# tomershay100/mp3-steganography-lib

Hardware: AMD Instinct MI355X
Metric: MP3 frames/sec (decode+re-encode) @44.1kHz stereo 128kbps, 1→8 GPU (higher is better)
Workload: dtype f64 (decode) / int32 (encode); 1 GPU; 10000-frame full decode->stego-embed->re-encode pipeline per MI355X (BASELINE configs[2]); MP3 main data + side info resident in HBM, MP3 frames out; the message cursor chain is decided and the serial chains of the rate loop are checked on the device inside every step; frames_per_gpu=10000, channels=2, message_bits=536, chain_verdict_units_to_redo=0, message_variant_entries=1874, parallelism=frames sharded over 1 GPU(s), no collective

## Files before the change

mp3-steganography-lib_amd/csrc/k_encode.hpp:

```cpp
#pragma once
#include <type_traits>
#include "analysis_plan.h"
#include "analysis_sign_plan.h"
#ifndef MP3S_AN_CLOCKS
#define MP3S_AN_CLOCKS 0
#endif
#if MP3S_AN_CLOCKS
__device__ uint32_t g_an_clocks[4096 * 8];
extern "C" __attribute__((visibility("default"))) int mp3s_debug_an_clocks(uint32_t *out)
{
    (void)hipDeviceSynchronize();
    return (int)hipMemcpyFromSymbol(out, HIP_SYMBOL(g_an_clocks), sizeof(uint32_t) * 4096 * 8);
}
#endif

namespace mp3s {

__device__ __forceinline__ int32_t mulhi_vs(int32_t v, int32_t s)
{
    int32_t r;
    asm("v_mul_hi_i32 %0, %1, %2" : "=v"(r) : "v"(v), "s"(s));
    return r;
}
typedef int32_t i32x4 __attribute__((ext_vector_type(4)));
typedef int32_t i32x16 __attribute__((ext_vector_type(16)));
typedef int32_t i32x8 __attribute__((ext_vector_type(8)));
template <int B, int E, class F>
__device__ __forceinline__ void static_for(F &&f)
{
    if constexpr (B < E) { f(std::integral_constant<int, B>{}); static_for<B + 1, E>(f); }
}

constexpr int ENC_ROW = 34;
constexpr int ENC_LDS_DW = 79 * 17 + 1;

constexpr int sign_plan_pass(int n)
{
    int p = 0;
    while (p < 7 && n >= ANALYSIS_SIGN_FIRST[p + 1]) p++;
    return p;
}
constexpr int sign_plan_pos(int n)
{
    int pos = 0;
    if (n >= ANALYSIS_SIGN_PRODUCTS) return 0;
    while (n - pos > ANALYSIS_SIGN_FIRST[sign_plan_pass(n)] && ANALYSIS_SIGN_SET[n - pos - 1] == ANALYSIS_SIGN_SET[n]) pos++;
    return pos;
}

constexpr int ENC_TROW = 33;
template <bool TILE, class Between>
__device__ __forceinline__ void enc_analysis_wave(const int16_t *__restrict__ pcm, const mp3s_frame_hdr *__restrict__ hdr, long Ts, int ch, long t0, int lane,
                                                  uint32_t *lds, int32_t *__restrict__ SB, uint32_t *rows, long tile_t0, long lo, long hi, bool shared, Between between)
{
    int16_t *tw = reinterpret_cast<int16_t *>(lds);
#if MP3S_AN_CLOCKS
    const unsigned long long ck_start = __builtin_readcyclecounter();
    unsigned long long ck_out = 0;
#endif
    if ((reinterpret_cast<uintptr_t>(pcm) & 15u) == 0) {
        const int c0 = (int)(t0 - 15) * 8, c1 = (int)Ts * 8;
        const uint4 *gp = reinterpret_cast<const uint4 *>(pcm);
        const uint32_t sel = ch ? 0x07060302u : 0x05040100u;
        constexpr int TRIPS = (79 * 8 + 63) / 64, LAST = 79 * 8 - 64 * (TRIPS - 1);
        uint4 q[TRIPS];
#pragma unroll
        for (int i = 0; i < TRIPS; i++) {
            const int gc = c0 + lane + 64 * i;
            q[i] = gp[gc < 0 ? 0 : gc < c1 ? gc : c1 - 1];
        }
#pragma unroll
        for (int i = 0; i < TRIPS; i++) {
            const int c = lane + 64 * i, gc = c0 + c;
            const bool in = gc >= 0 && gc < c1;
            asm volatile("" : "+v"(q[i].x), "+v"(q[i].y), "+v"(q[i].z), "+v"(q[i].w));
            uint2 o;
            o.x = in ? __builtin_amdgcn_perm(q[i].y, q[i].x, sel) : 0u;
            o.y = in ? __builtin_amdgcn_perm(q[i].w, q[i].z, sel) : 0u;
            uint32_t *dst = reinterpret_cast<uint32_t *>(tw + (c >> 3) * ENC_ROW + (c & 7) * 4);
            if (i < TRIPS - 1 || lane < LAST) { dst[0] = o.x; dst[1] = o.y; }
        }
    } else {
        for (int e = lane; e < 79 * 32; e += 64) {
            const int r = e >> 5, s = e & 31;
            const long row = t0 - 15 + r;
            int16_t v = 0;
            if (row >= 0 && row < Ts) v = pcm[(row * 32 + s) * 2 + ch];
            tw[r * ENC_ROW + s] = v;
        }
    }
    __builtin_amdgcn_s_waitcnt(0xc07f);
    __builtin_amdgcn_wave_barrier();
#if MP3S_AN_CLOCKS
    const unsigned long long ck_staged = __builtin_readcyclecounter();
#endif
    const long t = t0 + lane;
    const bool valid = t >= 0 && t < Ts;
    long s0 = 0;
    if (valid) s0 = (long)hdr[t / 36].stream_first * 36;

    int32_t y[64];
    const bool starts_inside = __ballot(valid && (t - 15) < s0) != 0;
    const uint32_t tw_lds = (uint32_t)(uintptr_t)(__attribute__((address_space(3))) const int16_t *)tw;
    uint32_t xs[16];
#pragma unroll
    for (int i = 0; i < 16; i++) xs[i] = 0;
#define MP3S_LDS_HI16(reg, addr, off) asm volatile("ds_read_u16_d16_hi %0, %1 offset:%2" : "+v"(reg) : "v"(addr), "n"(off))
    auto window_sums = [&](auto masked) {
    auto trip = [&](int k, auto first) {
        const i32x16 *ewa = reinterpret_cast<const i32x16 *>(c_tab.enwindow + 64 * k), *ewb = ewa + 4;
#pragma unroll
        for (int h = 0; h < 2; h++) {
            const i32x16 a0 = ewa[2 * h], a1 = ewa[2 * h + 1];
            const i32x16 b0 = ewb[2 * h], b1 = ewb[2 * h + 1];
            const int back_a = 2 * k + h, back_b = back_a + 2;
            const bool in_a = (t - back_a) >= s0, in_b = (t - back_b) >= s0;
            const uint32_t ra = tw_lds + (uint32_t)((lane + 15 - back_a) * ENC_ROW * 2), rb = ra - 2 * ENC_ROW * 2;
#pragma unroll
            for (int cb = 0; cb < 4; cb++) {
#pragma unroll
                for (int e = 0; e < 8; e++) {
                    MP3S_LDS_HI16(xs[e], ra, (cb * 8 + e) * 2);
                    MP3S_LDS_HI16(xs[8 + e], rb, (cb * 8 + e) * 2);
                }
                asm volatile("s_waitcnt lgkmcnt(0)" : "+v"(xs[0]), "+v"(xs[1]), "+v"(xs[2]), "+v"(xs[3]), "+v"(xs[4]), "+v"(xs[5]), "+v"(xs[6]), "+v"(xs[7]),
                             "+v"(xs[8]), "+v"(xs[9]), "+v"(xs[10]), "+v"(xs[11]), "+v"(xs[12]), "+v"(xs[13]), "+v"(xs[14]), "+v"(xs[15]));
#pragma unroll
                for (int e = 0; e < 8; e++) {
                    const int col = cb * 8 + e, c = 31 - col;
                    int32_t xa = (int32_t)xs[e], xb = (int32_t)xs[8 + e];
                    if (decltype(masked)::value && !in_a) xa = 0;
                    if (decltype(masked)::value && !in_b) xb = 0;
                    const int32_t two = mulhi_vs(xa, c < 16 ? a0[c & 15] : a1[c & 15]) + mulhi_vs(xb, c < 16 ? b0[c & 15] : b1[c & 15]);
                    if (decltype(first)::value) y[h * 32 + c] = two; else y[h * 32 + c] += two;
                }
                __builtin_amdgcn_sched_barrier(0);
            }
        }
    };
    trip(0, std::true_type{});
#pragma unroll 1
    for (int k = 2; k < 8; k += 2) trip(k, std::false_type{});
    };
    if (starts_inside) window_sums(std::true_type{}); else window_sums(std::false_type{});
#undef MP3S_LDS_HI16
#if MP3S_AN_CLOCKS
    asm volatile("" : "+v"(y[0]), "+v"(y[31]), "+v"(y[32]), "+v"(y[63]));
    const unsigned long long ck_summed = __builtin_readcyclecounter();
#endif
    const bool odd_slot = (t & 1) != 0;
    __builtin_amdgcn_wave_barrier();
    between();
    uint32_t *ot = lds;
    uint32_t *out = TILE ? nullptr : reinterpret_cast<uint32_t *>(SB) + ((long)ch * Ts + t0) * 32;
    const int n_rows = (Ts - t0) < 64 ? (int)(Ts - t0) : 64;
    uint32_t *trow = TILE ? rows + (valid && t >= lo && t < hi ? (t - tile_t0) : -1) * ENC_TROW : nullptr;
    int32_t a[4] = {0, 0, 0, 0};
    i32x8 cur[4], nxt[4];
    typedef const int32_t __attribute__((address_space(4))) *fl_ptr;
    fl_ptr flp = (fl_ptr)&c_tab.fl[0][0];
    asm volatile("" : "+s"(flp));
    auto load_block = [&](auto nc, i32x8 (&c)[4]) {
        constexpr int N = decltype(nc)::value, P = N >> 3, B = N & 7;
        constexpr int O[4] = {P, 15 - P, 16 + P, 31 - P};
#pragma unroll
        for (int o = 0; o < 4; o++) c[o] = *(const i32x8 __attribute__((address_space(4))) *)(flp + O[o] * 64 + 8 * B);
    };
    auto matrix_equal = [&](auto &&finish_pass) {
    load_block(std::integral_constant<int, 0>{}, cur);
    static_for<0, 64>([&](auto nc) {
        constexpr int N = decltype(nc)::value, P = N >> 3, B = N & 7;
        __builtin_amdgcn_sched_barrier(0);
        __builtin_amdgcn_s_waitcnt(0xc07f);
        __builtin_amdgcn_sched_barrier(0);
        if constexpr (N < 63) load_block(std::integral_constant<int, N + 1>{}, nxt);
        __builtin_amdgcn_sched_barrier(0);
#pragma unroll
        for (int j = 0; j < 8; j += 2) {
            int32_t m[2][4];
#pragma unroll
            for (int e = 0; e < 2; e++) {
                const int k = B * 8 + j + e;
                const unsigned plan = ANALYSIS_PLAN[P][k];
                const int32_t cj[4] = {cur[0][j + e], cur[1][j + e], cur[2][j + e], cur[3][j + e]};
#pragma unroll
                for (int o = 0; o < 4; o++) {
                    const unsigned rep = (plan >> (2 * o)) & 3u;
                    if ((plan >> (8 + o)) & 1u) m[e][o] = 0;
                    else if (rep == (unsigned)o) m[e][o] = mulhi_vs(y[k], cj[o]);
                    else m[e][o] = m[e][rep];
                }
            }
#pragma unroll
            for (int o = 0; o < 4; o++) {
                a[o] += m[0][o] + m[1][o];
                asm("" : "+v"(a[o]));
            }
            if (j == 2) __builtin_amdgcn_sched_barrier(0);
        }
        if constexpr (B == 7) {
            finish_pass(std::integral_constant<int, P>{});
            a[0] = a[1] = a[2] = a[3] = 0;
        }
        if constexpr (N < 63) {
#pragma unroll
            for (int o = 0; o < 4; o++) cur[o] = nxt[o];
        }
    });
    };
    auto finish_pass = [&](auto pc) {
            constexpr int P = decltype(pc)::value;
            if (odd_slot) {
                if (P & 1) { a[0] = (int32_t)(0u - (uint32_t)a[0]); a[2] = (int32_t)(0u - (uint32_t)a[2]); }
                else       { a[1] = (int32_t)(0u - (uint32_t)a[1]); a[3] = (int32_t)(0u - (uint32_t)a[3]); }
            }
            constexpr int q = P & 3;
            if constexpr (TILE) {
                trow[P] = (uint32_t)a[0]; trow[15 - P] = (uint32_t)a[1]; trow[16 + P] = (uint32_t)a[2]; trow[31 - P] = (uint32_t)a[3];
            } else {
            ot[lane * 17 + q] = (uint32_t)a[0];
            ot[lane * 17 + 4 + 3 - q] = (uint32_t)a[1];
            ot[lane * 17 + 8 + q] = (uint32_t)a[2];
            ot[lane * 17 + 12 + 3 - q] = (uint32_t)a[3];
            }
            if constexpr (q == 3 && !TILE) {
                constexpr int g = P >> 2;
#if MP3S_AN_CLOCKS
                const unsigned long long ck_o = __builtin_readcyclecounter();
#endif
                __builtin_amdgcn_s_waitcnt(0xc07f);
                __builtin_amdgcn_wave_barrier();
                const int piece = lane & 3;
#pragma unroll
                for (int r = lane >> 2; r < 64; r += 16) {
                    const uint32_t *src = ot + r * 17 + piece * 4;
                    const uint4 v = make_uint4(src[0], src[1], src[2], src[3]);
                    if (r < n_rows) *reinterpret_cast<uint4 *>(out + r * 32 + g * 16 + piece * 4) = v;
                }
                __builtin_amdgcn_s_waitcnt(0xc07f);
                __builtin_amdgcn_wave_barrier();
#if MP3S_AN_CLOCKS
                ck_out += __builtin_readcyclecounter() - ck_o;
#endif
            }
    };
    fl_ptr fsp = (fl_ptr)&c_fl_sign[0];
    auto load_sign_block = [&](auto bc, i32x8 (&c)[4]) {
        constexpr int Bk = decltype(bc)::value;
#pragma unroll
        for (int o = 0; o < 4; o++) c[o] = *(const i32x8 __attribute__((address_space(4))) *)(fsp + Bk * ANALYSIS_SIGN_BLOCK + 8 * o);
    };
    auto matrix_signed = [&]() {
    static_assert(ANALYSIS_SIGN_BLOCK == 32 && ANALYSIS_SIGN_STREAM % ANALYSIS_SIGN_BLOCK == 0, "four s_load_dwordx8 per block");
    constexpr int NBLK = ANALYSIS_SIGN_STREAM / ANALYSIS_SIGN_BLOCK;
    uint32_t S = 0, pend = 0;
    asm volatile("" : "+s"(fsp));
#pragma unroll
    for (int o = 0; o < 4; o++) a[o] = -ANALYSIS_SIGN_NEG[0][o];
    load_sign_block(std::integral_constant<int, 0>{}, cur);
    static_for<0, NBLK>([&](auto bc) {
        constexpr int Bk = decltype(bc)::value;
        __builtin_amdgcn_sched_barrier(0);
        __builtin_amdgcn_s_waitcnt(0xc07f);
        __builtin_amdgcn_sched_barrier(0);
        if constexpr (Bk + 1 < NBLK) load_sign_block(std::integral_constant<int, Bk + 1>{}, nxt);
        __builtin_amdgcn_sched_barrier(0);
        static_for<0, ANALYSIS_SIGN_BLOCK / 8>([&](auto qc) {
            constexpr int Q = decltype(qc)::value;
            uint32_t m[8];
            static_for<0, 8>([&](auto ic) {
                constexpr int I = Q * 8 + decltype(ic)::value, n = Bk * ANALYSIS_SIGN_BLOCK + I;
                if constexpr (n < ANALYSIS_SIGN_PRODUCTS) m[I & 7] = (uint32_t)mulhi_vs(y[ANALYSIS_SIGN_COL[n]], cur[I >> 3][I & 7]);
            });
            static_for<0, 8>([&](auto ic) {
                constexpr int I = Q * 8 + decltype(ic)::value, n = Bk * ANALYSIS_SIGN_BLOCK + I;
                if constexpr (n < ANALYSIS_SIGN_PRODUCTS) {
                    constexpr int P = sign_plan_pass(n), pos = sign_plan_pos(n);
                    constexpr unsigned set = ANALYSIS_SIGN_SET[n];
                    constexpr bool last = sign_plan_pos(n + 1) == 0;
                    constexpr bool multi = ((set & 0x55u) & ((set & 0x55u) - 1u)) != 0;
                    if constexpr ((pos & 1) == 0 && !last) pend = m[I & 7];
                    else {
                        const uint32_t two = (pos & 1) ? pend + m[I & 7] : m[I & 7];
                        if constexpr (!multi) {
#pragma unroll
                            for (int o = 0; o < 4; o++)
                                if ((set >> (2 * o)) & 1u) a[o] = (int32_t)((uint32_t)a[o] + two);
                        } else {
                            if constexpr (pos < 2) S = two; else S += two;
                            if constexpr (last) {
#pragma unroll
                                for (int o = 0; o < 4; o++) {
                                    const unsigned f = (set >> (2 * o)) & 3u;
                                    if (f == 1u) a[o] = (int32_t)((uint32_t)a[o] + S);
                                    if (f == 3u) a[o] = (int32_t)((uint32_t)a[o] - S);
                                }
                            }
                        }
                    }
                    if constexpr (n + 1 == ANALYSIS_SIGN_FIRST[P + 1]) {
                        finish_pass(std::integral_constant<int, P>{});
                        if constexpr (P < 7) {
#pragma unroll
                            for (int o = 0; o < 4; o++) a[o] = -ANALYSIS_SIGN_NEG[P + 1][o];
                        }
                    }
                }
            });
            asm("" : "+v"(a[0]), "+v"(a[1]), "+v"(a[2]), "+v"(a[3]), "+v"(S), "+v"(pend));
            __builtin_amdgcn_sched_barrier(0);
        });
        if constexpr (Bk + 1 < NBLK) {
#pragma unroll
            for (int o = 0; o < 4; o++) cur[o] = nxt[o];
        }
    });
    };
    bool use_signed = shared;
    if (shared) {
        uint32_t ymin = 0xffffffffu;
        static_for<0, 64>([&](auto kc) {
            constexpr int k = decltype(kc)::value;
            if constexpr ((ANALYSIS_SIGN_ZERO_COLS >> k) & 1u) ymin = ymin < (uint32_t)y[k] ? ymin : (uint32_t)y[k];
        });
        const bool counts = valid && (!TILE || (t >= lo && t < hi));
        use_signed = __ballot(counts && ymin == 0u) == 0;
    }
    if (use_signed) matrix_signed(); else matrix_equal(finish_pass);
#if MP3S_AN_CLOCKS
    if (!TILE && lane == 0) {
        const unsigned long long ck_end = __builtin_readcyclecounter();
        uint32_t *d = g_an_clocks + ((size_t)((t0 >> 6) * 2 + ch) & 4095) * 8;
        d[0] = (uint32_t)(ck_staged - ck_start); d[1] = (uint32_t)(ck_summed - ck_staged); d[2] = (uint32_t)(ck_end - ck_summed - ck_out);
        d[3] = (uint32_t)ck_out; d[4] = (uint32_t)(ck_end - ck_start); d[5] = (starts_inside ? 1u : 0u) | (use_signed ? 2u : 0u);
    }
#endif
}

__device__ __forceinline__ int sb_pos(int band) { return (int)((0x37621540u >> (4 * (band >> 2))) & 7u) * 4 + (band & 3); }
__global__ __launch_bounds__(256, 5) void k_enc_analysis(
    const int16_t *__restrict__ pcm, const mp3s_frame_hdr *__restrict__ hdr, int n_frames,
    int32_t *__restrict__ SB, long Ts, int shared)
{
    __shared__ __attribute__((aligned(16))) uint32_t lds_all[4][ENC_LDS_DW];
    static_assert(79 * ENC_ROW * 2 <= ENC_LDS_DW * 4, "PCM tile must fit");
    const int wave = __builtin_amdgcn_readfirstlane(threadIdx.x >> 6), lane = threadIdx.x & 63;
    const long wid = (long)xcd_tile() * 4 + wave;
    const int ch = (int)(wid & 1);
    const long t0 = (wid >> 1) * 64;
    if (t0 >= Ts) return;
    enc_analysis_wave<false>(pcm, hdr, Ts, ch, t0, lane, lds_all[wave], SB, nullptr, 0, 0, 0, shared != 0, [] {});
}

constexpr int MD_ROW = 33, MD_BLK = 18 * MD_ROW;

__device__ __forceinline__ void enc_mdct_pair(const int32_t (&in)[54], int32_t *xs, int lane, int32_t *__restrict__ mdct, long ga, long g_lo, long g_hi)
{
    const int ch = lane >> 5, band = lane & 31;
    int32_t *x0 = xs + ch * MD_BLK + band, *x1 = x0 + 2 * MD_BLK;
    struct Coef { i32x4 q[9]; };
    auto load_coef = [&](int k) {
        Coef c;
        const i32x4 *crow = reinterpret_cast<const i32x4 *>(c_tab.cos_l[k]);
#pragma unroll
        for (int q = 0; q < 9; q++) c.q[q] = crow[q];
        return c;
    };
    Coef cur = load_coef(0);
#pragma unroll 2
    for (int k = 0; k < 18; k++) {
        asm volatile("" ::"s"(cur.q[0].x));
        __builtin_amdgcn_sched_barrier(0);
        const Coef nxt = load_coef(k < 17 ? k + 1 : 17);
        __builtin_amdgcn_sched_barrier(0);
        int32_t a0 = 0, a1 = 0;
#pragma unroll
        for (int q = 0; q < 9; q++) {
            const i32x4 c = cur.q[q];
            a0 += mulhi_vs(in[4 * q], c.x);     a1 += mulhi_vs(in[18 + 4 * q], c.x);
            a0 += mulhi_vs(in[4 * q + 1], c.y); a1 += mulhi_vs(in[19 + 4 * q], c.y);
            a0 += mulhi_vs(in[4 * q + 2], c.z); a1 += mulhi_vs(in[20 + 4 * q], c.z);
            a0 += mulhi_vs(in[4 * q + 3], c.w); a1 += mulhi_vs(in[21 + 4 * q], c.w);
        }
        x0[k * MD_ROW] = a0;
        x1[k * MD_ROW] = a1;
        __builtin_amdgcn_sched_barrier(0);
        cur = nxt;
    }
    __builtin_amdgcn_s_waitcnt(0xc07f);
    __builtin_amdgcn_wave_barrier();
    if (band >= 1) {
#pragma unroll
        for (int g = 0; g < 2; g++)
#pragma unroll
            for (int i = 0; i < 8; i++) {
                int32_t *pa = x0 + g * 2 * MD_BLK + i * MD_ROW, *pb = x0 + g * 2 * MD_BLK + (17 - i) * MD_ROW - 1;
                const int64_t cs = c_tab.mdct_cs[i], ca = c_tab.mdct_ca[i];
                const int64_t a = *pa, b = *pb;
                *pa = (int32_t)((a * cs - b * ca) >> 31);
                *pb = (int32_t)((a * ca + b * cs) >> 31);
            }
    }
    __builtin_amdgcn_s_waitcnt(0xc07f);
    __builtin_amdgcn_wave_barrier();
#pragma unroll
    for (int q = 0; q < 4; q++) {
        const long g = ga + (q >> 1);
        if (g < g_lo || g >= g_hi) continue;
        const int32_t *src = xs + q * MD_BLK;
        int32_t *o = mdct + (((g >> 1) * 2 + (q & 1)) * 2 + (g & 1)) * 576;
#pragma unroll
        for (int t = 0; t < 9; t++) {
            const int e = lane + 64 * t, b = (e * 3641) >> 16, k = e - 18 * b;
            o[e] = src[k * MD_ROW + b];
        }
    }
}

__global__ __launch_bounds__(256, 4) void k_enc_mdct(
    const int32_t *__restrict__ SB, long Ts, const mp3s_frame_hdr *__restrict__ hdr, int n_frames,
    int32_t *__restrict__ mdct)
{
    __shared__ int32_t xs_all[4][4 * MD_BLK];
    const int wave = __builtin_amdgcn_readfirstlane(threadIdx.x >> 6), lane = threadIdx.x & 63;
    const int f = xcd_tile() * 4 + wave;
    if (f >= n_frames) return;
    const int ch = lane >> 5, band = lane & 31;
    const bool has_prev = f > (int)hdr[f].stream_first;
    const int32_t *row = SB + ((long)ch * Ts + (long)f * 36) * 32 + sb_pos(band);
    const int32_t *prow = has_prev ? row - 18 * 32 : row;
    int32_t in[54];
#pragma unroll
    for (int j = 0; j < 18; j++) {
        const int32_t pv = prow[j * 32];
        in[j] = has_prev ? pv : 0;
        in[18 + j] = row[j * 32];
        in[36 + j] = row[(18 + j) * 32];
    }
    enc_mdct_pair(in, xs_all[wave], lane, mdct, 2l * f, 2l * f, 2l * f + 2);
}

constexpr int EF_GR = 13, EF_SLOTS = 18 * (EF_GR + 1), EF_WAVES = 8;
constexpr int EF_TILE_DW = 2 * (EF_SLOTS + 1) * ENC_TROW;
static_assert(EF_SLOTS <= 4 * 64, "four analysis waves per channel");
static_assert(EF_WAVES * ENC_LDS_DW <= EF_TILE_DW, "the waves' PCM staging fits the tile");
static_assert(((EF_GR + 1) / 2) * 4 * MD_BLK <= EF_TILE_DW, "the MDCT waves' butterfly tiles fit the tile");

__global__ __launch_bounds__(EF_WAVES * 64, 4) void k_enc_fused(
    const int16_t *__restrict__ pcm, const mp3s_frame_hdr *__restrict__ hdr, int n_frames, int32_t *__restrict__ mdct, int shared)
{
    __shared__ __attribute__((aligned(16))) uint32_t tile[EF_TILE_DW];
    const int wave = __builtin_amdgcn_readfirstlane(threadIdx.x >> 6), lane = threadIdx.x & 63;
    const long Ts = (long)n_frames * 36, n_gran = (long)n_frames * 2;
    const long g0 = (long)xcd_tile() * EF_GR;
    const long s0 = g0 * 18, t_first = s0 - 18;
    {
        const int ch = wave >> 2;
        const long t0 = t_first + 64 * (wave & 3);
        uint32_t *rows = tile + ((long)ch * (EF_SLOTS + 1) + 1) * ENC_TROW;
        enc_analysis_wave<true>(pcm, hdr, Ts, ch, t0, lane, tile + wave * ENC_LDS_DW, nullptr, rows, t_first, t_first, t_first + EF_SLOTS, shared != 0,
                                [] { __syncthreads(); });
    }
    __syncthreads();
    const long ga = g0 - (g0 & 1) + 2 * wave;
    const long g_hi = g0 + EF_GR < n_gran ? g0 + EF_GR : n_gran;
    const bool unit = ga < g_hi;
    int32_t in[54];
    if (unit) {
        const int ch = lane >> 5, band = lane & 31;
        const bool has_prev = ga >= g0 && ga > (long)hdr[ga >> 1].stream_first * 2;
        const long r_prev = (ga - g0) * 18;
        const uint32_t *row = tile + ((long)ch * (EF_SLOTS + 1) + 1 + (r_prev >= 0 ? r_prev : 0)) * ENC_TROW + band;
        const long r_own = r_prev >= 0 ? 18 : 0;
#pragma unroll
        for (int j = 0; j < 18; j++) {
            const int32_t pv = (int32_t)row[j * ENC_TROW];
            in[j] = has_prev ? pv : 0;
            in[18 + j] = (int32_t)row[(r_own + j) * ENC_TROW];
            in[36 + j] = ga + 1 < g_hi ? (int32_t)row[(r_own + 18 + j) * ENC_TROW] : 0;
        }
    }
    __syncthreads();
    if (unit) enc_mdct_pair(in, reinterpret_cast<int32_t *>(tile) + wave * 4 * MD_BLK, lane, mdct, ga, g0, g_hi);
}

}
```

mp3-steganography-lib_amd/csrc/mp3s_api.cpp:

```cpp
#include "chain_resolve.h"

namespace {
thread_local std::string g_err;
}

int mp3s::fail(int code, const char *fmt, ...)
{
    char buf[512];
    va_list ap;
    va_start(ap, fmt);
    vsnprintf(buf, sizeof buf, fmt, ap);
    va_end(ap);
    g_err = buf;
    return code;
}

int max_part2_3(const mp3s_frame_side *side, long n)
{
    int m = 0;
    for (long f = 0; f < n; f++)
        for (int k = 0; k < 4; k++) m = std::max<int>(m, side[f].unit[k >> 1][k & 1].part2_3_length);
    return m;
}

void select_entries(int first_unit, int reach, int first_entry, int hide_end, int64_t bits_left, int32_t *ent_unit, int32_t *ent_cursor)
{
    const int tail = (int)MP3S_SELECT_TAIL_FIRST(bits_left, (int64_t)reach);
    int at = first_entry;
    for (int v = 0; v < MP3S_SELECT_VARIANTS; v++) {
        const int32_t cur = v < 8 ? 4 * v : hide_end - (10 - v);
        for (int j = v < 8 ? 0 : tail; j < reach; j++) {
            ent_unit[at] = first_unit + j;
            ent_cursor[at++] = cur;
        }
    }
}

enum OptKind { kOptFlag, kOptNumber, kOptClamped, kOptMask, kOptOneOf };
struct OptRow { int id; const char *env; bool env_off; OptKind kind; int64_t dflt, lo, hi; };
constexpr int64_t kOptNoLimit = INT64_MAX, kResampleValues[] = {0, 1, 32000, 44100, 48000};
constexpr OptRow kOptions[] = {
    {MP3S_OPT_ANALYSIS_SHARED, "MP3S_ANALYSIS_SHARED", false, kOptFlag, 1, 0, 1},
    {MP3S_OPT_SELECT, "MP3S_NO_SELECT", true, kOptFlag, 1, 0, 1},
    {MP3S_OPT_REDO, "MP3S_NO_REDO", true, kOptFlag, 1, 0, 1},
    {MP3S_OPT_FAST_IMDCT, "MP3S_FAST_IMDCT", false, kOptFlag, 1, 0, 1},
    {MP3S_OPT_PIPE_TAIL, "MP3S_PIPE_TAIL", false, kOptClamped, 1, 0, 2},
    {MP3S_OPT_CHUNK_FRAMES, "MP3S_CHUNK_FRAMES", false, kOptNumber, 0, 4, kOptNoLimit},
    {MP3S_OPT_DEVICE_PARSE, "MP3S_DEVICE_PARSE", false, kOptFlag, 1, 0, 1},
    {MP3S_OPT_FILE_PIPELINE, "MP3S_FILE_PIPELINE", false, kOptFlag, 1, 0, 1},
    {MP3S_OPT_SCAN_THREADS, "MP3S_SCAN_THREADS", false, kOptNumber, 0, 0, 64},
    {MP3S_OPT_FIRST_CHUNK_FRAMES, "MP3S_FIRST_CHUNK_FRAMES", false, kOptNumber, 0, 4, kOptNoLimit},
    {MP3S_OPT_FILE_UP, "MP3S_NO_FILE_UP", true, kOptFlag, 1, 0, 1},
    {MP3S_OPT_HUF_LANES, "MP3S_HUF_LANES", false, kOptNumber, 0, 0, kOptNoLimit},
    {MP3S_OPT_NUMA, "MP3S_NO_NUMA", true, kOptFlag, 1, 0, 1},
    {MP3S_OPT_FLOAT_FAST, "MP3S_FLOAT_FAST", false, kOptFlag, 0, 0, 1},
    {MP3S_OPT_FAIL_CHUNK, nullptr, false, kOptNumber, 0, 0, kOptNoLimit},
    {MP3S_OPT_FUSED_DECODE, "MP3S_FUSED_DECODE", false, kOptFlag, 1, 0, 1},
    {MP3S_OPT_FUSED_ENCODE, "MP3S_FUSED_ENCODE", false, kOptFlag, 0, 0, 1},
    {MP3S_OPT_PIPE_DEC, "MP3S_PIPE_DEC", false, kOptFlag, 0, 0, 1},
    {MP3S_OPT_RATE_SIGNALS, "MP3S_RATE_SIGNALS", false, kOptFlag, 0, 0, 1},
    {MP3S_OPT_PIPE_SIGNALS, "MP3S_PIPE_SIGNALS", false, kOptMask, 0, 0, 3},
    {MP3S_OPT_WAV_IMPORT, "MP3S_WAV_IMPORT", false, kOptFlag, 0, 0, 1},
    {MP3S_OPT_WAV_RESAMPLE, "MP3S_WAV_RESAMPLE", false, kOptOneOf, 0, 0, 48000},
};
constexpr bool options_in_order(int i = 0) { return i == MP3S_OPT_COUNT || (kOptions[i].id == i && options_in_order(i + 1)); }
static_assert(sizeof kOptions / sizeof *kOptions == MP3S_OPT_COUNT && options_in_order(), "one row per MP3S_OPT_*, row i for option i");

static bool resample_value(int64_t v) { return std::find(std::begin(kResampleValues), std::end(kResampleValues), v) != std::end(kResampleValues); }
static int64_t option_from_env(const OptRow &o)
{
    const char *v = o.env ? getenv(o.env) : nullptr;
    if (o.env_off) return v ? 0 : o.dflt;
    const int64_t x = v && *v ? (int64_t)atoll(v) : o.dflt;
    switch (o.kind) {
    case kOptFlag: return x != 0;
    case kOptNumber: return std::max<int64_t>(0, x);
    case kOptClamped: return std::min(o.hi, std::max(o.lo, x));
    case kOptMask: return x & o.hi;
    default: return resample_value(x) ? x : 0;
    }
}

extern "C" {

const char *mp3s_last_error(void) { return g_err.c_str(); }
const char *mp3s_version(void) { return "mp3s-hip 0.1 (gfx950)"; }
void mp3s_buf_free(mp3s_buf *b) { delete b; }
const void *mp3s_debug_tables(size_t *bytes)
{
    if (bytes) *bytes = sizeof(DevTables);
    return &host_tables().dev;
}

int mp3s_debug_scfsi_energies(const int32_t *xr576, int sr_idx, int32_t *en22)
{
    if (!xr576 || !en22 || sr_idx < 0 || sr_idx > 2) return fail(MP3S_E_ARG, "bad argument");
    host_scfsi_energies(xr576, sr_idx, en22);
    return MP3S_OK;
}

int mp3s_debug_parse_scanned_frame(const void *frame_side, const uint8_t *blob, int16_t *is2304, mp3s_granule_si *si4)
{
    if (!frame_side || !blob || !is2304 || !si4) return fail(MP3S_E_ARG, "null pointer");
    const int rc = parse_scanned_frame(*static_cast<const mp3s_frame_side *>(frame_side), blob, is2304, si4);
    return rc ? fail(rc, "malformed main data") : MP3S_OK;
}

int mp3s_debug_walk_rate(const uint8_t *file, size_t len, double seconds, double *frames_per_s, int64_t *frames_per_pass)
{
    if (!file || !frames_per_s || seconds <= 0) return fail(MP3S_E_ARG, "bad argument");
    std::vector<FrameRef> refs;
    std::vector<uint8_t> tables;
    const double t0 = now_ms();
    int64_t frames = 0, per_pass = 0;
    double t = t0;
    do {
        FrameWalker w;
        const long n = std::max(0L, walk_whole(file, len, refs, w, &tables, 1000));
        if (w.irregular) return fail(MP3S_E_UNSUPPORTED, "not a stream the walk takes");
        if (!w.ended) return fail(MP3S_E_MALFORMED, "malformed or unsupported MP3 stream");
        frames += n; per_pass = n;
        t = now_ms();
    } while (t - t0 < seconds * 1e3);
    *frames_per_s = (double)frames / ((t - t0) * 1e-3);
    if (frames_per_pass) *frames_per_pass = per_pass;
    return MP3S_OK;
}

int mp3s_device_count(int *n)
{
    if (!n) return fail(MP3S_E_ARG, "n is null");
    int k = 0;
    *n = hipGetDeviceCount(&k) == hipSuccess && k > 0 ? k : 0;
    return MP3S_OK;
}

int mp3s_ctx_create(int device, mp3s_ctx **out)
{
    if (!out) return fail(MP3S_E_ARG, "out is null");
    *out = nullptr;
    int n = 0;
    hipError_t e = hipGetDeviceCount(&n);
    if (e != hipSuccess || n <= 0)
        return fail(MP3S_E_NO_DEVICE, "no HIP device available (%s); the transforms have no CPU fallback",
                    e == hipSuccess ? "device count 0" : hipGetErrorString(e));
    if (device < 0 || device >= n) return fail(MP3S_E_ARG, "device %d out of range (0..%d)", device, n - 1);
    e = hipSetDevice(device);
    if (e != hipSuccess) return fail(MP3S_E_NO_DEVICE, "hipSetDevice(%d): %s", device, hipGetErrorString(e));
    mp3s_ctx *c = new mp3s_ctx();
    c->chain = new ChainResolver();
    c->device = device;
    for (const OptRow &o : kOptions) c->opt[o.id] = option_from_env(o);
    if (hipStreamCreateWithFlags(&c->stream, hipStreamNonBlocking) != hipSuccess ||
        hipEventCreate(&c->ev0) != hipSuccess || hipEventCreate(&c->ev1) != hipSuccess ||
        hipEventCreateWithFlags(&c->ev_order, hipEventDisableTiming) != hipSuccess) {
        mp3s_ctx_destroy(c);
        return fail(MP3S_E_NO_DEVICE, "stream/event creation failed");
    }
    if (hipMalloc((void **)&c->d_sync, 32) != hipSuccess || hipMemsetAsync(c->d_sync, 0, 32, c->stream) != hipSuccess) {
        mp3s_ctx_destroy(c);
        return fail(MP3S_E_NO_DEVICE, "device scratch allocation failed");
    }
    const int rc = dev_upload_tables(c->stream);
    if (rc) {
        mp3s_ctx_destroy(c);
        return fail(MP3S_E_NO_DEVICE, "constant table upload failed: %s (is this a gfx950 device?)",
                    hipGetErrorString((hipError_t)rc));
    }
    *out = c;
    return MP3S_OK;
}

void mp3s_ctx_destroy(mp3s_ctx *c)
{
    if (!c) return;
    hipSetDevice(c->device);
    destroy_own_pipe(c);
    if (c->stream) hipStreamSynchronize(c->stream);
    if (c->scratch) hipFree(c->scratch);
    if (c->scratch_enc) hipFree(c->scratch_enc);
    if (c->d_sync) hipFree(c->d_sync);
    for (void *q : c->pool) if (q) hipFree(q);
    for (const mp3s_ctx::ResampleTaps &t : c->res_taps) hipFree(t.d);
    if (c->ev0) hipEventDestroy(c->ev0);
    if (c->ev1) hipEventDestroy(c->ev1);
    if (c->ev_order) hipEventDestroy(c->ev_order);
    if (c->ev_sel) hipEventDestroy(c->ev_sel);
    if (c->ev_pcm_tiles) hipEventDestroy(c->ev_pcm_tiles);
    if (c->stream) hipStreamDestroy(c->stream);
    delete c->chain;
    delete c;
}

int mp3s_ctx_host_share(mp3s_ctx *c, mp3s_host_share *out)
{
    if (!out) return fail(MP3S_E_ARG, "null pointer");
    size_t held = 0, cap = 0;
    PinnedBlock::pool_state(&held, &cap);
    out->pinned_pooled_bytes = held; out->pinned_pool_cap_bytes = cap;
    out->local_world_size = local_world_size();
    out->cpus_allowed = host_cpus_allowed();
    out->gpu_node_cpus = c ? (int32_t)gpu_node_cpus(c->device).size() : 0;
    out->reserved = 0;
    return MP3S_OK;
}

int mp3s_ctx_set_option(mp3s_ctx *c, int option, int64_t value)
{
    if (!c || option < 0 || option >= MP3S_OPT_COUNT) return fail(MP3S_E_ARG, "unknown option %d", option);
    const OptRow &o = kOptions[option];
    if (value < 0 || (o.kind == kOptNumber && ((value != 0 && value < o.lo) || value > o.hi)))
        return fail(MP3S_E_ARG, "option %d: value %lld out of range", option, (long long)value);
    if (o.kind == kOptOneOf && !resample_value(value))
        return fail(MP3S_E_ARG, "option %d: %lld is not 0, 1, 32000, 44100 or 48000", option, (long long)value);
    c->opt[option] = o.kind == kOptFlag ? value != 0 : (o.kind == kOptClamped ? std::min(value, o.hi) : value);
    return MP3S_OK;
}

int mp3s_ctx_run_stats(mp3s_ctx *c, mp3s_run_stats *out)
{
    if (!c || !out) return fail(MP3S_E_ARG, "null pointer");
    *out = c->run_stats;
    own_pipe_lanes(c, out);
    return MP3S_OK;
}

int mp3s_ctx_get_option(mp3s_ctx *c, int option, int64_t *value)
{
    if (!c || !value || option < 0 || option >= MP3S_OPT_COUNT) return fail(MP3S_E_ARG, "unknown option %d", option);
    *value = c->opt[option];
    return MP3S_OK;
}

int mp3s_device_name(mp3s_ctx *c, char *buf, size_t n)
{
    if (!c || !buf || !n) return fail(MP3S_E_ARG, "bad argument");
    hipDeviceProp_t p;
    HIPCHK(hipGetDeviceProperties(&p, c->device));
    snprintf(buf, n, "%s (%s, %d CUs)", p.name, p.gcnArchName, p.multiProcessorCount);
    return MP3S_OK;
}

int mp3s_device_pci(mp3s_ctx *c, char *buf, size_t n)
{
    if (!c || !buf || n < 16) return fail(MP3S_E_ARG, "bad argument");
    HIPCHK(hipDeviceGetPCIBusId(buf, (int)n, c->device));
    for (char *p = buf; *p; p++) *p = (char)tolower(*p);
    return MP3S_OK;
}

int mp3s_sync(mp3s_ctx *c)
{
    if (!c) return fail(MP3S_E_ARG, "ctx is null");
    HIPCHK(hipStreamSynchronize(c->stream));
    return MP3S_OK;
}

int mp3s_ctx_wait(mp3s_ctx *c, mp3s_ctx *other)
{
    if (!c || !other) return fail(MP3S_E_ARG, "ctx is null");
    if (c == other) return MP3S_OK;
    if (c->device != other->device) return fail(MP3S_E_ARG, "contexts on different devices");
    HIPCHK(hipEventRecord(other->ev_order, other->stream));
    HIPCHK(hipStreamWaitEvent(c->stream, other->ev_order, 0));
    return MP3S_OK;
}

int mp3s_ctx_wait_last(mp3s_ctx *c, mp3s_ctx *other)
{
    if (!c || !other) return fail(MP3S_E_ARG, "ctx is null");
    if (c == other) return MP3S_OK;
    if (c->device != other->device) return fail(MP3S_E_ARG, "contexts on different devices");
    HIPCHK(hipStreamWaitEvent(c->stream, other->ev_order, 0));
    return MP3S_OK;
}

int mp3s_dev_alloc(mp3s_ctx *c, size_t bytes, void **dptr)
{
    if (!c || !dptr) return fail(MP3S_E_ARG, "bad argument");
    HIPCHK(hipSetDevice(c->device));
    hipError_t e = hipMalloc(dptr, bytes ? bytes : 16);
    if (e != hipSuccess) return fail(MP3S_E_NOMEM, "hipMalloc(%zu): %s", bytes, hipGetErrorString(e));
    return MP3S_OK;
}
int mp3s_dev_free(mp3s_ctx *c, void *dptr)
{
    if (!c) return fail(MP3S_E_ARG, "ctx is null");
    if (dptr) { HIPCHK(hipStreamSynchronize(c->stream)); HIPCHK(hipFree(dptr)); }
    return MP3S_OK;
}
int mp3s_dev_upload(mp3s_ctx *c, void *dptr, const void *host, size_t bytes)
{
    if (!c || (!dptr && bytes) || (!host && bytes)) return fail(MP3S_E_ARG, "bad argument");
    if (!bytes) return MP3S_OK;
    HIPCHK(hipMemcpyAsync(dptr, host, bytes, hipMemcpyHostToDevice, c->stream));
    HIPCHK(hipStreamSynchronize(c->stream));
    return MP3S_OK;
}
int mp3s_dev_download(mp3s_ctx *c, void *host, const void *dptr, size_t bytes)
{
    if (!c || (!dptr && bytes) || (!host && bytes)) return fail(MP3S_E_ARG, "bad argument");
    if (!bytes) return MP3S_OK;
    HIPCHK(hipMemcpyAsync(host, dptr, bytes, hipMemcpyDeviceToHost, c->stream));
    HIPCHK(hipStreamSynchronize(c->stream));
    return MP3S_OK;
}
int mp3s_dev_memset(mp3s_ctx *c, void *dptr, int value, size_t bytes)
{
    if (!c || !dptr) return fail(MP3S_E_ARG, "bad argument");
    HIPCHK(hipMemsetAsync(dptr, value, bytes, c->stream));
    return MP3S_OK;
}
int mp3s_dev_copy(mp3s_ctx *c, void *d_dst, const void *d_src, size_t bytes)
{
    if (!c || !d_dst || !d_src) return fail(MP3S_E_ARG, "bad argument");
    if (bytes) HIPCHK(hipMemcpyAsync(d_dst, d_src, bytes, hipMemcpyDeviceToDevice, c->stream));
    return MP3S_OK;
}
int mp3s_timer_start(mp3s_ctx *c)
{
    if (!c) return fail(MP3S_E_ARG, "ctx is null");
    HIPCHK(hipEventRecord(c->ev0, c->stream));
    return MP3S_OK;
}
int mp3s_timer_stop(mp3s_ctx *c, float *ms)
{
    if (!c || !ms) return fail(MP3S_E_ARG, "bad argument");
    HIPCHK(hipEventRecord(c->ev1, c->stream));
    HIPCHK(hipEventSynchronize(c->ev1));
    HIPCHK(hipEventElapsedTime(ms, c->ev0, c->ev1));
    return MP3S_OK;
}

int mp3s_synth_mode(mp3s_ctx *c, double eps_scale, int64_t *exact_samples)
{
    if (!c || eps_scale < 0) return fail(MP3S_E_ARG, "bad argument");
    HIPCHK(hipStreamSynchronize(c->stream));
    int32_t n = 0;
    HIPCHK(hipMemcpy(&n, c->d_sync + 2, 4, hipMemcpyDeviceToHost));
    HIPCHK(hipMemset(c->d_sync + 2, 0, 4));
    if (exact_samples) *exact_samples = n;
    c->synth_eps_scale = eps_scale;
    return MP3S_OK;
}

int mp3s_bench_copy(mp3s_ctx *c, size_t bytes, int iters, double *gb_per_s)
{
    if (!c || !gb_per_s || bytes < 4096 || iters < 1) return fail(MP3S_E_ARG, "bad argument");
    HIPCHK(hipSetDevice(c->device));
    bytes &= ~(size_t)15;
    void *a = nullptr, *b = nullptr;
    if (hipMalloc(&a, bytes) != hipSuccess || hipMalloc(&b, bytes) != hipSuccess) { if (a) hipFree(a); return fail(MP3S_E_NOMEM, "hipMalloc(%zu) x 2", bytes); }
    int rc = MP3S_OK;
    float ms = 0;
    if (hipMemsetAsync(a, 1, bytes, c->stream) != hipSuccess || launch_copy(c->stream, a, b, bytes) != 0) rc = fail(MP3S_E_HIP, "copy launch failed");
    if (!rc && hipEventRecord(c->ev0, c->stream) != hipSuccess) rc = fail(MP3S_E_HIP, "event");
    for (int i = 0; i < iters && !rc; i++) if (launch_copy(c->stream, i & 1 ? b : a, i & 1 ? a : b, bytes) != 0) rc = fail(MP3S_E_HIP, "copy launch failed");
    if (!rc && (hipEventRecord(c->ev1, c->stream) != hipSuccess || hipEventSynchronize(c->ev1) != hipSuccess ||
                hipEventElapsedTime(&ms, c->ev0, c->ev1) != hipSuccess)) rc = fail(MP3S_E_HIP, "event");
    hipStreamSynchronize(c->stream);
    hipFree(a); hipFree(b);
    if (!rc) *gb_per_s = 2.0 * (double)bytes * iters / (ms * 1e-3) / 1e9;
    return rc;
}

int mp3s_profile_enable(mp3s_ctx *c, int on)
{
    if (!c) return fail(MP3S_E_ARG, "ctx is null");
    HIPCHK(hipStreamSynchronize(c->stream));
    c->prof.enabled = on != 0;
    c->prof.n_pairs = 0;
    for (int k = 0; k < K_COUNT; k++) { c->prof.total_ms[k] = 0; c->prof.count[k] = 0; }
    return MP3S_OK;
}

int mp3s_profile_select(mp3s_ctx *c, unsigned mask)
{
    if (!c) return fail(MP3S_E_ARG, "ctx is null");
    c->prof.mask = mask;
    return MP3S_OK;
}

int mp3s_profile_collect(mp3s_ctx *c, double *total_ms, int64_t *launches, int n)
{
    if (!c || !total_ms || !launches || n < MP3S_N_KERNELS_MIN) return fail(MP3S_E_ARG, "bad argument (need %d slots)", (int)MP3S_N_KERNELS_MIN);
    HIPCHK(hipStreamSynchronize(c->stream));
    Profiler &p = c->prof;
    for (int i = 0; i < p.n_pairs; i++) {
        float ms = 0;
        HIPCHK(hipEventElapsedTime(&ms, p.ev[2 * i], p.ev[2 * i + 1]));
        p.total_ms[p.kid[i]] += ms;
        p.count[p.kid[i]] += 1;
    }
    p.n_pairs = 0;
    if (p.dropped) {
        const long lost = p.dropped;
        p.dropped = 0;
        return fail(MP3S_E_ARG, "%ld timed launches had no event pair left (collect at least every %d launches)", lost, Profiler::MAX_PAIRS);
    }
    for (int k = 0; k < K_COUNT && k < n; k++) { total_ms[k] = p.total_ms[k]; launches[k] = p.count[k]; }
    static_assert(K_COUNT == MP3S_N_KERNELS, "kernel list out of sync with mp3s.h");
    return MP3S_OK;
}

int mp3s_decode_transform_dev(mp3s_ctx *c, const int16_t *d_is, const mp3s_granule_si *d_si, const mp3s_frame_hdr *d_hdr,
                              int n_frames, int nch, int n_halo, int out_format, void *d_pcm)
{
    if (!c || !d_is || !d_si || !d_hdr || !d_pcm) return fail(MP3S_E_ARG, "null pointer");
    if (n_frames <= 0 || nch < 1 || nch > 2 || n_halo < 0 || n_halo >= n_frames || out_format < 0 || out_format > 2)
        return fail(MP3S_E_ARG, "bad sizes: n_frames=%d nch=%d n_halo=%d fmt=%d", n_frames, nch, n_halo, out_format);
    if (const int rc = c->ensure_scratch(dec_scratch_bytes(n_frames, nch))) return rc;
    if (int pe = guard_probe_usable(c, out_format)) return pe;
    const int e = launch_decode(c->stream, d_is, d_si, d_hdr, n_frames, nch, n_halo, out_format, d_pcm, c->scratch, &c->prof, decode_how(c, 0, nullptr, 0));
    return e ? fail(MP3S_E_HIP, "decode launch: %s", hipGetErrorString((hipError_t)e)) : (int)MP3S_OK;
}

int mp3s_debug_guard_margin(mp3s_ctx *c, double *d_x, double *d_eps, int64_t capacity)
{
    if (!c) return fail(MP3S_E_ARG, "null context");
    if ((d_x == nullptr) != (d_eps == nullptr) || (d_x && capacity <= 0)) return fail(MP3S_E_ARG, "both arrays and their capacity, or neither");
    HIPCHK(hipStreamSynchronize(c->stream));
    c->guard_probe = GuardProbe{d_x, d_eps, 0, d_x ? capacity : 0};
    return MP3S_OK;
}

static int check_hdr(const mp3s_frame_hdr *hdr, int n)
{
    for (int f = 0; f < n; f++) {
        if (hdr[f].stream_first > (uint32_t)f) return fail(MP3S_E_ARG, "hdr[%d].stream_first=%u points forward", f, hdr[f].stream_first);
        if (f && hdr[f].stream_first != (uint32_t)f && hdr[f].stream_first != hdr[f - 1].stream_first)
            return fail(MP3S_E_ARG, "hdr[%d].stream_first is not monotone", f);
        if (hdr[f].sr_idx > 2) return fail(MP3S_E_ARG, "hdr[%d].sr_idx=%d", f, hdr[f].sr_idx);
    }
    if (n && hdr[0].stream_first != 0) return fail(MP3S_E_ARG, "hdr[0].stream_first must be 0");
    return 0;
}

int mp3s_decode_transform(mp3s_ctx *c, const int16_t *is, const mp3s_granule_si *si, const mp3s_frame_hdr *hdr,
                          int n_frames, int nch, int n_halo, int out_format, void *pcm)
{
    if (!c || !is || !si || !hdr || !pcm) return fail(MP3S_E_ARG, "null pointer");
    if (n_frames <= 0 || n_halo < 0 || n_halo >= n_frames) return fail(MP3S_E_ARG, "bad sizes");
    int rc = check_hdr(hdr, n_frames);
    if (rc) return rc;
    for (size_t i = 0; i < (size_t)n_frames * 2304; i++)
        if (is[i] > 8206 || is[i] < -8206) return fail(MP3S_E_ARG, "is[%zu]=%d outside +-8206", i, is[i]);
    HIPCHK(hipSetDevice(c->device));
    void *d_is = nullptr, *d_si = nullptr, *d_hdr = nullptr, *d_pcm = nullptr;
    const size_t b_is = (size_t)n_frames * 2304 * 2, b_si = (size_t)n_frames * 4 * sizeof(mp3s_granule_si),
                 b_hdr = (size_t)n_frames * sizeof(mp3s_frame_hdr),
                 b_pcm = (size_t)(n_frames - n_halo) * 1152 * nch * pcm_elem(out_format);
    rc = MP3S_OK;
    if (hipMalloc(&d_is, b_is) != hipSuccess || hipMalloc(&d_si, b_si) != hipSuccess ||
        hipMalloc(&d_hdr, b_hdr) != hipSuccess || hipMalloc(&d_pcm, b_pcm) != hipSuccess)
        rc = fail(MP3S_E_NOMEM, "hipMalloc failed for a %d-frame batch", n_frames);
    if (!rc) rc = mp3s_dev_upload(c, d_is, is, b_is);
    if (!rc) rc = mp3s_dev_upload(c, d_si, si, b_si);
    if (!rc) rc = mp3s_dev_upload(c, d_hdr, hdr, b_hdr);
    if (!rc) rc = mp3s_decode_transform_dev(c, (const int16_t *)d_is, (const mp3s_granule_si *)d_si,
                                            (const mp3s_frame_hdr *)d_hdr, n_frames, nch, n_halo, out_format, d_pcm);
    if (!rc) rc = mp3s_dev_download(c, pcm, d_pcm, b_pcm);
    hipStreamSynchronize(c->stream);
    hipFree(d_is); hipFree(d_si); hipFree(d_hdr); hipFree(d_pcm);
    return rc;
}

int mp3s_encode_transform_dev(mp3s_ctx *c, const int16_t *d_pcm, const mp3s_frame_hdr *d_hdr, int n_frames, int32_t *d_mdct)
{
    if (!c || !d_pcm || !d_hdr || !d_mdct) return fail(MP3S_E_ARG, "null pointer");
    if (n_frames <= 0) return fail(MP3S_E_ARG, "n_frames=%d", n_frames);
    return encode_transform_step(c, c->stream, d_pcm, d_hdr, n_frames, d_mdct);
}

int mp3s_encode_transform(mp3s_ctx *c, const int16_t *pcm, const mp3s_frame_hdr *hdr, int n_frames, int32_t *mdct)
{
    if (!c || !pcm || !hdr || !mdct) return fail(MP3S_E_ARG, "null pointer");
    if (n_frames <= 0) return fail(MP3S_E_ARG, "n_frames=%d", n_frames);
    int rc = check_hdr(hdr, n_frames);
    if (rc) return rc;
    HIPCHK(hipSetDevice(c->device));
    void *d_pcm = nullptr, *d_hdr = nullptr, *d_mdct = nullptr;
    const size_t b_pcm = (size_t)n_frames * 1152 * 2 * 2, b_hdr = (size_t)n_frames * sizeof(mp3s_frame_hdr),
                 b_mdct = (size_t)n_frames * 2304 * 4;
    if (hipMalloc(&d_pcm, b_pcm) != hipSuccess || hipMalloc(&d_hdr, b_hdr) != hipSuccess ||
        hipMalloc(&d_mdct, b_mdct) != hipSuccess)
        rc = fail(MP3S_E_NOMEM, "hipMalloc failed for a %d-frame batch", n_frames);
    if (!rc) rc = mp3s_dev_upload(c, d_pcm, pcm, b_pcm);
    if (!rc) rc = mp3s_dev_upload(c, d_hdr, hdr, b_hdr);
    if (!rc) rc = mp3s_encode_transform_dev(c, (const int16_t *)d_pcm, (const mp3s_frame_hdr *)d_hdr, n_frames, (int32_t *)d_mdct);
    if (!rc) rc = mp3s_dev_download(c, mdct, d_mdct, b_mdct);
    hipStreamSynchronize(c->stream);
    hipFree(d_pcm); hipFree(d_hdr); hipFree(d_mdct);
    return rc;
}

int mp3s_rate_loop_dev(mp3s_ctx *c, const int32_t *d_mdct, const mp3s_rate_frame *d_frames, int n_frames,
                       const uint8_t *d_hide_bits, int n_hide, const int32_t *d_cursor_in, const int32_t *d_state_in,
                       const int32_t *d_unit_list, int n_list, int16_t *d_ix, mp3s_gr_out *d_out, int32_t *d_en)
{
    if (!c || !d_mdct || !d_frames || !d_ix || !d_out || !d_en) return fail(MP3S_E_ARG, "null pointer");
    if (n_frames <= 0 || n_hide < 0 || (n_hide > 0 && (!d_hide_bits || !d_cursor_in)))
        return fail(MP3S_E_ARG, "bad sizes / missing hide inputs");
    return rate_step(c, c->stream, rate_signal_default(c), d_mdct, d_frames, n_frames, d_hide_bits, n_hide, d_cursor_in, d_state_in, d_unit_list, n_list, d_ix, d_out, d_en);
}

void mp3s_select_patterns(uint8_t out[32])
{
    for (int v = 0; v < 8; v++) { out[4 * v] = (v >> 2) & 1; out[4 * v + 1] = (v >> 1) & 1; out[4 * v + 2] = v & 1; out[4 * v + 3] = 0; }
}

int mp3s_select_plan(const mp3s_chain_seg *segs, int n_segs, mp3s_select_span *spans, int32_t *ent_unit, int32_t *ent_cursor, int cap)
{
    return select_plan(segs, n_segs, spans, ent_unit, ent_cursor, cap, nullptr);
}

}

int select_plan(const mp3s_chain_seg *segs, int n_segs, mp3s_select_span *spans, int32_t *ent_unit, int32_t *ent_cursor, int cap,
                const int32_t *min_reach)
{
    if (!segs || !spans || n_segs <= 0 || cap < 0 || ((ent_unit == nullptr) != (ent_cursor == nullptr))) return fail(MP3S_E_ARG, "bad argument");
    int used = 0;
    for (int i = 0; i < n_segs; i++) {
        const mp3s_chain_seg &g = segs[i];
        spans[i].first_entry = used; spans[i].reach = 0;
        const int64_t left = (int64_t)g.hide_end - g.hide_begin;
        if (left <= 0 || g.n_frames <= 0 || g.hide_base < 32) continue;
        const int64_t reach = std::min<int64_t>((int64_t)g.n_frames * 4, std::max<int64_t>(left * 5 / 14 + 32, min_reach ? min_reach[i] : 0));
        if (reach > MP3S_SELECT_MAX_REACH || (int64_t)used + MP3S_SELECT_ENTRIES(left, reach) > cap) continue;
        spans[i].reach = (int32_t)reach;
        if (ent_unit) select_entries(g.first_frame * 4, (int)reach, used, g.hide_end, left, ent_unit, ent_cursor);
        used += (int)MP3S_SELECT_ENTRIES(left, reach);
    }
    return used;
}

int encode_transform_step(mp3s_ctx *c, hipStream_t stream, const int16_t *d_pcm, const mp3s_frame_hdr *d_hdr, int n_frames, int32_t *d_mdct)
{
    if (!host_tables().analysis_plan_ok)
        return fail(MP3S_E_TABLES, "the analysis filter table built on this host does not repeat itself where the kernel shares products "
                                   "(csrc/analysis_plan.h, csrc/analysis_sign_plan.h: run tools/gen_analysis_plan.py and tools/gen_analysis_sign_plan.py here and rebuild)");
    const bool fused = c->opt[MP3S_OPT_FUSED_ENCODE] != 0;
    if (const int rc = fused ? (int)MP3S_OK : c->ensure_scratch_enc(enc_scratch_bytes(n_frames))) return rc;
    const int e = launch_encode(stream, d_pcm, d_hdr, n_frames, d_mdct, c->scratch_enc, &c->prof, fused, c->opt[MP3S_OPT_ANALYSIS_SHARED] != 0);
    return e ? fail(MP3S_E_HIP, "encode launch: %s", hipGetErrorString((hipError_t)e)) : (int)MP3S_OK;
}

int rate_step(mp3s_ctx *c, hipStream_t stream, hipEvent_t done, const int32_t *d_mdct, const mp3s_rate_frame *d_frames, int n_frames, const uint8_t *d_hide,
              int n_hide, const int32_t *d_cursor, const int32_t *d_state, const int32_t *d_list, int n_list, int16_t *d_ix, mp3s_gr_out *d_out, int32_t *d_en,
              const RateVariantArgs *variants)
{
    if (variants && c->sel_pending && hipStreamWaitEvent(stream, c->ev_sel, 0) != hipSuccess) return fail(MP3S_E_HIP, "ordering behind the previous selection failed");
    if (variants) c->sel_pending = false;
    const int e = launch_rate(stream, d_mdct, d_frames, n_frames, d_hide, n_hide, d_cursor, d_state, d_list, n_list, d_ix, d_out, d_en, &c->prof, 0, 0, variants, done);
    return e ? fail(MP3S_E_HIP, "rate launch: %s", hipGetErrorString((hipError_t)e)) : (int)MP3S_OK;
}

int select_step(mp3s_ctx *c, hipStream_t stream, const uint8_t *d_hide, int32_t *d_cursor, const mp3s_chain_seg *d_segs, const mp3s_select_span *d_spans,
                int n_segs, int max_reach, const RateVariantArgs &va, int16_t *d_ix, mp3s_gr_out *d_out, int32_t *d_en)
{
    void *d_pairs = c->grab(kPoolSelectDev, (size_t)n_segs * max_reach * 8, stream);
    if (!d_pairs) return fail(MP3S_E_NOMEM, "hipMalloc failed for the selection scratch");
    const int e = launch_select(stream, d_segs, d_spans, n_segs, max_reach, d_hide, va, d_ix, d_en, d_out, d_cursor, d_pairs, &c->prof);
    if (e) return fail(MP3S_E_HIP, "select launch: %s", hipGetErrorString((hipError_t)e));
    if (stream == c->stream) return MP3S_OK;
    if (!c->ev_sel && hipEventCreateWithFlags(&c->ev_sel, hipEventDisableTiming) != hipSuccess) return fail(MP3S_E_HIP, "event creation failed");
    if (hipEventRecord(c->ev_sel, stream) != hipSuccess) return fail(MP3S_E_HIP, "event record failed");
    c->sel_pending = true;
    return MP3S_OK;
}

int pack_step(mp3s_ctx *c, hipStream_t stream, const int16_t *d_ix, const mp3s_gr_out *d_gr, const int32_t *d_en, int n_frames, int sri, int bri, int whole,
              const uint32_t *d_frame_off, const uint8_t *d_padding, uint8_t *d_mp3, int32_t *d_scfsi, int32_t *d_status)
{
    const int e = launch_pack(stream, d_ix, d_gr, d_en, n_frames, sri, bri, whole, d_frame_off, d_padding, d_mp3, d_scfsi, d_status, c->d_sync, &c->prof);
    return e ? fail(MP3S_E_HIP, "pack launch: %s", hipGetErrorString((hipError_t)e)) : (int)MP3S_OK;
}

extern "C" {

int mp3s_rate_variants_dev(mp3s_ctx *c, const int32_t *d_mdct, const mp3s_rate_frame *d_frames, int n_frames, const uint8_t *d_hide_bits,
                           int n_hide, const int32_t *d_cursor, const int32_t *d_ent_unit, const int32_t *d_ent_cursor, int n_entries,
                           int16_t *d_ix, mp3s_gr_out *d_out, int32_t *d_en, int16_t *d_ixv, mp3s_gr_out *d_outv, int32_t *d_env)
{
    if (!c || !d_mdct || !d_frames || !d_ix || !d_out || !d_en || !d_hide_bits || !d_cursor || !d_ent_unit || !d_ent_cursor || !d_ixv ||
        !d_outv || !d_env)
        return fail(MP3S_E_ARG, "null pointer");
    if (n_frames <= 0 || n_hide < 32 || n_entries <= 0) return fail(MP3S_E_ARG, "bad sizes");
    const RateVariantArgs va = variant_args(d_ent_unit, d_ent_cursor, n_entries, d_ixv, d_outv, d_env);
    return rate_step(c, c->stream, rate_signal_default(c), d_mdct, d_frames, n_frames, d_hide_bits, n_hide, d_cursor, nullptr, nullptr, 0, d_ix, d_out, d_en, &va);
}

int mp3s_select_dev(mp3s_ctx *c, const uint8_t *d_hide_bits, int32_t *d_cursor, const mp3s_chain_seg *d_segs, const mp3s_select_span *d_spans,
                    int n_segs, int max_reach, const int32_t *d_ent_unit, const int32_t *d_ent_cursor, int n_entries, int16_t *d_ix,
                    mp3s_gr_out *d_out, int32_t *d_en, int16_t *d_ixv, mp3s_gr_out *d_outv, int32_t *d_env)
{
    if (!c || !d_ix || !d_out || !d_en || !d_hide_bits || !d_cursor || !d_segs || !d_spans || !d_ent_unit || !d_ent_cursor || !d_ixv ||
        !d_outv || !d_env)
        return fail(MP3S_E_ARG, "null pointer");
    if (n_segs <= 0 || n_entries <= 0 || max_reach <= 0 || max_reach > MP3S_SELECT_MAX_REACH) return fail(MP3S_E_ARG, "bad sizes");
    return select_step(c, c->stream, d_hide_bits, d_cursor, d_segs, d_spans, n_segs, max_reach, variant_args(d_ent_unit, d_ent_cursor, n_entries, d_ixv, d_outv, d_env),
                       d_ix, d_out, d_en);
}

int mp3s_rate_select_dev(mp3s_ctx *c, const int32_t *d_mdct, const mp3s_rate_frame *d_frames, int n_frames, const uint8_t *d_hide_bits,
                         int n_hide, int32_t *d_cursor, const mp3s_chain_seg *d_segs, const mp3s_select_span *d_spans, int n_segs,
                         int max_reach, const int32_t *d_ent_unit, const int32_t *d_ent_cursor, int n_entries, int16_t *d_ix,
                         mp3s_gr_out *d_out, int32_t *d_en, int16_t *d_ixv, mp3s_gr_out *d_outv, int32_t *d_env)
{
    if (!d_segs || !d_spans) return fail(MP3S_E_ARG, "null pointer");
    if (n_segs <= 0 || max_reach <= 0 || max_reach > MP3S_SELECT_MAX_REACH) return fail(MP3S_E_ARG, "bad sizes");
    if (const int rc = mp3s_rate_variants_dev(c, d_mdct, d_frames, n_frames, d_hide_bits, n_hide, d_cursor, d_ent_unit, d_ent_cursor, n_entries, d_ix, d_out, d_en, d_ixv,
                                              d_outv, d_env)) return rc;
    return mp3s_select_dev(c, d_hide_bits, d_cursor, d_segs, d_spans, n_segs, max_reach, d_ent_unit, d_ent_cursor, n_entries, d_ix, d_out, d_en,
                           d_ixv, d_outv, d_env);
}

int mp3s_chain_resolve_dev(mp3s_ctx *c, mp3s_gr_out *d_gr, const mp3s_rate_frame *d_frames, int n_frames, const mp3s_chain_seg *d_segs,
                           int n_segs, const int32_t *d_cursor_in, const int32_t *d_state_in, int32_t *d_verdict,
                           mp3s_chain_seg_out *d_seg_out)
{
    if (!c || !d_gr || !d_frames || !d_segs || !d_verdict || !d_seg_out) return fail(MP3S_E_ARG, "null pointer");
    if (n_frames <= 0 || n_segs <= 0) return fail(MP3S_E_ARG, "bad sizes");
    void *d_agg = c->grab(kPoolChainDev, chain_agg_bytes(n_frames));
    if (!d_agg) return fail(MP3S_E_NOMEM, "hipMalloc failed for the chain scratch");
    const int e = launch_chain(c->stream, d_gr, d_frames, n_frames, d_segs, d_cursor_in, d_state_in, d_agg, d_verdict, d_seg_out, &c->prof);
    if (e) return fail(MP3S_E_HIP, "chain launch: %s", hipGetErrorString((hipError_t)e));
    return MP3S_OK;
}

int mp3s_chain_redo_dev(mp3s_ctx *c, const int32_t *d_mdct, const mp3s_rate_frame *d_frames, int n_frames, const uint8_t *d_hide_bits, int n_hide,
                        int32_t *d_cursor, const mp3s_chain_seg *d_segs, int n_segs, int16_t *d_ix, mp3s_gr_out *d_gr, int32_t *d_en,
                        int32_t *d_verdict, mp3s_chain_seg_out *d_seg_out)
{
    if (!c || !d_mdct || !d_gr || !d_frames || !d_segs || !d_verdict || !d_seg_out || !d_ix || !d_en) return fail(MP3S_E_ARG, "null pointer");
    if (n_frames <= 0 || n_segs <= 0 || n_hide < 0 || (n_hide > 0 && (!d_hide_bits || !d_cursor))) return fail(MP3S_E_ARG, "bad sizes");
    void *d_agg = c->grab(kPoolChainDev, chain_agg_bytes(n_frames));
    if (!d_agg) return fail(MP3S_E_NOMEM, "hipMalloc failed for the chain scratch");
    const ChainRedoArgs redo = {d_mdct, d_hide_bits, n_hide, d_ix, d_en};
    const int e = launch_chain(c->stream, d_gr, d_frames, n_frames, d_segs, d_cursor, nullptr, d_agg, d_verdict, d_seg_out, &c->prof, &redo);
    if (e) return fail(MP3S_E_HIP, "chain launch: %s", hipGetErrorString((hipError_t)e));
    return MP3S_OK;
}

int mp3s_huffman_decode_dev(mp3s_ctx *c, const uint8_t *d_blob, const mp3s_frame_side *d_side, int n_frames, int nch,
                            int max_part2_3_length, int16_t *d_is, mp3s_granule_si *d_si, int32_t *d_status)
{
    if (!c || !d_blob || !d_side || !d_is || !d_si || !d_status) return fail(MP3S_E_ARG, "null pointer");
    if (n_frames <= 0 || nch < 1 || nch > 2 || max_part2_3_length < 0) return fail(MP3S_E_ARG, "bad sizes");
    if (max_part2_3_length == 0 || max_part2_3_length > 4095) max_part2_3_length = 4095;
    const int e = launch_huffman(c->stream, d_blob, d_side, n_frames, nch, max_part2_3_length, d_is, d_si, d_status, c->d_sync + 4, &c->prof, false, (int)c->opt[MP3S_OPT_HUF_LANES]);
    if (e) return fail(MP3S_E_HIP, "huffman launch: %s", hipGetErrorString((hipError_t)e));
    return MP3S_OK;
}

int mp3s_pack_frames_dev(mp3s_ctx *c, const int16_t *d_ix, const mp3s_gr_out *d_gr, const int32_t *d_en, int n_frames,
                         int samplerate, int bitrate_kbps, const uint32_t *d_frame_off, const uint8_t *d_padding,
                         uint8_t *d_mp3, int32_t *d_scfsi, int32_t *d_status)
{
    if (!c || !d_ix || !d_gr || !d_en || !d_frame_off || !d_padding || !d_mp3 || !d_scfsi || !d_status)
        return fail(MP3S_E_ARG, "null pointer");
    int sri, bri, whole;
    if (n_frames <= 0 || stream_params(samplerate, bitrate_kbps, &sri, &bri, &whole))
        return fail(MP3S_E_UNSUPPORTED, "unsupported samplerate/bitrate %d/%d", samplerate, bitrate_kbps);
    return pack_step(c, c->stream, d_ix, d_gr, d_en, n_frames, sri, bri, whole, d_frame_off, d_padding, d_mp3, d_scfsi, d_status);
}

int mp3s_scan_stream(const uint8_t *file, size_t len, mp3s_buf **owner, mp3s_scanned *out)
{
    if (!file || !owner || !out) return fail(MP3S_E_ARG, "null pointer");
    mp3s_buf *b = new mp3s_buf();
    const int rc = parse_stream(file, len, b->parsed, &b->scanned);
    if (rc) { delete b; return fail(rc, "malformed or unsupported MP3 stream"); }
    const ParsedStream &p = b->parsed;
    out->n_frames = p.n_frames; out->nch = p.nch; out->sampling_rate = p.sampling_rate; out->bit_rate = p.bit_rate;
    out->n_bits = (int32_t)p.bits.size(); out->dup_last_frame = p.dup_last_frame;
    out->gpu_ok = b->scanned.gpu_ok ? 1 : 0;
    out->max_part2_3_length = max_part2_3(b->scanned.side.data(), p.n_frames);
    out->side = b->scanned.side.data(); out->hdr = p.hdr.data();
    out->blob = b->scanned.blob.data(); out->blob_len = b->scanned.blob.size();
    out->bits = p.bits.data(); out->frame_size = p.frame_size.data();
    *owner = b;
    return MP3S_OK;
}

int mp3s_walk_stream(const uint8_t *file, size_t len, mp3s_buf **owner, mp3s_walked *out)
{
    if (!file || !owner || !out) return fail(MP3S_E_ARG, "null pointer");
    std::memset(out, 0, sizeof *out);
    std::unique_ptr<mp3s_buf> b(new mp3s_buf());
    FrameWalker w;
    const long n = std::max(0L, walk_whole(file, len, b->refs, w, &b->bits, 0x7fffffffffffffffL));
    if (!w.irregular && !w.ended) return fail(w.error, "malformed or unsupported MP3 stream");
    const FrameRef *refs = b->refs.data();
    const uint8_t *tables = b->bits.data();
    *owner = b.release();
    if (w.irregular) return MP3S_OK;
    out->regular = 1;
    out->n_frames = (int32_t)n; out->nch = w.nch; out->sampling_rate = w.sampling_rate; out->bit_rate = w.bit_rate;
    out->dup_last_frame = w.dup_last ? 1 : 0; out->max_part2_3_length = w.max_p23; out->any_silent = w.any_silent ? 1 : 0;
    out->blob_len = n > 0 ? (size_t)refs[n - 1].md_off + refs[n - 1].md_len + 8 : 0; out->refs = refs; out->tables = tables;
    out->stream.base = 0; out->stream.end = (uint32_t)len; out->stream.first_frame = 0; out->stream.n_frames = (uint32_t)n;
    if (n > 0) FrameWalker::history(refs, 0, out->stream.prev_size);
    return MP3S_OK;
}

int mp3s_parse_frames_dev(mp3s_ctx *c, const uint8_t *d_image, uint32_t image_base, const mp3s_frame_ref *d_refs, const mp3s_stream_ref *d_streams,
                          int n_frames, uint32_t md_base, mp3s_frame_side *d_side, mp3s_frame_hdr *d_hdr, uint8_t *d_blob, uint64_t *d_tsel,
                          int32_t *d_status)
{
    if (!c || !d_image || !d_refs || !d_streams || !d_side || !d_hdr || !d_blob || !d_status) return fail(MP3S_E_ARG, "null pointer");
    if (n_frames <= 0) return fail(MP3S_E_ARG, "n_frames=%d", n_frames);
    const int e = launch_parse(c->stream, d_image, image_base, d_refs, d_streams, n_frames, md_base, d_side, d_hdr, d_blob, d_tsel, d_status);
    if (e) return fail(MP3S_E_HIP, "parse launch: %s", hipGetErrorString((hipError_t)e));
    return MP3S_OK;
}

int mp3s_stego_bits(const uint64_t *tsel, int64_t n_frames, int nch, uint8_t carry[4], mp3s_buf **owner, const uint8_t **bits, size_t *n_bits)
{
    if ((!tsel && n_frames) || n_frames < 0 || nch < 1 || nch > 2 || !carry || !owner || !bits || !n_bits) return fail(MP3S_E_ARG, "bad argument");
    mp3s_buf *b = new mp3s_buf();
    stego_bits_from_tsel(tsel, (long)n_frames, nch, carry, b->bits);
    *bits = b->bits.data(); *n_bits = b->bits.size(); *owner = b;
    return MP3S_OK;
}

int mp3s_parse_stream(const uint8_t *file, size_t len, mp3s_buf **owner, mp3s_parsed *out)
{
    if (!file || !owner || !out) return fail(MP3S_E_ARG, "null pointer");
    mp3s_buf *b = new mp3s_buf();
    const int rc = parse_stream(file, len, b->parsed);
    if (rc) { delete b; return fail(rc, "malformed or unsupported MP3 stream"); }
    const ParsedStream &p = b->parsed;
    out->n_frames = p.n_frames; out->nch = p.nch; out->sampling_rate = p.sampling_rate; out->bit_rate = p.bit_rate;
    out->n_bits = (int32_t)p.bits.size(); out->dup_last_frame = p.dup_last_frame;
    out->is = p.is.data(); out->si = p.si.data(); out->hdr = p.hdr.data(); out->bits = p.bits.data();
    out->table_select = p.table_select.data(); out->frame_size = p.frame_size.data();
    *owner = b;
    return MP3S_OK;
}

int mp3s_rate_frames(int samplerate, int bitrate_kbps, int nch, int n_frames, mp3s_rate_frame *out, int32_t *padding)
{
    if (!out || n_frames < 0) return fail(MP3S_E_ARG, "bad argument");
    const int rc = rate_frames(samplerate, bitrate_kbps, nch, n_frames, out, padding);
    if (rc) return fail(rc, "unsupported samplerate/bitrate %d/%d", samplerate, bitrate_kbps);
    return MP3S_OK;
}

int mp3s_format_stream(int samplerate, int bitrate_kbps, int n_frames, const int16_t *ix, const mp3s_gr_out *gr,
                       const int32_t *scfsi, mp3s_buf **owner, const uint8_t **mp3, size_t *mp3_len)
{
    if (!ix || !gr || !scfsi || !owner || !mp3 || !mp3_len) return fail(MP3S_E_ARG, "null pointer");
    mp3s_buf *b = new mp3s_buf();
    const int rc = format_stream(samplerate, bitrate_kbps, n_frames, ix, gr, scfsi, b->bytes);
    if (rc) { delete b; return fail(rc, "format_stream failed"); }
    *owner = b; *mp3 = b->bytes.data(); *mp3_len = b->bytes.size();
    return MP3S_OK;
}

int mp3s_wav_parse(const uint8_t *file, size_t len, int bitrate_kbps, mp3s_wav_info *out)
{
    if ((!file && len) || !out) return fail(MP3S_E_ARG, "null pointer");
    const char *msg = "";
    const int rc = wav_parse(file, len, bitrate_kbps, out, &msg);
    return rc ? fail(rc, "%s", msg) : MP3S_OK;
}

int mp3s_wav_import_info(const uint8_t *file, size_t len, int bitrate_kbps, mp3s_wav_import *out)
{
    if (!file || !len || !out) return fail(MP3S_E_ARG, "null pointer");
    const char *msg = "";
    const int rc = wav_import_parse(file, len, bitrate_kbps, out, &msg);
    return rc ? fail(rc, "%s", msg) : MP3S_OK;
}

int mp3s_wav_resample_info(const uint8_t *file, size_t len, int bitrate_kbps, int mode, mp3s_wav_resample *out)
{
    if (!file || !len || !out) return fail(MP3S_E_ARG, "null pointer");
    if (mode != 1 && mode != 32000 && mode != 44100 && mode != 48000) return fail(MP3S_E_ARG, "mode %d is not 1, 32000, 44100 or 48000", mode);
    const char *msg = "";
    mp3s_wav_import w;
    const int rc = wav_import_parse(file, len, bitrate_kbps, &w, &msg, mode, out);
    return rc ? fail(rc, "%s", msg) : MP3S_OK;
}

int mp3s_wav_resample_taps(int L, int M, int32_t *taps, int cap, int32_t *T)
{
    if (!taps || !T || cap < 0) return fail(MP3S_E_ARG, "bad argument");
    std::vector<int32_t> c;
    int t = 0;
    *T = 0;
    if (wav_resample_taps(L, M, c, &t)) return fail(MP3S_E_ARG, "no tap table for the ratio %d / %d", L, M);
    *T = t;
    if (c.size() > (size_t)cap) return fail(MP3S_E_ARG, "%zu taps, room for %d", c.size(), cap);
    std::memcpy(taps, c.data(), c.size() * sizeof(int32_t));
    return MP3S_OK;
}

int mp3s_wav_header(int64_t n_rows, int nch, int rate, uint8_t *out44)
{
    if (!out44 || n_rows < 0 || nch < 1 || nch > 2 || rate < 0) return fail(MP3S_E_ARG, "bad argument");
    wav_header(n_rows, nch, rate, out44);
    return MP3S_OK;
}

int mp3s_message_frame(const uint8_t *utf8, size_t n, mp3s_buf **owner, const uint8_t **bits, size_t *n_bits)
{
    if ((!utf8 && n) || !owner || !bits || !n_bits) return fail(MP3S_E_ARG, "null pointer");
    mp3s_buf *b = new mp3s_buf();
    message_frame(utf8, n, b->bits);
    *bits = b->bits.data(); *n_bits = b->bits.size(); *owner = b;
    return MP3S_OK;
}

int mp3s_message_reveal(const uint8_t *bits, size_t n_bits, mp3s_buf **owner, const uint8_t **text, size_t *n_text)
{
    if ((!bits && n_bits) || !owner || !text || !n_text) return fail(MP3S_E_ARG, "null pointer");
    mp3s_buf *b = new mp3s_buf();
    message_reveal(bits, n_bits, b->bytes);
    *text = b->bytes.data(); *n_text = b->bytes.size(); *owner = b;
    return MP3S_OK;
}

int mp3s_reveal_message(const uint8_t *mp3, size_t len, mp3s_buf **owner, mp3s_file *out)
{
    if (!mp3 || !owner || !out) return fail(MP3S_E_ARG, "null pointer");
    mp3s_buf *b = new mp3s_buf();
    const int rc = parse_stream(mp3, len, b->parsed, &b->scanned);
    if (rc) { delete b; return fail(rc, "malformed or unsupported MP3 stream"); }
    message_reveal(b->parsed.bits.data(), b->parsed.bits.size(), b->bytes);
    std::memset(out, 0, sizeof *out);
    out->data = b->bytes.data(); out->len = b->bytes.size();
    out->kbps = b->parsed.bit_rate / 1000; out->sampling_rate = b->parsed.sampling_rate; out->channels = b->parsed.nch;
    out->n_frames = b->parsed.n_frames; out->n_bits = (int32_t)b->parsed.bits.size(); out->bits = b->parsed.bits.data();
    *owner = b;
    return MP3S_OK;
}

}
```

mp3-steganography-lib_amd/csrc/mp3s_device.h:

```cpp
#pragma once
#include <hip/hip_runtime_api.h>
#include <stddef.h>
#include <stdint.h>

#include "../../include/mp3s.h"

namespace mp3s {

#ifndef MP3S_DEC_SYNTH_TW
#define MP3S_DEC_SYNTH_TW 2
#endif
constexpr int DEC_SYNTH_TW = MP3S_DEC_SYNTH_TW;
constexpr int DEC_SYNTH_FAST_TW = 2;

enum KernelId { K_DEC_IMDCT = 0, K_DEC_SYNTH, K_ENC_ANALYSIS, K_ENC_MDCT, K_RATE_LOOP, K_DEC_HUFFMAN, K_ENC_PACK, K_CHAIN, K_WAV_RESAMPLE, K_COUNT };
struct Profiler {
    static constexpr int MAX_PAIRS = 8192;
    hipEvent_t ev[2 * MAX_PAIRS];
    int kid[MAX_PAIRS];
    int n_pairs = 0, n_created = 0;
    long dropped = 0;
    bool enabled = false;
    unsigned mask = ~0u;
    double total_ms[K_COUNT] = {0};
    long count[K_COUNT] = {0};
    int take(int k);
    int begin(hipStream_t s, int k);
    void end(hipStream_t s, int pair);
    bool attach(int k, hipEvent_t *start, hipEvent_t *stop);
};

int dev_upload_tables(hipStream_t stream);

struct GuardProbe { double *x, *eps; int64_t base, cap; };
size_t dec_scratch_bytes(int n_frames, int nch);
struct DecodeHow {
    int sf_base;
    double eps_scale;
    int32_t *d_sync;
    bool fast_imdct, float_fast, fused;
    hipEvent_t done;
    const GuardProbe *probe;
};
int launch_decode(hipStream_t stream, const int16_t *d_is, const mp3s_granule_si *d_si, const mp3s_frame_hdr *d_hdr,
                  int n_frames, int nch, int n_halo, int out_format, void *d_pcm, void *d_scratch, Profiler *prof, const DecodeHow &how);

size_t enc_scratch_bytes(int n_frames);
int launch_encode(hipStream_t stream, const int16_t *d_pcm, const mp3s_frame_hdr *d_hdr, int n_frames, int32_t *d_mdct,
                  void *d_scratch, Profiler *prof, bool fused = false ,
                  bool analysis_shared = true );

struct RateVariantArgs {
    const int32_t *d_unit, *d_cursor;
    int n;
    int16_t *d_ix; mp3s_gr_out *d_out; int32_t *d_en;
    uint8_t *d_tables;
};
inline size_t variant_out_bytes(int n) { return (size_t)n * sizeof(mp3s_gr_out) + (((size_t)n + 15) & ~(size_t)15); }
int launch_rate(hipStream_t stream, const int32_t *d_mdct, const mp3s_rate_frame *d_frames, int n_frames,
                const uint8_t *d_hide, int n_hide, const int32_t *d_cursor, const int32_t *d_state,
                const int32_t *d_list, int n_list, int16_t *d_ix, mp3s_gr_out *d_out, int32_t *d_en, Profiler *prof,
                int out_base = 0 ,
                int compact = 0 ,
                const RateVariantArgs *variants = nullptr,
                hipEvent_t done = nullptr );

struct ChainRedoArgs { const int32_t *d_mdct; const uint8_t *d_hide; int n_hide; int16_t *d_ix; int32_t *d_en; };
size_t chain_agg_bytes(int n_frames);
int launch_chain(hipStream_t stream, mp3s_gr_out *d_gr, const mp3s_rate_frame *d_frames, int n_frames, const mp3s_chain_seg *d_segs,
                 const int32_t *d_cursor, const int32_t *d_state, void *d_agg, int32_t *d_verdict, mp3s_chain_seg_out *d_seg_out,
                 Profiler *prof, const ChainRedoArgs *redo = nullptr);

int launch_select(hipStream_t stream, const mp3s_chain_seg *d_segs, const mp3s_select_span *d_spans, int n_segs, int max_reach,
                  const uint8_t *d_hide, const RateVariantArgs &v, int16_t *d_ix, int32_t *d_en, mp3s_gr_out *d_out, int32_t *d_cursor,
                  void *d_pairs , Profiler *prof);

using FrameRef = mp3s_frame_ref;
using StreamRef = mp3s_stream_ref;
constexpr int kParseInherits = 1, kParseMismatch = 2;
int launch_parse(hipStream_t stream, const uint8_t *d_image, uint32_t image_base, const FrameRef *d_refs, const StreamRef *d_streams, int n_frames,
                 uint32_t md_base, mp3s_frame_side *d_side, mp3s_frame_hdr *d_hdr, uint8_t *d_blob, uint64_t *d_tsel, int32_t *d_status);

constexpr int kRevealTile = MP3S_REVEAL_TILE;
constexpr int kRevealBadRef = MP3S_RV_BAD_REF;
constexpr int kRevealMaxStreams = 65535;
inline size_t reveal_packed_bytes(uint64_t n_frames) { return (size_t)((n_frames * 12 + 31) / 32 * 4); }
int launch_reveal(hipStream_t stream, const uint8_t *d_image, uint32_t image_base, const FrameRef *d_refs, const StreamRef *d_streams, int n_streams,
                  const uint32_t *d_out_off, uint8_t *d_packed, int32_t *d_n_bits, int32_t *d_status);

int launch_capacity(hipStream_t stream, const mp3s_gr_out *d_gr, const mp3s_chain_seg *d_segs, int n_segs, mp3s_capacity_seg *d_out, uint32_t *d_profile);

int launch_table_audit(hipStream_t stream, const int16_t *d_is, const mp3s_frame_side *d_side, int n_frames, int nch, const mp3s_table_audit_seg *d_segs,
                       int n_segs, mp3s_table_audit_unit *d_units, mp3s_table_audit *d_out, uint32_t *d_profile);

constexpr int kPcmDiffWaves = 4;
struct PcmTile { uint32_t pair, first; };
template <class Tiles>
bool pcm_diff_tiles(const mp3s_pcm_pair *pairs, int n_pairs, Tiles &tiles)
{
    uint64_t n = tiles.size();
    for (int p = 0; p < n_pairs; p++) n += ((uint64_t)pairs[p].n_frames + kPcmDiffWaves - 1) / kPcmDiffWaves;
    if (n > 0x7fffffffu) return false;
    for (int p = 0; p < n_pairs; p++)
        for (uint64_t f = 0; f < pairs[p].n_frames; f += kPcmDiffWaves) tiles.push_back(PcmTile{(uint32_t)p, (uint32_t)f});
    return true;
}
int launch_pcm_diff(hipStream_t stream, const int16_t *d_pcm, int nch, const mp3s_pcm_pair *d_pairs, int n_pairs, const PcmTile *d_tiles, int n_tiles,
                    mp3s_pcm_frame_diff *d_frames, mp3s_pcm_pair_diff *d_out);

constexpr int kPcmMaxLag = MP3S_PCM_MAX_LAG;
int launch_pcm_align(hipStream_t stream, const int16_t *d_pcm, int nch, const mp3s_pcm_run_pair *d_runs, int n_pairs, int max_lag, int search_rows,
                     const int32_t *d_given, const PcmTile *d_tiles, int n_tiles, uint64_t *d_scores, mp3s_pcm_lag *d_lags, mp3s_pcm_pair *d_geo,
                     mp3s_pcm_frame_diff *d_frames, mp3s_pcm_pair_diff *d_out);
template <class Pairs>
void pcm_align_bound_pairs(const mp3s_pcm_run_pair *runs, int n_pairs, Pairs &pairs)
{
    for (int p = 0; p < n_pairs; p++) {
        const uint32_t rows = runs[p].a_rows < runs[p].b_rows ? runs[p].a_rows : runs[p].b_rows;
        pairs.push_back(mp3s_pcm_pair{0, 0, (uint32_t)(((uint64_t)rows + 1151) / 1152), 0});
    }
}

constexpr int kPcmBatchThreads = 256;
struct PcmBatchTile { uint32_t item, first; };
template <class Tiles>
bool pcm_batch_tiles(int n_items, int64_t T, Tiles &tiles)
{
    if (n_items <= 0 || T <= 0 || T > ((int64_t)1 << 40)) return false;
    const uint64_t groups = ((uint64_t)T + 6) / 8 + 1, per = (groups + kPcmBatchThreads - 1) / kPcmBatchThreads;
    if ((uint64_t)tiles.size() + per * (uint64_t)n_items > 0x7fffffffu) return false;
    for (int i = 0; i < n_items; i++)
        for (uint64_t f = 0; f < per; f++) tiles.push_back(PcmBatchTile{(uint32_t)i, (uint32_t)f});
    return true;
}
template <class Tiles>
bool pcm_unbatch_tiles(const mp3s_pcm_unbatch_item *items, int n_items, Tiles &tiles)
{
    uint64_t n = tiles.size();
    for (int i = 0; i < n_items; i++) {
        if (items[i].n_rows < 1 || items[i].n_rows > ((int64_t)1 << 40)) return false;
        n += (((uint64_t)items[i].n_rows + 1151) / 1152 * 288 + kPcmBatchThreads - 1) / kPcmBatchThreads;
    }
    if (n > 0x7fffffffu) return false;
    for (int i = 0; i < n_items; i++) {
        const uint64_t per = (((uint64_t)items[i].n_rows + 1151) / 1152 * 288 + kPcmBatchThreads - 1) / kPcmBatchThreads;
        for (uint64_t f = 0; f < per; f++) tiles.push_back(PcmBatchTile{(uint32_t)i, (uint32_t)f});
    }
    return true;
}
inline bool pcm_batch_items_ok(const mp3s_pcm_batch_item *items, int n_items)
{
    for (int i = 0; i < n_items; i++)
        if (items[i].src_row < 0 || items[i].n_rows < 0 || items[i].first_row < 0 || items[i].slot < 0 || items[i].src_row > INT64_MAX / 4 - items[i].first_row) return false;
    return true;
}
inline bool pcm_unbatch_items_ok(const mp3s_pcm_unbatch_item *items, int n_items, int64_t T)
{
    for (int i = 0; i < n_items; i++)
        if (items[i].dst_frame < 0 || items[i].dst_frame > 0x7fffffff || items[i].n_rows < 1 || items[i].n_rows > T || items[i].slot < 0) return false;
    return true;
}
int launch_pcm_batch(hipStream_t stream, const int16_t *d_pcm, int nch, const mp3s_pcm_batch_item *d_items, const PcmBatchTile *d_tiles, int n_tiles,
                     int out_channels, int out_format, int64_t T, void *d_out);
int launch_pcm_unbatch(hipStream_t stream, const void *d_in, int in_channels, int in_format, int64_t T, const mp3s_pcm_unbatch_item *d_items,
                       const PcmBatchTile *d_tiles, int n_tiles, int16_t *d_pcm);

struct WavRun { uint64_t src; uint32_t first_frame, n_frames; };
struct WavImportRun { uint64_t src, n_samples; uint32_t first_frame, n_frames, format, channels; };
constexpr size_t kWavSlack = 64;
struct WavResampleRun { const uint32_t *taps; uint64_t src_row, n_in, n_out; uint32_t first_frame, n_frames, L, M, T, span, mono, taps_lds; };
constexpr int kResTile = 1024;
constexpr uint32_t kResTapsLds = 2048;
inline uint32_t resample_span(uint32_t L, uint32_t M, uint32_t T) { return (uint32_t)(((uint64_t)(kResTile - 1) * M + L - 1) / L) + T; }
int launch_wav_resample(hipStream_t stream, const uint32_t *d_rows, const WavResampleRun *d_runs, int n_runs, int max_frames ,
                        size_t lds_bytes , int16_t *d_pcm, Profiler *prof);
struct PcmResampleRun { const uint32_t *taps; int64_t src_row, n_in, n_out, first_row; uint32_t L, M, T, span, taps_lds, mono; int32_t slot; uint32_t pad; };
constexpr int kPcmResGroups = 128, kPcmResRows = 8 * kPcmResGroups + 8;
inline uint32_t pcm_resample_span(uint32_t L, uint32_t M, uint32_t T) { return T ? (uint32_t)(((uint64_t)(kPcmResRows - 1) * M + L - 1) / L) + T : (uint32_t)kPcmResRows; }
inline size_t pcm_resample_lds(const PcmResampleRun &r) { return ((size_t)kPcmResRows + r.span + (r.taps_lds ? (size_t)r.L * (r.T / 2) : 0)) * 4; }
template <class Tiles>
bool pcm_resample_tiles(int n_items, int64_t T, Tiles &tiles)
{
    if (n_items <= 0 || T <= 0 || T > ((int64_t)1 << 40)) return false;
    const uint64_t groups = ((uint64_t)T + 6) / 8 + 1, per = (groups + kPcmResGroups - 1) / kPcmResGroups;
    if ((uint64_t)tiles.size() + per * (uint64_t)n_items > 0x7fffffffu) return false;
    for (int i = 0; i < n_items; i++)
        for (uint64_t f = 0; f < per; f++) tiles.push_back(PcmBatchTile{(uint32_t)i, (uint32_t)f});
    return true;
}
int launch_pcm_batch_resample(hipStream_t stream, const int16_t *d_pcm, int nch, const PcmResampleRun *d_runs, const PcmBatchTile *d_tiles, int n_tiles,
                              size_t lds_bytes, int out_channels, int out_format, int64_t T, void *d_out);
int launch_wav_import(hipStream_t stream, const uint8_t *d_image, const WavImportRun *d_runs, int n_runs, int max_frames , int16_t *d_pcm);
int launch_wav_gather(hipStream_t stream, const uint8_t *d_image, const WavRun *d_runs, int n_runs, int max_frames , int16_t *d_pcm);

struct PlaceEntry { int32_t frame; int32_t pad[3]; int16_t is[2304]; mp3s_granule_si si[4]; };
static_assert(sizeof(PlaceEntry) == 4912 && offsetof(PlaceEntry, is) == 16 && offsetof(PlaceEntry, si) == 16 + 4608, "k_place_frames copies dwords from byte 16 on");
template <class Decode>
static inline bool fill_place_entry(PlaceEntry &e, int32_t frame, Decode &&decode) { e.frame = frame; e.pad[0] = e.pad[1] = e.pad[2] = 0; return decode(e.is, e.si); }
int launch_place_frames(hipStream_t stream, const uint8_t *d_entries, int n_entries, int16_t *d_is, mp3s_granule_si *d_si);
int launch_copy(hipStream_t stream, const void *d_src, void *d_dst, size_t bytes);
int launch_spin(hipStream_t stream, int microseconds);
int launch_noop(hipStream_t stream);

int launch_huffman(hipStream_t stream, const uint8_t *d_blob, const mp3s_frame_side *d_side, int n_frames, int nch, int max_bits,
                   int16_t *d_is, mp3s_granule_si *d_si, int32_t *d_status, int32_t *d_sync ,
                   Profiler *prof,
                   bool per_frame = false ,
                   int lanes_opt = 0 );
int launch_gather_tables(hipStream_t stream, const mp3s_gr_out *d_outv, int n, uint8_t *d_tables);
int launch_scatter(hipStream_t stream, const int32_t *d_pairs, int n_pairs, const int16_t *d_ixv, const int32_t *d_env,
                   const mp3s_gr_out *d_outv, int16_t *d_ix, int32_t *d_en, mp3s_gr_out *d_out);
int launch_pack(hipStream_t stream, const int16_t *d_ix, const mp3s_gr_out *d_gr, const int32_t *d_en, int n_frames, int sri,
                int bri, int whole_slots, const uint32_t *d_frame_off, const uint8_t *d_padding, uint8_t *d_mp3,
                int32_t *d_scfsi, int32_t *d_status, int32_t *d_sync , Profiler *prof,
                int f_begin = 0, int f_end = -1 );

}
```

mp3-steganography-lib_amd/csrc/mp3s_device.hip:

```cpp
#include <hip/hip_runtime.h>
#include <hip/hip_ext.h>
#include <atomic>
#include <stdint.h>
#include <stdlib.h>

#include "../../include/mp3s.h"
#include "mp3s_device.h"
#include "mp3s_host.h"
#include "mp3s_tables.h"
#include "analysis_sign_plan.h"

namespace mp3s {
__constant__ DevTables c_tab;
__constant__ __attribute__((aligned(64))) int32_t c_fl_sign[ANALYSIS_SIGN_STREAM];
}

#include "k_wave.hpp"
#include "k_sync.hpp"
#include "k_decode.hpp"
#include "k_decode_stream.hpp"
#include "k_encode.hpp"
#include "k_rate.hpp"
#include "k_huffman.hpp"
#include "k_parse.hpp"
#include "k_reveal.hpp"
#include "k_capacity.hpp"
#include "k_table_audit.hpp"
#include "k_pcmdiff.hpp"
#include "k_pcmalign.hpp"
#include "k_pcmbatch.hpp"
#include "k_pack.hpp"
#include "k_chain.hpp"
#include "k_wav.hpp"
#include "k_resample.hpp"
#include "k_pcmresample.hpp"

namespace mp3s {

int Profiler::take(int k)
{
    if (!enabled || !((mask >> k) & 1u)) return -1;
    if (n_pairs >= MAX_PAIRS) { dropped++; return -1; }
    while (n_created < 2 * (n_pairs + 1)) {
        if (hipEventCreate(&ev[n_created]) != hipSuccess) { dropped++; return -1; }
        n_created++;
    }
    kid[n_pairs] = k;
    return n_pairs++;
}
int Profiler::begin(hipStream_t s, int k)
{
    const int pair = take(k);
    if (pair >= 0) (void)hipEventRecord(ev[2 * pair], s);
    return pair;
}
void Profiler::end(hipStream_t s, int pair)
{
    if (pair >= 0) (void)hipEventRecord(ev[2 * pair + 1], s);
}
bool Profiler::attach(int k, hipEvent_t *start, hipEvent_t *stop)
{
    const int pair = take(k);
    if (pair < 0) return false;
    *start = ev[2 * pair]; *stop = ev[2 * pair + 1];
    return true;
}

int dev_upload_tables(hipStream_t stream)
{
    const HostTables &h = host_tables();
    hipError_t e = hipMemcpyToSymbolAsync(HIP_SYMBOL(c_tab), &h.dev, sizeof(DevTables), 0, hipMemcpyHostToDevice, stream);
    if (e != hipSuccess) return (int)e;
    static_assert(sizeof h.fl_sign == sizeof(int32_t) * ANALYSIS_SIGN_STREAM, "the coefficient stream and its symbol");
    e = hipMemcpyToSymbolAsync(HIP_SYMBOL(c_fl_sign), h.fl_sign, sizeof h.fl_sign, 0, hipMemcpyHostToDevice, stream);
    if (e != hipSuccess) return (int)e;
    return (int)hipStreamSynchronize(stream);
}

static size_t dec_S_bytes(int n_frames, int nch) { return (size_t)nch * (size_t)n_frames * 36 * 32 * sizeof(double); }
static size_t dec_G_bytes(int n_frames) { return (size_t)n_frames * 2 * 2 * sizeof(double); }
size_t dec_scratch_bytes(int n_frames, int nch)
{
    return dec_S_bytes(n_frames, nch) + dec_G_bytes(n_frames) + (size_t)nch * (size_t)n_frames * 36 * sizeof(uint2);
}

static int dec_run_length(int n_gran, int r_min, int r_max, long slots, double priming)
{
    int run = r_max; double best = 1e30;
    for (int r = r_min; r <= r_max; r++) {
        const long waves = (n_gran + r - 1) / r;
        const long rounds = (waves + slots - 1) / slots;
        const double cost = (double)rounds * (r + priming);
        if (cost < best) { best = cost; run = r; }
    }
    return run;
}

static void launch_dec_fixup(hipStream_t stream, hipEvent_t done, const int16_t *d_is, const mp3s_granule_si *d_si, const mp3s_frame_hdr *d_hdr,
                             int n_gran, int nch, long T, int n_halo, int sf_base, void *d_pcm, const uint2 *fix_list, int32_t *d_sync)
{
    const int fix_groups = (int)((T * nch + DEC_A_WAVES - 1) / DEC_A_WAVES) < 128 ? (int)((T * nch + DEC_A_WAVES - 1) / DEC_A_WAVES) : 128;
    if (done)
        hipExtLaunchKernelGGL(k_dec_fixup, dim3(fix_groups), dim3(DEC_A_WAVES * 64), 0, stream, nullptr, done, 0, d_is, d_si, d_hdr, n_gran, nch, T, n_halo,
                              sf_base, (int16_t *)d_pcm, fix_list, d_sync + 6, d_sync + 2);
    else
        hipLaunchKernelGGL(k_dec_fixup, dim3(fix_groups), dim3(DEC_A_WAVES * 64), 0, stream, d_is, d_si, d_hdr, n_gran, nch, T, n_halo,
                           sf_base, (int16_t *)d_pcm, fix_list, d_sync + 6, d_sync + 2);
}

int launch_decode(hipStream_t stream, const int16_t *d_is, const mp3s_granule_si *d_si, const mp3s_frame_hdr *d_hdr,
                  int n_frames, int nch, int n_halo, int out_format, void *d_pcm, void *d_scratch, Profiler *prof, const DecodeHow &how)
{
    const int sf_base = how.sf_base; int32_t *const d_sync = how.d_sync; hipEvent_t done = how.done;
    const long T = (long)n_frames * 36;
    double *S = (double *)d_scratch;
    double *G = (double *)((char *)d_scratch + dec_S_bytes(n_frames, nch));
    uint2 *fix_list = (uint2 *)((char *)G + dec_G_bytes(n_frames));
    const int n_gran = n_frames * 2;
    const bool fast = out_format == MP3S_PCM_I16 && how.eps_scale > 0 && d_sync;
    const bool fast32 = out_format == MP3S_PCM_F32 && how.float_fast;
    const bool streamed = how.fused && ((fast && how.fast_imdct) || fast32);
    const int run = streamed ? dec_run_length(n_gran, 4, 16, 2048, 1.6) : dec_run_length(n_gran, 2, 8, 3072, 0.55);
    const int runs = (n_gran + run - 1) / run;
    const double eps = fast ? how.eps_scale : 1.0;
    uint2 *const fix = fast ? fix_list : nullptr;
    int32_t *const fix_count = fast ? d_sync + 6 : nullptr;
    int pp;
    if (streamed) {
        const bool probing = !fast32 && how.probe && how.probe->x;
        auto *const kernel = fast32 ? (nch == 2 ? k_dec_stream<2, true> : k_dec_stream<1, true>)
                           : probing ? (nch == 2 ? k_dec_stream<2, false, true> : k_dec_stream<1, false, true>)
                                     : (nch == 2 ? k_dec_stream<2, false> : k_dec_stream<1, false>);
        pp = prof ? prof->begin(stream, K_DEC_SYNTH) : -1;
        hipLaunchKernelGGL(kernel, dim3((runs + ST_WAVES - 1) / ST_WAVES), dim3(ST_WAVES * 64), 0, stream, d_is, d_si, d_hdr, n_gran, run, n_halo, d_pcm, sf_base, eps, fix, fix_count,
                           probing ? how.probe->x : (double *)nullptr, probing ? how.probe->eps : (double *)nullptr, probing ? (long)how.probe->base : 0L,
                           probing ? (long)how.probe->cap : 0L);
        if (!fast32) {
            launch_dec_fixup(stream, done, d_is, d_si, d_hdr, n_gran, nch, T, n_halo, sf_base, d_pcm, fix_list, d_sync);
            done = nullptr;
        }
    } else {
        pp = prof ? prof->begin(stream, K_DEC_IMDCT) : -1;
        const bool mirrored = (fast && how.fast_imdct) || fast32;
        hipLaunchKernelGGL(mirrored ? k_dec_imdct<true> : k_dec_imdct<false>, dim3((runs + DEC_A_WAVES - 1) / DEC_A_WAVES), dim3(DEC_A_WAVES * 64), 0, stream,
                           d_is, d_si, d_hdr, n_gran, nch, run, S, T, sf_base, mirrored && !fast32 ? G : (double *)nullptr);
        if (prof) prof->end(stream, pp);
        constexpr int TW = DEC_SYNTH_TW, W = DEC_SYNTH_FAST_TW;
        pp = prof ? prof->begin(stream, K_DEC_SYNTH) : -1;
        if (fast32 || fast) {
            hipLaunchKernelGGL((fast32 ? k_dec_synth_fast<W, true> : k_dec_synth_fast<W>), dim3((unsigned)((T + (W * 64 - 15) - 1) / (W * 64 - 15))), dim3(W * 64 * nch), 0, stream,
                               (const double *)S, T, d_hdr, nch, n_halo, (int16_t *)d_pcm, sf_base, eps, mirrored && !fast32 ? (const double *)G : nullptr, n_gran, fix, fix_count);
            if (!fast32) launch_dec_fixup(stream, nullptr, d_is, d_si, d_hdr, n_gran, nch, T, n_halo, sf_base, d_pcm, fix_list, d_sync);
        } else {
            const int tiles = (int)((T + (TW * 64 - 15) - 1) / (TW * 64 - 15));
            hipLaunchKernelGGL(k_dec_synth<TW>, dim3(tiles), dim3(TW * 64 * nch), 0, stream, (const double *)S, T, d_hdr, nch, n_halo, out_format, d_pcm, sf_base);
        }
    }
    if (prof) prof->end(stream, pp);
    if (done && hipEventRecord(done, stream) != hipSuccess) return (int)hipErrorUnknown;
    return (int)hipGetLastError();
}

size_t enc_scratch_bytes(int n_frames)
{
    return (size_t)2 * 32 * (size_t)n_frames * 36 * sizeof(int32_t);
}

int launch_encode(hipStream_t stream, const int16_t *d_pcm, const mp3s_frame_hdr *d_hdr, int n_frames, int32_t *d_mdct,
                  void *d_scratch, Profiler *prof, bool fused, bool analysis_shared)
{
    if (fused) {
        const long n_gran = (long)n_frames * 2;
        const int pf = prof ? prof->begin(stream, K_ENC_ANALYSIS) : -1;
        hipLaunchKernelGGL(k_enc_fused, dim3((unsigned)((n_gran + EF_GR - 1) / EF_GR)), dim3(EF_WAVES * 64), 0, stream, d_pcm, d_hdr, n_frames, d_mdct, (int)analysis_shared);
        if (prof) prof->end(stream, pf);
        return (int)hipGetLastError();
    }
    const long Ts = (long)n_frames * 36;
    int32_t *SB = (int32_t *)d_scratch;
    const long waves = 2 * ((Ts + 63) / 64);
    int pp = prof ? prof->begin(stream, K_ENC_ANALYSIS) : -1;
    hipLaunchKernelGGL(k_enc_analysis, dim3((unsigned)((waves + 3) / 4)), dim3(256), 0, stream, d_pcm, d_hdr, n_frames, SB,
                       Ts, (int)analysis_shared);
    if (prof) prof->end(stream, pp);
    pp = prof ? prof->begin(stream, K_ENC_MDCT) : -1;
    hipLaunchKernelGGL(k_enc_mdct, dim3((n_frames + 3) / 4), dim3(256), 0, stream, (const int32_t *)SB, Ts, d_hdr, n_frames,
                       d_mdct);
    if (prof) prof->end(stream, pp);
    return (int)hipGetLastError();
}

int launch_rate(hipStream_t stream, const int32_t *d_mdct, const mp3s_rate_frame *d_frames, int n_frames,
                const uint8_t *d_hide, int n_hide, const int32_t *d_cursor, const int32_t *d_state,
                const int32_t *d_list, int n_list, int16_t *d_ix, mp3s_gr_out *d_out, int32_t *d_en, Profiler *prof, int out_base, int compact,
                const RateVariantArgs *variants, hipEvent_t done)
{
    const int n_units = n_frames * 4;
    if (compact && !d_list) return (int)hipErrorInvalidValue;
    const int n = d_list ? n_list : n_units;
    RateVariants var = {nullptr, nullptr, 0, nullptr, nullptr, nullptr, nullptr};
    if (variants && variants->n > 0) var = RateVariants{variants->d_unit, variants->d_cursor, variants->n, variants->d_ix, variants->d_out, variants->d_en, variants->d_tables};
    if (n + var.n <= 0) return done ? (int)hipEventRecord(done, stream) : 0;
    hipEvent_t t_start = nullptr, t_stop = nullptr;
    const bool timed = prof && prof->attach(K_RATE_LOOP, &t_start, &t_stop);
    if (timed || done)
        hipExtLaunchKernelGGL(k_rate_loop, dim3((n + var.n + RL_WAVES - 1) / RL_WAVES), dim3(RL_WAVES * 64), 0, stream, timed ? t_start : nullptr, timed ? t_stop : done, 0,
                              d_mdct, d_frames, n_units, d_hide, n_hide, d_cursor, d_state, d_list, n, d_ix, d_out, d_en, out_base, compact, var);
    else
        hipLaunchKernelGGL(k_rate_loop, dim3((n + var.n + RL_WAVES - 1) / RL_WAVES), dim3(RL_WAVES * 64), 0, stream, d_mdct, d_frames,
                           n_units, d_hide, n_hide, d_cursor, d_state, d_list, n, d_ix, d_out, d_en, out_base, compact, var);
    if (timed && done && hipEventRecord(done, stream) != hipSuccess) return (int)hipErrorUnknown;
    return (int)hipGetLastError();
}

static size_t chain_scan_bytes(int n_frames) { return ((size_t)((n_frames + CH_THREADS - 1) / CH_THREADS) * sizeof(ChainEl) + 31) & ~(size_t)15; }
constexpr int kRedoRounds = 1;
size_t chain_agg_bytes(int n_frames) { return chain_scan_bytes(n_frames) + (size_t)2 * REDO_WORDS * 4; }

int launch_chain(hipStream_t stream, mp3s_gr_out *d_gr, const mp3s_rate_frame *d_frames, int n_frames, const mp3s_chain_seg *d_segs,
                 const int32_t *d_cursor, const int32_t *d_state, void *d_agg, int32_t *d_verdict, mp3s_chain_seg_out *d_seg_out,
                 Profiler *prof, const ChainRedoArgs *redo)
{
    if (n_frames <= 0) return 0;
    const int blocks = (n_frames + CH_THREADS - 1) / CH_THREADS;
    int32_t *d_redo = redo ? (int32_t *)((uint8_t *)d_agg + chain_scan_bytes(n_frames)) : nullptr;
    int32_t *cursor = const_cast<int32_t *>(d_cursor);
    const int pp = prof ? prof->begin(stream, K_CHAIN) : -1;
    hipLaunchKernelGGL(k_chain_sum, dim3(blocks), dim3(CH_THREADS), 0, stream, (const mp3s_gr_out *)d_gr, d_frames, d_segs, n_frames,
                       (ChainEl *)d_agg, d_verdict, d_seg_out, d_redo, (const int32_t *)nullptr);
    hipLaunchKernelGGL(k_chain_apply, dim3(blocks), dim3(CH_THREADS), 0, stream, d_gr, d_frames, d_segs, n_frames,
                       (const ChainEl *)d_agg, cursor, d_state, d_verdict, d_seg_out, d_redo, (const int32_t *)nullptr);
    if (redo) {
        int32_t *lists[2] = {d_redo, d_redo + REDO_WORDS};
        for (int round = 0; round < kRedoRounds; round++) {
            const int32_t *cur = lists[round & 1];
            int32_t *nxt = round + 1 < kRedoRounds ? lists[(round + 1) & 1] : nullptr;
            hipLaunchKernelGGL(k_rate_redo, dim3(REDO_GROUPS), dim3(RL_WAVES * 64), 0, stream, redo->d_mdct, d_frames, n_frames * 4,
                               redo->d_hide, redo->n_hide, cur, redo->d_ix, d_gr, redo->d_en, (const int32_t *)d_cursor);
            hipLaunchKernelGGL(k_chain_sum, dim3(blocks), dim3(CH_THREADS), 0, stream, (const mp3s_gr_out *)d_gr, d_frames, d_segs, n_frames,
                               (ChainEl *)d_agg, d_verdict, d_seg_out, nxt, cur);
            hipLaunchKernelGGL(k_chain_apply, dim3(blocks), dim3(CH_THREADS), 0, stream, d_gr, d_frames, d_segs, n_frames,
                               (const ChainEl *)d_agg, cursor, d_state, d_verdict, d_seg_out, nxt, cur);
        }
    }
    if (prof) prof->end(stream, pp);
    return (int)hipGetLastError();
}

int launch_select(hipStream_t stream, const mp3s_chain_seg *d_segs, const mp3s_select_span *d_spans, int n_segs, int max_reach,
                  const uint8_t *d_hide, const RateVariantArgs &v, int16_t *d_ix, int32_t *d_en, mp3s_gr_out *d_out, int32_t *d_cursor,
                  void *d_pairs, Profiler *prof)
{
    if (n_segs <= 0 || max_reach <= 0 || v.n <= 0) return 0;
    if (max_reach > MP3S_SELECT_MAX_REACH || (int64_t)n_segs * max_reach > 0x3fffffff) return (int)hipErrorInvalidValue;
    const int pp = prof ? prof->begin(stream, K_CHAIN) : -1;
    hipLaunchKernelGGL(k_chain_select, dim3(n_segs), dim3(SEL_THREADS), select_lds_bytes(max_reach), stream, d_segs, d_spans, max_reach,
                       d_hide, (const uint8_t *)v.d_tables, (const mp3s_gr_out *)d_out, d_cursor, (int2 *)d_pairs);
    const int n_pairs = n_segs * max_reach;
    hipLaunchKernelGGL(k_scatter_entries, dim3((n_pairs + 3) / 4), dim3(256), 0, stream, (const int2 *)d_pairs, n_pairs,
                       (const int16_t *)v.d_ix, (const int32_t *)v.d_en, (const mp3s_gr_out *)v.d_out, d_ix, d_en, d_out);
    if (prof) prof->end(stream, pp);
    return (int)hipGetLastError();
}

int launch_gather_tables(hipStream_t stream, const mp3s_gr_out *d_outv, int n, uint8_t *d_tables)
{
    if (n <= 0) return 0;
    hipLaunchKernelGGL(k_gather_tables, dim3((n + 255) / 256), dim3(256), 0, stream, d_outv, n, d_tables);
    return (int)hipGetLastError();
}

int launch_scatter(hipStream_t stream, const int32_t *d_pairs, int n_pairs, const int16_t *d_ixv, const int32_t *d_env,
                   const mp3s_gr_out *d_outv, int16_t *d_ix, int32_t *d_en, mp3s_gr_out *d_out)
{
    if (n_pairs <= 0) return 0;
    hipLaunchKernelGGL(k_scatter_entries, dim3((n_pairs + 3) / 4), dim3(256), 0, stream, (const int2 *)d_pairs, n_pairs, d_ixv, d_env,
                       d_outv, d_ix, d_en, d_out);
    return (int)hipGetLastError();
}

int launch_huffman(hipStream_t stream, const uint8_t *d_blob, const mp3s_frame_side *d_side, int n_frames, int nch, int max_bits,
                   int16_t *d_is, mp3s_granule_si *d_si, int32_t *d_status, int32_t *d_sync, Profiler *prof, bool per_frame, int lanes_opt)
{
    const long units = (long)n_frames * 4;
    const int W = huf_words_for(max_bits);
    int dev = 0;
    (void)hipGetDevice(&dev);
    const int dslot = dev >= 0 && dev < 64 ? dev : 0;
    static std::atomic<int> lds_of_device[64];
    int lds_max = lds_of_device[dslot].load(std::memory_order_relaxed);
    if (lds_max == 0) {
        if (hipDeviceGetAttribute(&lds_max, hipDeviceAttributeMaxSharedMemoryPerBlock, dev) != hipSuccess || lds_max < 64 * 1024) lds_max = 64 * 1024;
        lds_of_device[dslot].store(lds_max, std::memory_order_relaxed);
    }
    const size_t kLdsMax = (size_t)lds_max;
    auto dyn = [&](int cols, int wv) { return ((size_t)(W + 17) * cols + 17 * wv) * 4; };
    auto fits = [&](int cols) { return dyn(cols, 8) + HUF_TAB_N * 2 + 256 <= kLdsMax; };
    int lanes = 16, waves = 4;
    if (fits(128)) { lanes = 32; waves = 4; }
    if (fits(256) && units > 32 * 1024) { lanes = 64; waves = 4; }
    if (lanes_opt > 0) {
        const int a = lanes_opt;
        if (a == 64 && fits(256)) { lanes = 64; waves = 4; }
        if (a == 62 && fits(128)) { lanes = 64; waves = 2; }
        if (a == 32 && fits(128)) { lanes = 32; waves = 4; }
        if (a == 16) { lanes = 16; waves = 4; }
        if (a == 8) { lanes = 8; waves = 8; }
    }
    static const bool trace = getenv("MP3S_TRACE") != nullptr;
    if (trace) fprintf(stderr, "[mp3s] huffman launch: %ld units, W %d, %d waves x %d lanes, %zu bytes of dynamic LDS\n", units, W, waves, lanes, dyn(waves * lanes, waves));
    const int pp = prof ? prof->begin(stream, K_DEC_HUFFMAN) : -1;
#define MP3S_HUF_LAUNCH(WV, LN)                                                                                         \
    do {                                                                                                                \
        static std::atomic<unsigned long long> asked{0};                                                              \
        if (!(asked.load(std::memory_order_relaxed) & (1ull << dslot))) {                                               \
            (void)hipFuncSetAttribute(reinterpret_cast<const void *>(&k_dec_huffman<WV, LN>), hipFuncAttributeMaxDynamicSharedMemorySize, \
                                      (int)(kLdsMax - HUF_TAB_N * 2 - 256));                                            \
            asked.fetch_or(1ull << dslot, std::memory_order_relaxed);                                                   \
        }                                                                                                               \
        hipLaunchKernelGGL((k_dec_huffman<WV, LN>), dim3((unsigned)((units + WV * LN - 1) / (WV * LN))), dim3(WV * 64), \
                           dyn(WV * LN, WV), stream, d_blob, d_side, n_frames, nch, W, max_bits, d_is, d_si, d_status, per_frame ? 1 : 0, d_sync); \
    } while (0)
    if (lanes == 64 && waves == 4) MP3S_HUF_LAUNCH(4, 64);
    else if (lanes == 64) MP3S_HUF_LAUNCH(2, 64);
    else if (lanes == 32) MP3S_HUF_LAUNCH(4, 32);
    else if (lanes == 8) MP3S_HUF_LAUNCH(8, 8);
    else MP3S_HUF_LAUNCH(4, 16);
#undef MP3S_HUF_LAUNCH
    if (prof) prof->end(stream, pp);
    return (int)hipGetLastError();
}

static_assert(sizeof(ParseFrameRef) == sizeof(FrameRef) && sizeof(ParseStreamRef) == sizeof(StreamRef), "frame / stream references out of sync with mp3s_host.h");

int launch_parse(hipStream_t stream, const uint8_t *d_image, uint32_t image_base, const FrameRef *d_refs, const StreamRef *d_streams, int n_frames,
                 uint32_t md_base, mp3s_frame_side *d_side, mp3s_frame_hdr *d_hdr, uint8_t *d_blob, uint64_t *d_tsel, int32_t *d_status)
{
    if (n_frames <= 0) return 0;
    hipLaunchKernelGGL(k_dec_parse, dim3((n_frames + PARSE_WAVES - 1) / PARSE_WAVES), dim3(PARSE_WAVES * 64), 0, stream, d_image, image_base,
                       reinterpret_cast<const ParseFrameRef *>(d_refs), reinterpret_cast<const ParseStreamRef *>(d_streams), n_frames, md_base, d_side,
                       d_hdr, d_blob, d_tsel, d_status);
    return (int)hipGetLastError();
}

static_assert(REVEAL_TILE == kRevealTile && REVEAL_BAD_REF == kRevealBadRef, "k_reveal's constants out of sync with mp3s_device.h");

int launch_reveal(hipStream_t stream, const uint8_t *d_image, uint32_t image_base, const FrameRef *d_refs, const StreamRef *d_streams, int n_streams,
                  const uint32_t *d_out_off, uint8_t *d_packed, int32_t *d_n_bits, int32_t *d_status)
{
    if (n_streams <= 0) return 0;
    if (n_streams > kRevealMaxStreams) return (int)hipErrorInvalidValue;
    const HostTables &HT = host_tables();
    uint32_t h0_mask = 0;
    for (int t = 0; t < 32; t++) if (HT.in_h0[t]) h0_mask |= 1u << t;
    hipLaunchKernelGGL(k_reveal, dim3((unsigned)n_streams), dim3(REVEAL_TILE), 0, stream, d_image, image_base, reinterpret_cast<const ParseFrameRef *>(d_refs),
                       reinterpret_cast<const ParseStreamRef *>(d_streams), d_out_off, h0_mask, d_packed, d_n_bits, d_status);
    return (int)hipGetLastError();
}

int launch_capacity(hipStream_t stream, const mp3s_gr_out *d_gr, const mp3s_chain_seg *d_segs, int n_segs, mp3s_capacity_seg *d_out, uint32_t *d_profile)
{
    if (n_segs <= 0) return 0;
    hipLaunchKernelGGL(k_capacity, dim3((unsigned)n_segs), dim3(CAP_TILE), 0, stream, d_gr, d_segs, d_out, d_profile);
    return (int)hipGetLastError();
}

int launch_table_audit(hipStream_t stream, const int16_t *d_is, const mp3s_frame_side *d_side, int n_frames, int nch, const mp3s_table_audit_seg *d_segs,
                       int n_segs, mp3s_table_audit_unit *d_units, mp3s_table_audit *d_out, uint32_t *d_profile)
{
    if (n_frames <= 0 || n_segs <= 0) return 0;
    if ((nch != 1 && nch != 2) || ((uintptr_t)d_is & 3) || ((uintptr_t)d_units & 15)) return (int)hipErrorInvalidValue;
    hipLaunchKernelGGL(k_table_audit_units, dim3((unsigned)n_frames), dim3(256), 0, stream, d_is, d_side, nch, d_units);
    if (const hipError_t e = hipGetLastError()) return (int)e;
    hipLaunchKernelGGL(k_table_audit_streams, dim3((unsigned)n_segs), dim3(TA_TILE), 0, stream, d_units, d_segs, nch, d_out, d_profile);
    return (int)hipGetLastError();
}

int launch_pcm_diff(hipStream_t stream, const int16_t *d_pcm, int nch, const mp3s_pcm_pair *d_pairs, int n_pairs, const PcmTile *d_tiles, int n_tiles,
                    mp3s_pcm_frame_diff *d_frames, mp3s_pcm_pair_diff *d_out)
{
    if (n_pairs <= 0) return 0;
    if ((nch != 1 && nch != 2) || ((uintptr_t)d_pcm & 15)) return (int)hipErrorInvalidValue;
    if (n_tiles > 0) {
        if (nch == 2) hipLaunchKernelGGL(k_pcm_diff_frames<2>, dim3((unsigned)n_tiles), dim3(PCMDIFF_WAVES * 64), 0, stream, d_pcm, d_pairs, d_tiles, d_frames);
        else hipLaunchKernelGGL(k_pcm_diff_frames<1>, dim3((unsigned)n_tiles), dim3(PCMDIFF_WAVES * 64), 0, stream, d_pcm, d_pairs, d_tiles, d_frames);
        if (const hipError_t e = hipGetLastError()) return (int)e;
    }
    hipLaunchKernelGGL(k_pcm_diff_pairs, dim3((unsigned)n_pairs), dim3(PCMDIFF_TILE), 0, stream, d_pairs, d_frames, nch, d_out);
    return (int)hipGetLastError();
}

int launch_pcm_align(hipStream_t stream, const int16_t *d_pcm, int nch, const mp3s_pcm_run_pair *d_runs, int n_pairs, int max_lag, int search_rows,
                     const int32_t *d_given, const PcmTile *d_tiles, int n_tiles, uint64_t *d_scores, mp3s_pcm_lag *d_lags, mp3s_pcm_pair *d_geo,
                     mp3s_pcm_frame_diff *d_frames, mp3s_pcm_pair_diff *d_out)
{
    if (n_pairs <= 0) return 0;
    if ((nch != 1 && nch != 2) || ((uintptr_t)d_pcm & 15) || max_lag < 0 || max_lag > kPcmMaxLag || search_rows < 1) return (int)hipErrorInvalidValue;
    if (!d_given) {
        const int tiles_per_pair = (2 * max_lag + 1 + PCMALIGN_LAGS - 1) / PCMALIGN_LAGS;
        if ((uint64_t)n_pairs * (uint64_t)tiles_per_pair > 0x7fffffffu) return (int)hipErrorInvalidValue;
        const dim3 grid((unsigned)n_pairs * (unsigned)tiles_per_pair);
        if (nch == 2) hipLaunchKernelGGL(k_pcm_lag_scores<2>, grid, dim3(64), 0, stream, d_pcm, d_runs, max_lag, search_rows, tiles_per_pair, d_scores);
        else hipLaunchKernelGGL(k_pcm_lag_scores<1>, grid, dim3(64), 0, stream, d_pcm, d_runs, max_lag, search_rows, tiles_per_pair, d_scores);
        if (const hipError_t e = hipGetLastError()) return (int)e;
    }
    hipLaunchKernelGGL(k_pcm_lag_pick, dim3((unsigned)n_pairs), dim3(PCMALIGN_PICK), 0, stream, d_runs, d_scores, d_given, max_lag, search_rows, d_lags, d_geo);
    if (const hipError_t e = hipGetLastError()) return (int)e;
    if (n_tiles > 0) {
        if (nch == 2) hipLaunchKernelGGL(k_pcm_diff_lagged<2>, dim3((unsigned)n_tiles), dim3(PCMDIFF_WAVES * 64), 0, stream, d_pcm, d_geo, d_lags, d_tiles, d_frames);
        else hipLaunchKernelGGL(k_pcm_diff_lagged<1>, dim3((unsigned)n_tiles), dim3(PCMDIFF_WAVES * 64), 0, stream, d_pcm, d_geo, d_lags, d_tiles, d_frames);
        if (const hipError_t e = hipGetLastError()) return (int)e;
    }
    hipLaunchKernelGGL(k_pcm_diff_pairs, dim3((unsigned)n_pairs), dim3(PCMDIFF_TILE), 0, stream, d_geo, d_frames, nch, d_out);
    return (int)hipGetLastError();
}

int launch_pcm_batch(hipStream_t stream, const int16_t *d_pcm, int nch, const mp3s_pcm_batch_item *d_items, const PcmBatchTile *d_tiles, int n_tiles,
                     int out_channels, int out_format, int64_t T, void *d_out)
{
    if (n_tiles <= 0) return 0;
    const bool f32 = out_format == MP3S_BATCH_F32;
    if ((nch != 1 && nch != 2) || (out_channels != 1 && out_channels != 2) || (!f32 && out_format != MP3S_BATCH_I16) || T <= 0 ||
        ((uintptr_t)d_pcm & (uintptr_t)(2 * nch - 1)) || ((uintptr_t)d_out & (uintptr_t)(f32 ? 3 : 1)))
        return (int)hipErrorInvalidValue;
#define PCM_BATCH_LAUNCH(N, C, F) hipLaunchKernelGGL((k_pcm_batch<N, C, F>), dim3((unsigned)n_tiles), dim3(PCMBATCH_THREADS), 0, stream, d_pcm, d_items, d_tiles, T, (uint8_t *)d_out)
    switch ((nch - 1) * 4 + (out_channels - 1) * 2 + (f32 ? 1 : 0)) {
    case 0: PCM_BATCH_LAUNCH(1, 1, false); break;
    case 1: PCM_BATCH_LAUNCH(1, 1, true); break;
    case 2: PCM_BATCH_LAUNCH(1, 2, false); break;
    case 3: PCM_BATCH_LAUNCH(1, 2, true); break;
    case 4: PCM_BATCH_LAUNCH(2, 1, false); break;
    case 5: PCM_BATCH_LAUNCH(2, 1, true); break;
    case 6: PCM_BATCH_LAUNCH(2, 2, false); break;
    default: PCM_BATCH_LAUNCH(2, 2, true); break;
    }
#undef PCM_BATCH_LAUNCH
    return (int)hipGetLastError();
}

int launch_pcm_unbatch(hipStream_t stream, const void *d_in, int in_channels, int in_format, int64_t T, const mp3s_pcm_unbatch_item *d_items,
                       const PcmBatchTile *d_tiles, int n_tiles, int16_t *d_pcm)
{
    if (n_tiles <= 0) return 0;
    const bool f32 = in_format == MP3S_BATCH_F32;
    if ((in_channels != 1 && in_channels != 2) || (!f32 && in_format != MP3S_BATCH_I16) || T <= 0 || ((uintptr_t)d_pcm & 15) ||
        ((uintptr_t)d_in & (uintptr_t)(f32 ? 3 : 1)))
        return (int)hipErrorInvalidValue;
#define PCM_UNBATCH_LAUNCH(C, F) hipLaunchKernelGGL((k_pcm_unbatch<C, F>), dim3((unsigned)n_tiles), dim3(PCMBATCH_THREADS), 0, stream, (const uint8_t *)d_in, d_items, d_tiles, T, d_pcm)
    if (in_channels == 1) { if (f32) PCM_UNBATCH_LAUNCH(1, true); else PCM_UNBATCH_LAUNCH(1, false); }
    else { if (f32) PCM_UNBATCH_LAUNCH(2, true); else PCM_UNBATCH_LAUNCH(2, false); }
#undef PCM_UNBATCH_LAUNCH
    return (int)hipGetLastError();
}

__global__ __launch_bounds__(256) void k_place_frames(const uint8_t *__restrict__ entries, int n_entries, int16_t *__restrict__ is,
                                                      mp3s_granule_si *__restrict__ si)
{
    const uint8_t *e = entries + (size_t)blockIdx.x * sizeof(PlaceEntry);
    const int f = *reinterpret_cast<const int32_t *>(e);
    const uint32_t *src = reinterpret_cast<const uint32_t *>(e + 16);
    uint32_t *d_is = reinterpret_cast<uint32_t *>(is + (size_t)f * 2304), *d_si = reinterpret_cast<uint32_t *>(si + (size_t)f * 4);
    for (int i = threadIdx.x; i < 1152; i += 256) d_is[i] = src[i];
    for (int i = threadIdx.x; i < 72; i += 256) d_si[i] = src[1152 + i];
}
int launch_place_frames(hipStream_t stream, const uint8_t *d_entries, int n_entries, int16_t *d_is, mp3s_granule_si *d_si)
{
    if (n_entries <= 0) return 0;
    hipLaunchKernelGGL(k_place_frames, dim3(n_entries), dim3(256), 0, stream, d_entries, n_entries, d_is, d_si);
    return (int)hipGetLastError();
}

__global__ void k_spin(long long ticks, int *sink)
{
    const long long t0 = wall_clock64();
    int it = 0;
    while (wall_clock64() - t0 < ticks && it < (1 << 22)) it++;
    if (sink && it < 0) *sink = it;
}
__global__ void k_noop() {}
int launch_spin(hipStream_t stream, int microseconds)
{
    hipLaunchKernelGGL(k_spin, dim3(1), dim3(64), 0, stream, (long long)microseconds * 100, (int *)nullptr);
    return (int)hipGetLastError();
}
int launch_noop(hipStream_t stream)
{
    hipLaunchKernelGGL(k_noop, dim3(1), dim3(64), 0, stream);
    return (int)hipGetLastError();
}

// ... 83 lines not shown
```

mp3-steganography-lib_amd/csrc/mp3s_internal.h:

```cpp
#pragma once
#include <hip/hip_runtime_api.h>

#include <algorithm>
#include <array>
#include <atomic>
#include <chrono>
#include <cstdarg>
#include <cstddef>
#include <cstdio>
#include <cstdlib>
#include <cstring>
#include <functional>
#include <memory>
#include <mutex>
#include <string>
#include <thread>
#include <type_traits>
#include <vector>

#include "../../include/mp3s.h"
#include "mp3s_device.h"
#include "mp3s_host.h"

namespace mp3s {
int fail(int code, const char *fmt, ...) __attribute__((format(printf, 2, 3)));
}

using namespace mp3s;

#define HIPCHK(call)                                                                                 \
    do {                                                                                             \
        hipError_t e_ = (call);                                                                      \
        if (e_ != hipSuccess) return fail(MP3S_E_HIP, "%s: %s", #call, hipGetErrorString(e_));       \
    } while (0)

enum PoolSlot : int {
    kPoolIs0, kPoolSi0,
    kPoolFrameHdr, kPoolPcmChunk, kPoolHufStatus, kPoolMainData, kPoolSideInfo,
    kPoolPcm0,
    kPoolPcmUp,
    kPoolInputs,
    kPoolMdct,
    kPoolRedo,
    kPoolIx, kPoolGrOut, kPoolEnergy,
    kPoolChainAgg,
    kPoolMp3, kPoolScfsi,
    kPoolSmall,
    kPoolVarEntries, kPoolVarIx, kPoolVarOut, kPoolVarEnergy, kPoolVarPairs,
    kPoolIs1, kPoolSi1, kPoolPcm1,
    kPoolWavImage, kPoolResampleRows,
    kPoolSelectDev,
    kPoolChainDev,
    kPoolReveal,
    kPoolSlotCount
};
constexpr PoolSlot kPoolIs[2] = {kPoolIs0, kPoolIs1}, kPoolSi[2] = {kPoolSi0, kPoolSi1}, kPoolPcm[2] = {kPoolPcm0, kPoolPcm1};

struct mp3s_pipe;
struct ChainResolver;
struct mp3s_ctx {
    int device = 0;
    int64_t opt[MP3S_OPT_COUNT] = {0};
    mp3s_run_stats run_stats = {0, 0, 0, 0, 0};
    mp3s_pipe *own_pipe = nullptr;
    std::vector<mp3s_pipe *> parked_pipes;
    int sink_fd = -1; size_t sink_done = 0, sink_base = 0; bool sink_early = false;
    hipStream_t stream = nullptr;
    hipEvent_t ev0 = nullptr, ev1 = nullptr, ev_order = nullptr;
    hipEvent_t ev_sel = nullptr; bool sel_pending = false;
    int32_t *d_sync = nullptr;
    double synth_eps_scale = 1.0;
    GuardProbe guard_probe = {nullptr, nullptr, 0, 0};
    void *scratch = nullptr, *scratch_enc = nullptr; size_t scratch_bytes = 0, scratch_enc_bytes = 0;
    Profiler prof;
    static constexpr int kPoolSlots = 32;
    struct ResampleTaps { int L, M, T; uint32_t *d; };
    std::vector<ResampleTaps> res_taps;
    void *pool[kPoolSlots] = {nullptr};
    size_t pool_bytes[kPoolSlots] = {0};
    void *grab(PoolSlot slot, size_t bytes, hipStream_t user = nullptr )
    {
        if (slot < 0 || slot >= kPoolSlots) return nullptr;
        if (bytes < 16) bytes = 16;
        if (pool_bytes[slot] >= bytes) return pool[slot];
        if (pool[slot]) { hipStreamSynchronize(user ? user : stream); hipFree(pool[slot]); pool[slot] = nullptr; pool_bytes[slot] = 0; }
        const size_t want = bytes + bytes / 4;
        if (hipMalloc(&pool[slot], want) != hipSuccess) { pool[slot] = nullptr; return nullptr; }
        pool_bytes[slot] = want;
        return pool[slot];
    }
    ChainResolver *chain = nullptr;
    std::vector<uint8_t> h_in;
    std::vector<mp3s_frame_hdr> h_hdr;
    std::vector<mp3s_frame_side> h_side;
    std::vector<uint8_t> h_blob;
    ScannedStream spare_scan;
    std::vector<FrameRef> h_refs;
    std::vector<uint8_t> h_tables;
    std::vector<PcmTile> h_pcm_tiles;
    hipEvent_t ev_pcm_tiles = nullptr;
    std::vector<uint8_t> h_pcm_align;
    std::vector<uint8_t> h_pcm_batch;
    static int ensure(void *&buf, size_t &have, size_t bytes)
    {
        if (bytes <= have) return 0;
        if (buf) { hipFree(buf); buf = nullptr; have = 0; }
        hipError_t e = hipMalloc(&buf, bytes);
        if (e != hipSuccess) return fail(MP3S_E_NOMEM, "hipMalloc(%zu) for scratch: %s", bytes, hipGetErrorString(e));
        have = bytes;
        return 0;
    }
    int ensure_scratch(size_t bytes) { return ensure(scratch, scratch_bytes, bytes); }
    int ensure_scratch_enc(size_t bytes) { return ensure(scratch_enc, scratch_enc_bytes, bytes); }
};
static_assert(kPoolSlotCount <= mp3s_ctx::kPoolSlots, "every PoolSlot needs a place in mp3s_ctx::pool");

inline int guard_probe_usable(const mp3s_ctx *c, int out_format)
{
    if (!c->guard_probe.x || out_format != MP3S_PCM_I16) return MP3S_OK;
    if (c->opt[MP3S_OPT_FUSED_DECODE] && c->opt[MP3S_OPT_FAST_IMDCT] && c->synth_eps_scale > 0 && c->d_sync) return MP3S_OK;
    return fail(MP3S_E_ARG, "the guard probe is set (mp3s_debug_guard_margin) and this int16 decode would not run the stream kernel that fills it "
                            "(MP3S_OPT_FUSED_DECODE / MP3S_OPT_FAST_IMDCT off, or the guard's scale is 0)");
}

inline DecodeHow decode_how(mp3s_ctx *c, int sf_base, hipEvent_t done, int64_t probe_base)
{
    if (c->guard_probe.x) c->guard_probe.base = probe_base;
    return {sf_base, c->synth_eps_scale, c->d_sync, c->opt[MP3S_OPT_FAST_IMDCT] != 0, c->opt[MP3S_OPT_FLOAT_FAST] != 0, c->opt[MP3S_OPT_FUSED_DECODE] != 0,
            done, c->guard_probe.x ? &c->guard_probe : nullptr};
}

int local_world_size();

class PinnedBlock {
public:
    PinnedBlock() = default;
    PinnedBlock(const PinnedBlock &) = delete;
    PinnedBlock &operator=(const PinnedBlock &) = delete;
    ~PinnedBlock() { release(); }
    bool reserve(size_t bytes)
    {
        if (bytes <= cap_) return true;
        release();
        if (bytes > kMaxPinned) {
            p_ = (uint8_t *)std::malloc(bytes);
            if (!p_) return false;
            cap_ = bytes; pinned_ = false;
            return true;
        }
        pinned_ = true;
        {
            std::lock_guard<std::mutex> g(mu());
            auto &fl = free_list();
            size_t best = fl.size();
            const size_t too_big = std::max(4 * bytes, bytes + ((size_t)1 << 20));
            for (size_t i = 0; i < fl.size(); i++)
                if (fl[i].second >= bytes && fl[i].second <= too_big && (best == fl.size() || fl[i].second < fl[best].second)) best = i;
            if (best < fl.size()) { p_ = fl[best].first; cap_ = fl[best].second; fl.erase(fl.begin() + best); return true; }
        }
        const size_t want = bytes + bytes / 8 + (1 << 16);
        void *q = nullptr;
        if (hipHostMalloc(&q, want, hipHostMallocDefault) != hipSuccess) return false;
        p_ = (uint8_t *)q; cap_ = want;
        return true;
    }
    uint8_t *data() const { return p_; }
    static void pool_state(size_t *held, size_t *cap)
    {
        std::lock_guard<std::mutex> g(mu());
        size_t h = 0;
        for (auto &e : free_list()) h += e.second;
        *held = h; *cap = pool_cap();
    }

private:
    void release()
    {
        if (!p_) return;
        if (!pinned_) { std::free(p_); p_ = nullptr; cap_ = 0; return; }
        std::lock_guard<std::mutex> g(mu());
        auto &fl = free_list();
        size_t held = 0;
        for (auto &e : fl) held += e.second;
        if (fl.size() < 48 && held + cap_ <= pool_cap()) fl.emplace_back(p_, cap_);
        else hipHostFree(p_);
        p_ = nullptr; cap_ = 0;
    }
    static std::mutex &mu() { static std::mutex *m = new std::mutex(); return *m; }
    static std::vector<std::pair<uint8_t *, size_t>> &free_list()
    {
        static auto *v = new std::vector<std::pair<uint8_t *, size_t>>();
        return *v;
    }
    static constexpr size_t kMaxPinned = (size_t)4 << 30;
    static size_t pool_cap()
    {
        static const size_t cap = std::max<size_t>((size_t)1 << 30, kMaxPinned / (size_t)local_world_size());
        return cap;
    }
    uint8_t *p_ = nullptr;
    size_t cap_ = 0;
    bool pinned_ = true;
};

struct mp3s_multi {
    std::vector<std::pair<const uint8_t *, size_t>> files;
    std::vector<ParsedStream> parsed;
    std::vector<ScannedStream> scanned;
    PinnedBlock arena[3];
    size_t head_room = 0;
    std::vector<const uint8_t *> pcm;
    struct Window { long first, count; bool keep_dup; };
    std::vector<Window> window;
    std::vector<std::vector<uint8_t>> all_bits;
    const StreamIndex *index = nullptr;
};

struct mp3s_buf {
    std::shared_ptr<mp3s_multi> multi;
    ParsedStream parsed;
    ScannedStream scanned;
    std::vector<uint8_t> bytes;
    std::vector<uint8_t> bits;
    std::vector<FrameRef> refs;
    std::vector<int32_t> scfsi;
    std::vector<std::unique_ptr<mp3s_buf>> parts;
    std::vector<std::vector<uint8_t>> lists;
    PinnedBlock big[3];
    uint8_t *mp3 = nullptr;
    mp3s_gr_out *gr_out = nullptr;
};

inline bool trace_on() { static const bool on = getenv("MP3S_TRACE") != nullptr; return on; }
inline double now_ms() { return std::chrono::duration<double, std::milli>(std::chrono::steady_clock::now().time_since_epoch()).count(); }


inline size_t up16(size_t x) { return (x + 15) & ~(size_t)15; }

inline int file_workers(int n, size_t total_bytes, int max_threads)
{
    return (int)std::min<size_t>({(size_t)n, (size_t)max_threads, total_bytes / (256u << 10) + 1});
}
inline int host_threads16() { const unsigned hw = std::thread::hardware_concurrency(); return (int)std::min(hw ? hw : 1u, 16u); }
template <class F>
void parallel_files(int workers, int n, F f)
{
    if (workers <= 1) {
        for (int i = 0; i < n; i++) f(0, i);
        return;
    }
    std::atomic<int> next{0};
    auto run = [&](int w) { for (int i; (i = next.fetch_add(1)) < n;) f(w, i); };
    std::vector<std::thread> pool;
    for (int w = 1; w < workers; w++) pool.emplace_back(run, w);
    run(0);
    for (auto &t : pool) t.join();
}

long walk_whole(const uint8_t *file, size_t len, std::vector<FrameRef> &refs, FrameWalker &w, std::vector<uint8_t> *tables = nullptr,
                long tables_wanted = 0);

struct EncSeg;
void file_from_seg(const EncSeg &seg, const uint8_t *mp3_base, int kbps, int rate, int64_t hide_offset, mp3s_file *out);

struct FileGroups {
    struct Group { int a, b; std::vector<int> idx; };
    std::vector<Group> groups;
    void add(int a, int b, int i)
    {
        size_t g = 0;
        while (g < groups.size() && (groups[g].a != a || groups[g].b != b)) g++;
        if (g == groups.size()) groups.push_back({a, b, {}});
        groups[g].idx.push_back(i);
    }
};

struct FileStatus {
    std::vector<int32_t> st;
    std::vector<std::string> why;
    explicit FileStatus(int n) : st((size_t)n, MP3S_OK), why((size_t)n) {}
    void set(int i, int code) { st[(size_t)i] = code; if (code) why[(size_t)i] = mp3s_last_error(); }
};
int front_end_failed(int code, int i);
int finish_files(const FileStatus &fs, int32_t *status);
int finish_list(const FileStatus &fs, int32_t *status, std::unique_ptr<mp3s_buf> &top, mp3s_buf **owner);

struct mp3s_multi;
std::vector<int32_t> mp3_list_front(mp3s_ctx *c, mp3s_multi &m, int n_files, const std::function<std::pair<const uint8_t *, size_t>(int)> &file_of);
void mp3_list_done(mp3s_ctx *c, mp3s_multi &m);
void reencode_list_front(mp3s_ctx *c, mp3s_multi &m, const uint8_t *const *mp3s, const size_t *lens, int n_files, const uint8_t *const *msgs,
                         const size_t *msg_lens, FileStatus &fs, std::vector<std::vector<uint8_t>> &bits, FileGroups &groups, double *t_scanned = nullptr);

template <class Run, class After>
void run_groups(const FileGroups &groups, Run run, FileStatus &fs, After after_failure)
{
    for (const FileGroups::Group &g : groups.groups) {
        const int rc = run(g.a, g.b, g.idx);
        if (!rc) continue;
        if (g.idx.size() == 1) fs.set(g.idx[0], rc);
        after_failure();
        if (g.idx.size() > 1)
            for (int i : g.idx) fs.set(i, run(g.a, g.b, std::vector<int>{i}));
    }
}

constexpr int kDecodeChunk = 16384;
inline size_t pcm_elem(int fmt) { return fmt == MP3S_PCM_I16 ? 2 : (fmt == MP3S_PCM_F32 ? 4 : 8); }
int max_part2_3(const mp3s_frame_side *side, long n);
void cut_window(ParsedStream &p, ScannedStream &sc, long first, long count);
int front_end(mp3s_multi &m, int i);
int decode_transform_chunk(mp3s_ctx *c, const int16_t *d_is, const mp3s_granule_si *d_si, const mp3s_frame_hdr *d_hdr, long first, int cnt,
                           int nch, int halo, int out_format, void *d_pcm, hipStream_t stream = nullptr ,
                           hipEvent_t done = nullptr );
struct DecodeFront {
    long n = 0;
    std::vector<long> first_of;
    void *d_is = nullptr, *d_si = nullptr, *d_hdr = nullptr, *d_pcm = nullptr, *d_st = nullptr, *d_blob = nullptr, *d_side = nullptr;
};
int decode_front(mp3s_ctx *c, mp3s_multi &m, const std::vector<int> &idx, int nch, size_t frame_bytes, DecodeFront &F);
int decode_group(mp3s_ctx *c, mp3s_multi &m, const std::vector<int> &idx, int nch, int out_format, void *d_keep = nullptr);

inline int64_t pcm_frames(const ParsedStream &p) { return (int64_t)p.n_frames + (p.dup_last_frame ? 1 : 0); }
void distortion_from_record(const mp3s_pcm_pair_diff &r, const ParsedStream &a, const ParsedStream &b, int64_t n_frames, int64_t n_samples,
                            const mp3s_pcm_frame_diff *profile, mp3s_pcm_distortion *out);
struct PcmPairBatch {
    std::vector<int> streams;
    std::vector<int64_t> first, frames_a, frames_b;
    std::vector<int64_t> out_first;
    int64_t rows_frames = 0, cmp_frames = 0;
    std::unique_ptr<mp3s_buf> part;
    const uint8_t *res = nullptr;
    int lay(const mp3s_multi &m, int n_pairs, const std::vector<int> &idx, int64_t max_frames);
    int run(mp3s_ctx *c, mp3s_multi &m, int nch, const uint8_t *in, size_t in_bytes, size_t res_bytes, size_t down_bytes,
            const std::function<int(const int16_t *d_pcm, const uint8_t *d_in, uint8_t *d_res)> &launch);
private:
    int n_pairs = 0;
    const std::vector<int> *idx = nullptr;
};
int pcm_pairs_call(mp3s_ctx *c, const uint8_t *const *a, const size_t *a_lens, const uint8_t *const *b, const size_t *b_lens, int n_pairs, void *out,
                   size_t out_size, mp3s_buf **owner, int32_t *status, const std::function<void(const mp3s_multi &m, int i)> &empty,
                   const std::function<bool(const mp3s_multi &m, FileStatus &fs, int i)> &refuse,
                   const std::function<int(mp3s_multi &m, const std::vector<int> &idx, int nch, mp3s_buf *top)> &group);
int pcm_dev_host_block(mp3s_ctx *c, const std::function<int()> &fill_and_copy);

constexpr int kLongMessageBits = 1024;
constexpr int32_t kNoCursor = MP3S_NO_CURSOR;
constexpr int kPatternBytes = 32;
constexpr int kVariantEntries = 65536;
constexpr size_t kFewUnits = 8;

struct EncSeg {
    int n_frames = 0;
    const uint8_t *hide = nullptr;
    int n_hide = 0;
    int lead = 0;
    int64_t first_frame = 0;
    bool last = true;
    const mp3s_carry *carry_in = nullptr;
    const uint8_t *tables_guess = nullptr;
    int n_guess = -1;
    int any_silent = -1;
    int first = 0, hide_base = 0;
    int reach = 0, first_entry = 0;
    int64_t hide_offset = 0;
    size_t mp3_off = 0, mp3_len = 0;
// ... 181 lines not shown
```

mp3-steganography-lib_amd/csrc/mp3s_tables.cpp:

```cpp
#include "mp3s_tables.h"
#include "iso_tables.h"
#include "analysis_plan.h"
#include "analysis_sign_plan.h"

#include <algorithm>
#include <cmath>
#include <cstdio>
#include <cstdlib>
#include <cstring>
#include <functional>
#include <mutex>

namespace mp3s {

namespace {

double round_decimals(double x, int nd)
{
    char buf[64];
    std::snprintf(buf, sizeof buf, "%.*f", nd, x);
    return std::strtod(buf, nullptr);
}

const int kSfbLong[3][23] = {
    {0, 4, 8, 12, 16, 20, 24, 30, 36, 44, 52, 62, 74, 90, 110, 134, 162, 196, 238, 288, 342, 418, 576},
    {0, 4, 8, 12, 16, 20, 24, 30, 36, 42, 50, 60, 72, 88, 106, 128, 156, 190, 230, 276, 330, 384, 576},
    {0, 4, 8, 12, 16, 20, 24, 30, 36, 44, 54, 66, 82, 102, 126, 156, 194, 240, 296, 364, 448, 550, 576}};
const int kSfbShortW[3][12] = {{4, 4, 4, 4, 6, 8, 10, 12, 14, 18, 22, 30},
                               {4, 4, 4, 4, 6, 6, 10, 12, 14, 16, 20, 26},
                               {4, 4, 4, 4, 6, 8, 12, 16, 20, 26, 34, 42}};
const int kPreTab[21] = {0, 0, 0, 0, 0, 0, 0, 0, 0, 0, 0, 1, 1, 1, 1, 2, 2, 3, 3, 3, 2};
const int kSlen[16][2] = {{0, 0}, {0, 1}, {0, 2}, {0, 3}, {3, 0}, {1, 1}, {1, 2}, {1, 3},
                          {2, 1}, {2, 2}, {2, 3}, {3, 1}, {3, 2}, {3, 3}, {4, 2}, {4, 3}};
const int kSubdv[23][2] = {{0, 0}, {0, 0}, {0, 0}, {0, 0}, {0, 0}, {0, 1}, {1, 1}, {1, 1}, {1, 2}, {2, 2}, {2, 3}, {2, 3},
                           {3, 4}, {3, 4}, {3, 4}, {4, 5}, {4, 5}, {4, 6}, {5, 6}, {5, 6}, {5, 7}, {6, 7}, {6, 7}};
const double kAliasC[8] = {-0.6, -0.535, -0.33, -0.185, -0.095, -0.041, -0.0142, -0.0037};
const uint8_t kTransform[32][2] = {
    {0, 0},   {3, 1},   {3, 2},   {3, 2},   {0, 0},   {6, 5},   {6, 5},   {8, 7},   {8, 7},   {8, 9},   {11, 10},
    {11, 10}, {12, 10}, {15, 13}, {0, 0},   {15, 13}, {17, 16}, {17, 18}, {19, 18}, {19, 20}, {21, 20}, {21, 22},
    {23, 22}, {23, 31}, {24, 25}, {26, 25}, {26, 27}, {28, 27}, {28, 29}, {30, 29}, {30, 31}, {23, 31}};
const int kH0[14] = {3, 6, 8, 11, 12, 15, 17, 19, 21, 23, 24, 26, 28, 30};

HostTables g_tables;
std::once_flag g_once;

void set_huff(int n, int xl, int yl, int lb, int lm, const uint16_t *c, const uint8_t *l)
{
    g_tables.huff[n] = HostHuff{xl, yl, lb, lm, c, l};
}

void build_rq_map(int sr, int cse, uint8_t *map)
{
    const int *short_win = kSfbShortW[sr];
    const int *long_win = kSfbLong[sr];
    const bool bt2 = cse == 1, mixed = cse == 2;
    int window = 0, sfb = 0, i = 0;
    for (int sample = 0; sample < 576; sample++, i++) {
        bool sh;
        if (bt2 || (mixed && sfb >= 8)) {
            int swv = sfb < 12 ? short_win[sfb] : 0;
            if (i == swv) {
                i = 0;
                if (window == 2) { window = 0; sfb += 1; } else window += 1;
            }
            sh = true;
        } else {
            if (sample == long_win[sfb + 1]) sfb += 1;
            sh = false;
        }
        const int slot = sh ? 22 + 13 * window + (sfb < 13 ? sfb : 12) : (sfb < 22 ? sfb : 21);
        map[sample] = (uint8_t)(((sh ? 1 + window : 0) << 6) | slot);
    }
}

void build()
{
    HostTables &H = g_tables;
    DevTables &T = H.dev;
    std::memset(&H, 0, sizeof H);
    const double kPi = 3.141592653589793;

    for (int i = 0; i < 512; i++) {
        T.synth_window[i] = round_decimals((double)ISO_WINDOW_NUM[i] / 65536.0, 9);
        T.synth_window_t[i & 31][i >> 5] = T.synth_window[i];
        T.enwindow[i] = (int32_t)(round_decimals((double)ISO_WINDOW_NUM[i] / 2097152.0, 6) * 2147483647.0);
    }
    for (int i = 0; i < 64; i++)
        for (int j = 0; j < 32; j++) T.synth_matrix[i][j] = std::cos((16.0 + i) * (2.0 * j + 1.0) * (kPi / 64.0));
    for (int i = 0; i < 36; i++)
        for (int k = 0; k < 18; k++)
            T.imdct_cos36[i][k] = std::cos(kPi / (double)(2 * 36) * (double)(2 * i + 1 + 18) * (double)(2 * k + 1));
    for (int i = 0; i < 12; i++)
        for (int k = 0; k < 6; k++)
            T.imdct_cos12[i][k] = std::cos(kPi / (double)(2 * 12) * (double)(2 * i + 1 + 6) * (double)(2 * k + 1));
    for (int i = 0; i < 36; i++) T.sine_block[0][i] = std::sin(kPi / 36.0 * (i + 0.5));
    for (int i = 0; i < 18; i++) T.sine_block[1][i] = std::sin(kPi / 36.0 * (i + 0.5));
    for (int i = 18; i < 24; i++) T.sine_block[1][i] = 1.0;
    for (int i = 24; i < 30; i++) T.sine_block[1][i] = std::sin(kPi / 12.0 * (i - 18.0 + 0.5));
    for (int i = 30; i < 36; i++) T.sine_block[1][i] = 1.0;
    for (int i = 0; i < 12; i++) T.sine_block[2][i] = std::sin(kPi / 12.0 * (i + 0.5));
    for (int i = 6; i < 12; i++) T.sine_block[3][i] = std::sin(kPi / 12.0 * (i - 6.0 + 0.5));
    for (int i = 12; i < 18; i++) T.sine_block[3][i] = 1.0;
    for (int i = 18; i < 36; i++) T.sine_block[3][i] = std::sin(kPi / 36.0 * (i + 0.5));
    for (int i = 0; i < 8; i++) {
        const double c = kAliasC[i];
        T.alias_cs[i] = round_decimals(1.0 / std::sqrt(1.0 + c * c), 10);
        T.alias_ca[i] = round_decimals(c / std::sqrt(1.0 + c * c), 10);
        T.mdct_ca[i] = (int32_t)(c / std::sqrt(1.0 + (c * c)) * 2147483647.0);
        T.mdct_cs[i] = (int32_t)(1.0 / std::sqrt(1.0 + (c * c)) * 2147483647.0);
    }
    for (int i = 0; i < POW43_N; i++) T.pow43[i] = std::pow((double)i, 4.0 / 3.0);
    for (int i = 0; i < POW2Q_N; i++) T.pow2q[i] = std::pow(2.0, (double)(i + POW2Q_MIN) / 4.0);
    for (int i = 0; i < POW2H_N; i++) T.pow2h[i] = std::pow(2.0, -((double)i * 0.5));
    T.sqrt2 = std::sqrt(2.0);
    {
        int o = 0;
        for (int n = 32; n >= 2; n >>= 1)
            for (int m = 0; m < n / 2; m++)
                for (int j = 0; j < n / 2; j++)
                    T.synth_fast[o++] = std::cos((double)((2 * j + 1) * (2 * m + 1)) * (kPi / (2.0 * n)));
        const double u = 1.1102230246251565e-16;
        long double dN = 0;
        const long double pil = 3.14159265358979323846264338327950288L;
        for (int i = 0; i < 64; i++)
            for (int j = 0; j < 32; j++) {
                const long double c = cosl((long double)((16 + i) * (2 * j + 1)) * pil / 64.0L);
                const long double d = fabsl((long double)T.synth_matrix[i][j] - c);
                if (d > dN) dN = d;
            }
        double dsum = 0;
        for (int i = 0; i < 32; i++) {
            double a = 0;
            for (int k = 0; k < 16; k++) a += std::fabs(T.synth_window[32 * k + i]);
            if (a > dsum) dsum = a;
        }
        const double g33 = 33 * u / (1 - 33 * u), g24 = 24 * u / (1 - 24 * u), g18s = 18 * u / (1 - 18 * u);
        const double dV = (double)dN + 1e-19 + g33 + g24;
        T.synth_eps_a = 2.0 * 32767.0 * dsum * (dV + 2 * g18s * (1 + dV));
        long double dT = 0;
        for (int i = 0; i < 9; i++)
            for (int k = 0; k < 18; k++) {
                const long double a = fabsl((long double)T.imdct_cos36[i][k] + (long double)T.imdct_cos36[17 - i][k]);
                const long double b = fabsl((long double)T.imdct_cos36[18 + i][k] - (long double)T.imdct_cos36[35 - i][k]);
                if (a > dT) dT = a;
                if (b > dT) dT = b;
            }
        const double g18 = 18 * u / (1 - 18 * u);
        long double dC = 0;
        for (int i = 0; i < 36; i++)
            for (int k = 0; k < 18; k++) {
                const long double c = cosl((long double)((2 * i + 19) * (2 * k + 1)) * pil / 72.0L);
                const long double d = fabsl((long double)T.imdct_cos36[i][k] - c);
                if (d > dC) dC = d;
            }
        const double kappa_mirror = 2 * g18 + (double)dT + 4.2 * u, kappa_dct4 = g18 + (double)dC + 1e-19 + 22 * u + 4.2 * u;
        T.imdct_kappa = kappa_mirror > kappa_dct4 ? kappa_mirror : kappa_dct4;
        for (int k = 0; k < 9; k++) {
            T.imdct_rot[0][2 * k] = (double)cosl((long double)(2 * k + 1) * pil / 72.0L);
            T.imdct_rot[0][2 * k + 1] = (double)sinl((long double)(2 * k + 1) * pil / 72.0L);
        }
        for (int m = 0; m < 10; m++)
            for (int k = 0; k < 9; k++) {
                const int r = (m * (2 * k + 1)) % 36;
                T.imdct_pq[m][k] = m == 9 ? 0.0 : (double)cosl((long double)r * pil / 18.0L);
                T.imdct_pq[m][9 + k] = m == 0 ? 0.0 : (double)sinl((long double)r * pil / 18.0L);
            }
        T.synth_eps_g = 2.0 * 32767.0 * dsum * 2.0002 * T.imdct_kappa;
        T.synth_eps_x = 2.0 * 2 * u;
        for (int i = 0; i < 32; i++)
            for (int k = 0; k < 16; k++) {
                double w = T.synth_window_t[i][k];
                if (i == 0 && (k & 1)) w = -w;
                if (i == 16 && !(k & 1)) w = 0.0;
                if (i > 16 && !(k & 1)) w = -w;
                T.synth_window_f[i][k] = w;
                T.synth_window_fs[i][k] = w * 32767.0;
            }
        T.synth_xbound = 32767.0 * dsum * (1.0 + 1e-6);
        for (int v = 0; v < 2; v++)
            for (int t = 0; t < 8; t++) {
                double *q = T.synth_stream[v][t];
                const double (*W)[16] = v ? T.synth_window_fs : T.synth_window_f;
                const double *C32 = T.synth_fast, *C16 = T.synth_fast + 256, *C8 = T.synth_fast + 320, *C4 = T.synth_fast + 336;
                const int ka1 = 17 + 2 * t, kb1 = 15 - 2 * t, ka0 = 16 + 2 * t, kb0 = 16 - 2 * t;
                for (int j = 0; j < 16; j++) { q[j] = C32[(ka1 >> 1) * 16 + j]; q[16 + j] = C32[(kb1 >> 1) * 16 + j]; }
                if (t & 1) for (int j = 0; j < 8; j++) { q[32 + j] = C16[((ka0 - 2) >> 2) * 8 + j]; q[40 + j] = C16[((kb0 - 2) >> 2) * 8 + j]; }
                else if (t & 2) for (int j = 0; j < 4; j++) { q[32 + j] = C8[((ka0 - 4) >> 3) * 4 + j]; q[40 + j] = C8[((kb0 - 4) >> 3) * 4 + j]; }
                else if (t) for (int j = 0; j < 2; j++) { q[32 + j] = C4[((ka0 - 8) >> 4) * 2 + j]; q[40 + j] = C4[((kb0 - 8) >> 4) * 2 + j]; }
                const int oa = 2 * t, ob = t ? 32 - 2 * t : 16, oc = 2 * t + 1, od = 31 - 2 * t;
                if (t) for (int j = 0; j < 8; j++) { q[48 + j] = W[oa][j]; q[56 + j] = W[ob][j]; q[64 + j] = W[oa][8 + j]; q[72 + j] = W[ob][8 + j]; }
                else for (int j = 0; j < 16; j++) { q[48 + j] = W[oa][j]; q[64 + j] = W[ob][j]; }
                for (int j = 0; j < 8; j++) { q[80 + j] = W[oc][j]; q[88 + j] = W[od][j]; q[96 + j] = W[oc][8 + j]; q[104 + j] = W[od][8 + j]; }
            }
    }
    for (int sb = 0; sb < 32; sb++)
        for (int j = 0; j < 16; j++) {
            const int k = sb < 16 ? 2 * sb + 1 : 2 * (sb - 16);
            const int n = ((sb < 16 ? 2 * j + 1 : 31 - 2 * j) * k) % 128;
            T.stream_cx[sb][j] = (double)cosl((long double)n * 3.14159265358979323846264338327950288L / 64.0L);
            const double d = T.synth_window_t[sb][j];
            const double w = (j & 1) ? -d : (sb <= 15 ? d : (sb == 16 ? 0.0 : -d));
            T.stream_taps[0][sb][j] = w;
            T.stream_taps[1][sb][j] = w * 32767.0;
        }
    for (int sr = 0; sr < 3; sr++) {
        for (int c = 0; c < 3; c++) {
            uint8_t flat[576];
            build_rq_map(sr, c, flat);
            for (int sb = 0; sb < 32; sb++)
                for (int k = 0; k < 18; k++) T.rq_map[sr][c][sb][k] = flat[sb * 18 + k];
        }
        for (int i = 0; i < 576; i++) T.reorder_src[sr][i] = -1;
        int total = 0, start = 0, block = 0;
        for (int sb = 0; sb < 12; sb++) {
            const int w = kSfbShortW[sr][sb];
            for (int ss = 0; ss < w; ss++) {
                T.reorder_src[sr][start + block + 0] = (int16_t)(total + ss + w * 0);
                T.reorder_src[sr][start + block + 6] = (int16_t)(total + ss + w * 1);
                T.reorder_src[sr][start + block + 12] = (int16_t)(total + ss + w * 2);
                if (block != 0 && block % 5 == 0) { start += 18; block = 0; } else block += 1;
            }
            total += w * 3;
        }
        for (int i = 0; i < 23; i++) T.sfb_long[sr][i] = kSfbLong[sr][i];
        for (int i = 0; i < 12; i++) H.sfb_short_width[sr][i] = kSfbShortW[sr][i];
    }
    for (int sr = 0; sr < 3; sr++)
        for (int bv = 1; bv <= 288; bv++) {
            const int *sfb = kSfbLong[sr];
            const int bvr = 2 * bv;
            int anz = 0;
            while (sfb[anz] < bvr) anz++;
            int tc = kSubdv[anz][0];
            while (tc > 0) { if (sfb[tc + 1] <= bvr) break; tc--; }
            const int r0c = tc, a1 = sfb[tc + 1], base = tc + 1;
            tc = kSubdv[anz][1];
            while (tc > 0) { if (sfb[base + tc + 1] <= bvr) break; tc--; }
            const int r1c = tc, a2 = sfb[base + tc + 1];
            T.subdiv_lut[sr][bv] = (uint32_t)r0c | ((uint32_t)r1c << 4) | ((uint32_t)a1 << 8) | ((uint32_t)a2 << 18);
        }
    for (int i = 0; i < 21; i++) T.pre_tab[i] = (uint8_t)kPreTab[i];
    std::memcpy(H.slen, kSlen, sizeof kSlen);
    std::memcpy(T.subdv, kSubdv, sizeof kSubdv);
    std::memcpy(T.transform, kTransform, sizeof kTransform);
    for (int t : kH0) H.in_h0[t] = 1;

    for (int i = 0; i < 32; i++)
        for (int j = 0; j < 64; j++) {
            double f = 1e9 * std::cos((double)((2 * i + 1) * (16 - j)) * 0.049087385212), ip;
            if (f >= 0) std::modf(f + 0.5, &ip); else std::modf(f - 0.5, &ip);
            T.fl[i][j] = (int32_t)(ip * 2147483647.0 * 1e-9);
        }
    H.analysis_plan_ok = true;
    for (int p = 0; p < 8; p++)
        for (int k = 0; k < 64; k++) {
            const int o[4] = {p, 15 - p, 16 + p, 31 - p};
            unsigned word = 0;
            for (int j = 0; j < 4; j++) {
                int rep = j;
                for (int q = j - 1; q >= 0; q--) if (T.fl[o[q]][k] == T.fl[o[j]][k]) rep = q;
                word |= (unsigned)rep << (2 * j);
                if (T.fl[o[j]][k] == 0) word |= 1u << (8 + j);
            }
            if (word != ANALYSIS_PLAN[p][k]) H.analysis_plan_ok = false;
        }
    {
        static_assert(sizeof H.fl_sign == sizeof(int32_t) * ANALYSIS_SIGN_STREAM, "HostTables::fl_sign holds the plan's stream");
        uint8_t fed[32][64] = {};
        for (int p = 0; p < 8; p++) {
            const int o[4] = {p, 15 - p, 16 + p, 31 - p};
            for (int n = ANALYSIS_SIGN_FIRST[p]; n < ANALYSIS_SIGN_FIRST[p + 1]; n++) {
                const int k = ANALYSIS_SIGN_COL[n];
                const unsigned set = ANALYSIS_SIGN_SET[n];
                int32_t rep = 0;
                bool have = false;
                for (int j = 0; j < 4; j++) {
                    const unsigned f = (set >> (2 * j)) & 3u;
                    if (!f) continue;
                    const int32_t c = T.fl[o[j]][k];
                    if (!have) { rep = c; have = true; if (f != 1u) H.analysis_plan_ok = false; }
                    if (c == 0 || c == INT32_MIN || (int64_t)c != (f == 1u ? (int64_t)rep : -(int64_t)rep)) H.analysis_plan_ok = false;
                    fed[o[j]][k]++;
                }
                if (!have || rep != ANALYSIS_SIGN_COEF[n]) H.analysis_plan_ok = false;
                H.fl_sign[n] = rep;
            }
        }
        for (int i = 0; i < 32; i++)
            for (int k = 0; k < 64; k++)
                if (fed[i][k] != (T.fl[i][k] != 0 ? 1 : 0)) H.analysis_plan_ok = false;
    }
    for (int m = 0; m < 18; m++)
        for (int k = 0; k < 36; k++)
            T.cos_l[m][k] = (int32_t)(std::sin(0.087266462599717 * (k + 0.5)) *
                                      std::cos((3.14159265358979 / 72) * (double)(2 * k + 19) * (double)(2 * m + 1)) *
                                      2147483647.0);
    for (int i = 0; i < 128; i++) {
        T.steptab[i] = std::pow(2.0, (double)(127 - i) / 4);
        T.steptabi[i] = (T.steptab[i] * 2 > 2147483647.0) ? 0x7fffffff : (int32_t)(T.steptab[i] * 2 + 0.5);
    }
    for (int i = 0; i < 10000; i++)
        T.int2idx[i] = (uint16_t)(int32_t)(std::sqrt(std::sqrt((double)i) * (double)i) - 0.0946 + 0.5);
    {
        int l1 = 0, l2 = 0;
        while (l1 < 9999 && T.int2idx[l1] < 1) l1++;
        while (l2 < 9999 && T.int2idx[l2] < 2) l2++;
        auto at_least = [](int ln, uint32_t scalei) -> uint32_t {
            if (scalei == 0) return 0xffffffffu;
            const unsigned __int128 need = ((unsigned __int128)(uint32_t)ln << 32) - (1ull << 31);
            const unsigned __int128 a = (need + scalei - 1) / scalei;
            return a > 0x80000000ull ? 0xffffffffu : (uint32_t)a;
        };
        for (int i = 0; i < 128; i++) {
            const uint32_t sc = (uint32_t)T.steptabi[i];
            T.rl_t1[i] = at_least(l1, sc);
            T.rl_t2[i] = at_least(l2, sc);
            auto big = [&](uint64_t a) {
                const double dbl = (double)(uint32_t)a * T.steptab[i] * 4.656612875e-10;
                return (int32_t)std::sqrt(std::sqrt(dbl) * dbl) > 8192;
            };
            const uint64_t lo_ln = at_least(10000, sc);
            uint64_t lo = lo_ln, hi = 0x80000000ull;
            if (lo_ln == 0xffffffffu || !big(hi)) T.rl_t8[i] = 0xffffffffu;
            else {
                while (lo < hi) { const uint64_t mid = (lo + hi) / 2; if (big(mid)) hi = mid; else lo = mid + 1; }
                T.rl_t8[i] = (uint32_t)lo;
            }
        }
    }

    set_huff(0, 0, 0, 0, 0, nullptr, nullptr);
    set_huff(1, 2, 2, 0, 0, ISO_HCOD_1, ISO_HLEN_1);
    set_huff(2, 3, 3, 0, 0, ISO_HCOD_2, ISO_HLEN_2);
    set_huff(3, 3, 3, 0, 0, ISO_HCOD_3, ISO_HLEN_3);
    set_huff(4, 0, 0, 0, 0, nullptr, nullptr);
    set_huff(5, 4, 4, 0, 0, ISO_HCOD_5, ISO_HLEN_5);
    set_huff(6, 4, 4, 0, 0, ISO_HCOD_6, ISO_HLEN_6);
    set_huff(7, 6, 6, 0, 0, ISO_HCOD_7, ISO_HLEN_7);
    set_huff(8, 6, 6, 0, 0, ISO_HCOD_8, ISO_HLEN_8);
    set_huff(9, 6, 6, 0, 0, ISO_HCOD_9, ISO_HLEN_9);
    set_huff(10, 8, 8, 0, 0, ISO_HCOD_10, ISO_HLEN_10);
    set_huff(11, 8, 8, 0, 0, ISO_HCOD_11, ISO_HLEN_11);
    set_huff(12, 8, 8, 0, 0, ISO_HCOD_12, ISO_HLEN_12);
    set_huff(13, 16, 16, 0, 0, ISO_HCOD_13, ISO_HLEN_13);
    set_huff(14, 0, 0, 0, 0, nullptr, nullptr);
    set_huff(15, 16, 16, 0, 0, ISO_HCOD_15, ISO_HLEN_15);
    static const int lb16[8] = {1, 2, 3, 4, 6, 8, 10, 13}, lb24[8] = {4, 5, 6, 7, 8, 9, 11, 13};
    for (int k = 0; k < 8; k++) {
        set_huff(16 + k, 16, 16, lb16[k], (1 << lb16[k]) - 1, ISO_HCOD_16, ISO_HLEN_16);
        set_huff(24 + k, 16, 16, lb24[k], (1 << lb24[k]) - 1, ISO_HCOD_24, ISO_HLEN_24);
    }
    {
        auto en_of = [](int64_t e) { return (int32_t)(std::log((double)e * 4.768371584e-7) / 0.69314718); };
        for (int k = 0; k < 32; k++) { T.en_base[k] = 0; T.en_step[k] = 0x7fffffff; }
        for (int k = 0; k < 31; k++) {
            const int64_t lo = (int64_t)1 << k, hi = ((int64_t)1 << (k + 1)) - 1;
            T.en_base[k] = en_of(lo);
            if (en_of(hi) == T.en_base[k]) continue;
            if (en_of(hi) != T.en_base[k] + 1) abort();
            int64_t a = lo, b = hi;
            while (b - a > 1) { const int64_t m = (a + b) / 2; (en_of(m) == T.en_base[k] ? a : b) = m; }
            T.en_step[k] = (int32_t)b;
        }
    }

    set_huff(32, 1, 16, 0, 0, ISO_HCOD_32, ISO_HLEN_32);
    set_huff(33, 1, 16, 0, 0, ISO_HCOD_33, ISO_HLEN_33);
    for (int i = 0; i < 256; i++) {
        T.hlen13[i] = ISO_HLEN_13[i]; T.hlen15[i] = ISO_HLEN_15[i];
        T.hlen16[i] = ISO_HLEN_16[i]; T.hlen24[i] = ISO_HLEN_24[i];
    }
    for (int i = 0; i < 16; i++) T.hlen_c1a[i] = ISO_HLEN_32[i];
    for (int i = 0; i < 256; i++) {
        const uint32_t x = (uint32_t)i >> 4, y = (uint32_t)i & 15u, nz = (x != 0) + (y != 0), esc = (x == 15) + (y == 15);
        const uint32_t l13 = T.hlen13[i], l15 = T.hlen15[i], l16 = T.hlen16[i], l24 = T.hlen24[i];
        const uint32_t shortest = std::min(std::min(l13, l15), std::min(l16, l24)), longest = std::max(std::max(l13, l15), std::max(l16, l24));
        T.rl_hl[i][0] = l13 | (l15 << 5) | (l16 << 10) | (l24 << 15) | (nz << 20) | (esc << 22) | (i ? (shortest + nz) << 25 : 0u);
        T.rl_hl[i][1] = (i ? shortest + nz : 0u) | ((longest + nz + 13u * esc) << 16);
    }
    for (int i = 0; i < 16; i++) T.rl_c1w[i] = (uint32_t)T.hlen_c1a[i] | ((uint32_t)__builtin_popcount(i & 3) << 16);
    for (int i = 0; i < 32; i++) { T.linbits[i] = (uint8_t)H.huff[i].linbits; T.linmax[i] = H.huff[i].linmax; }
    static const int kDecMax[32] = {1, 2, 3, 3, 0, 4, 4, 6, 6, 6, 8, 8, 8, 16, 0, 16,
                                    16, 16, 16, 16, 16, 16, 16, 16, 16, 16, 16, 16, 16, 16, 16, 16};
    static const int kBooks[15] = {1, 2, 3, 5, 6, 7, 8, 9, 10, 11, 12, 13, 15, 16, 24};
    for (int t = 0; t < 32; t++) T.dec_max[t] = (uint8_t)kDecMax[t];
    uint16_t *L1 = T.huf_tab, *L2 = T.huf_tab + HUF_L1_N, *C1 = T.huf_tab + HUF_L1_N + HUF_L2_N;
    int l1_used = 1, l2_used = 0;
    for (int t = 0; t < 32; t++) T.huf_tinfo[t] = (uint32_t)H.huff[t].linbits << 4;
    for (int b = 0; b < 15; b++) {
        const int t = kBooks[b];
        const HostHuff &h = H.huff[t];
        static uint16_t tree[512][2];
        std::memset(tree, 0, sizeof tree);
        int n_nodes = 1, longest = 0;
        for (int x = 0; x < kDecMax[t]; x++)
            for (int y = 0; y < kDecMax[t]; y++) {
                const int len = h.hlen[x * h.ylen + y];
                const uint32_t code = h.hcod[x * h.ylen + y];
                longest = std::max(longest, len);
                int node = 0;
                for (int d = 0; d < len; d++) {
                    const int bit = (code >> (len - 1 - d)) & 1;
                    if (d == len - 1) { if (!tree[node][bit]) tree[node][bit] = (uint16_t)(0x8000 | (x << 4) | y); }
                    else {
                        if (!tree[node][bit]) tree[node][bit] = (uint16_t)n_nodes++;
                        node = tree[node][bit];
                        if (node & 0x8000) break;
                    }
                }
            }
        std::function<int(int)> depth = [&](int node) {
            int m = 0;
            for (int bit = 0; bit < 2; bit++) {
                const uint16_t nx = tree[node][bit];
                if (!nx) continue;
                m = std::max(m, (nx & 0x8000) ? 1 : 1 + depth(nx));
            }
            return m;
        };
        const int w = std::min(longest, HUF_W_MAX), base = l1_used;
        const bool has_linbits = t >= 16;
        auto leaf = [&](int len_total, int rel, uint16_t sym) {
            const int x = (sym >> 4) & 15, y = sym & 15, nsig = (x != 0) + (y != 0), adv = len_total + nsig - rel;
            const int c = nsig + (x == 0 && y != 0);
            if (adv < 0 || adv > 15) abort();
            return (uint16_t)(((has_linbits && (x == 15 || y == 15)) ? 0x4000 : 0) | (c << 12) | (adv << 8) | (x << 4) | y);
        };
        if (l1_used + (1 << w) > HUF_L1_N) abort();
        l1_used += 1 << w;
        const uint32_t info = ((uint32_t)(base * 2) << 16) | ((uint32_t)((32 - w) & 31) << 8) | (uint32_t)w;
        for (int k = (t == 16 || t == 24 ? t : t), k_end = (t == 16 || t == 24 ? t + 8 : t + 1); k < k_end; k++)
            T.huf_tinfo[k] = info | ((uint32_t)H.huff[k].linbits << 4);
        for (uint32_t v = 0; v < (1u << w); v++) {
            int node = 0;
            uint16_t e = 0;
            for (int d = 0; d < w; d++) {
                const uint16_t nxt = tree[node][(v >> (w - 1 - d)) & 1];
                if (!nxt) { e = 0; node = -1; break; }
                if (nxt & 0x8000) { e = leaf(d + 1, 0, nxt); node = -1; break; }
                node = nxt;
            }
            if (node > 0) {
                const int k = depth(node), off = l2_used;
                if (k > 15 || (off & 1) || off + (1 << k) > HUF_L2_N || (off >> 1) >= 2048) abort();
                l2_used += (1 << k) + ((1 << k) & 1);
                for (uint32_t u = 0; u < (1u << k); u++) {
                    int nd = node;
                    uint16_t le = 0;
                    for (int d = 0; d < k; d++) {
                        const uint16_t nxt = tree[nd][(u >> (k - 1 - d)) & 1];
                        if (!nxt) break;
                        if (nxt & 0x8000) { le = leaf(w + d + 1, w, nxt); break; }
                        nd = nxt;
                    }
                    L2[off + u] = le;
                }
                e = (uint16_t)(0x8000 | (k << 11) | (off >> 1));
            }
            L1[base + v] = e;
        }
    }
    {
        const HostHuff &q = H.huff[32];
        uint16_t qa[64] = {0};
        for (int e = 0; e < 16; e++) {
            const int len = q.hlen[e];
            const uint32_t base = (uint32_t)q.hcod[e] << (6 - len);
            for (uint32_t f = 0; f < (1u << (6 - len)); f++)
                if (!qa[base + f]) qa[base + f] = (uint16_t)((len << 4) | e);
            T.hcod_c1a[e] = (uint8_t)q.hcod[e];
        }
        for (int book = 0; book < 2; book++) {
            const int w = book ? 8 : 10;
            uint16_t *half0 = C1 + (book ? 2048 : 0), *half1 = half0 + (1 << w);
            for (uint32_t v = 0; v < (1u << w); v++) {
                int val, len;
                if (book) { val = (int)((v >> 4) ^ 15u); len = 4; }
                else { const uint16_t s = qa[v >> 4]; val = s ? (s & 15) : 0; len = s >> 4; }
                const int q0 = (val >> 3) & 1, q1 = (val >> 2) & 1, q2 = (val >> 1) & 1, q3 = val & 1;
                const int n01 = q0 + q1, n23 = q2 + q3;
                half0[v] = (uint16_t)(((n01 + (!q0 && q1)) << 12) | ((len + n01) << 8) | (q0 << 4) | q1);
                half1[v] = (uint16_t)(((n23 + (!q2 && q3)) << 12) | ((len + n01 + n23) << 8) | (q2 << 4) | q3);
            }
        }
        for (int i = 0; i < 256; i++) {
            T.hcod[0][i] = ISO_HCOD_13[i]; T.hcod[1][i] = ISO_HCOD_15[i];
            T.hcod[2][i] = ISO_HCOD_16[i]; T.hcod[3][i] = ISO_HCOD_24[i];
        }
    }
}

}

const HostTables &host_tables()
{
    std::call_once(g_once, build);
    return g_tables;
}

}
```

mp3-steganography-lib_amd/csrc/mp3s_tables.h:

```cpp
#pragma once
#include <stdint.h>

namespace mp3s {

constexpr int POW43_N = 8207;
constexpr int POW2Q_MIN = -266;
constexpr int POW2Q_N = 312;
constexpr int POW2H_N = 40;
constexpr int HUF_W_MAX = 10;
constexpr int HUF_L1_N = 1 + 8 + 64 + 64 + 256 + 128 + 512 + 9 * (1 << HUF_W_MAX) + 7;
constexpr int HUF_L2_N = 1200;
constexpr int HUF_C1_N = 2560;
constexpr int HUF_TAB_N = HUF_L1_N + HUF_L2_N + HUF_C1_N;
static_assert(HUF_L1_N % 8 == 0 && HUF_L2_N % 8 == 0, "the kernel copies the tables 16 bytes at a time");

struct DevTables {
    double synth_matrix[64][32];
    double synth_window[512];
    double synth_window_t[32][16];
    double imdct_cos36[36][18];
    double imdct_cos12[12][6];
    double sine_block[4][36];
    double alias_cs[8], alias_ca[8];
    double pow43[POW43_N];
    double pow2q[POW2Q_N];
    double pow2h[POW2H_N];
    double sqrt2;
    double synth_fast[344];
    double synth_eps_a, synth_eps_x;
    double synth_eps_g, imdct_kappa;
    double synth_window_f[32][16];
    double synth_window_fs[32][16];
    double synth_xbound, synth_reserved;
    double synth_stream[2][8][112];
    double stream_cx[32][16];
    double stream_taps[2][32][16];
    double imdct_rot[1][18];
    double imdct_pq[10][18];
    uint8_t rq_map[3][3][32][20];
    int16_t reorder_src[3][576];
    uint8_t pre_tab[24];
    int32_t enwindow[512];
    int32_t fl[32][64];
    int32_t cos_l[18][36];
    int32_t mdct_cs[8], mdct_ca[8];
    double steptab[128];
    int32_t steptabi[128];
    alignas(16) uint16_t int2idx[10000];
    int32_t sfb_long[3][23];
    int32_t en_base[32], en_step[32];
    int32_t subdv[23][2];
    uint32_t subdiv_lut[3][289];
    uint8_t hlen13[256], hlen15[256], hlen16[256], hlen24[256];
    uint8_t hlen_c1a[16];
    uint8_t linbits[32];
    int32_t linmax[32];
    uint8_t transform[32][2];
    uint8_t dec_max[32];
    uint32_t huf_tinfo[32];
    alignas(16) uint16_t huf_tab[HUF_TAB_N];
    uint32_t hcod[4][256];
    uint8_t hcod_c1a[16];
    uint32_t rl_hl[256][2];
    uint32_t rl_c1w[16];
    uint32_t rl_t1[128], rl_t2[128], rl_t8[128];
};

struct HostHuff {
    int xlen, ylen, linbits, linmax;
    const uint16_t *hcod;
    const uint8_t *hlen;
};

struct HostTables {
    DevTables dev;
    HostHuff huff[34];
    int sfb_short_width[3][12];
    int slen[16][2];
    uint8_t in_h0[32];
    bool analysis_plan_ok;
    int32_t fl_sign[1056];
};

const HostTables &host_tables();

}
```

Measured before the change: 20.97 million frames/s.

## Share MDCT products across outputs with equal-magnitude coefficients via sign plan

Adds a generated plan that groups MDCT cosine coefficients sharing a magnitude, so each mulhi product is computed once and added or subtracted into several outputs. This replaces the plain 18x36 per-output multiply loop in both the standalone and fused MDCT kernels. A per-wave check falls back to the plain path when inputs could make shared rounding differ. The host validates that the table matches the plan. The cost is the extra per-wave check and higher register pressure from the unrolled shared path.

```diff
diff --git a/mp3-steganography-lib_amd/csrc/k_encode.hpp b/mp3-steganography-lib_amd/csrc/k_encode.hpp
--- a/mp3-steganography-lib_amd/csrc/k_encode.hpp
+++ b/mp3-steganography-lib_amd/csrc/k_encode.hpp
@@ -2,6 +2,7 @@
 #include <type_traits>
 #include "analysis_plan.h"
 #include "analysis_sign_plan.h"
+#include "mdct_sign_plan.h"
 #ifndef MP3S_AN_CLOCKS
 #define MP3S_AN_CLOCKS 0
 #endif
@@ -45,6 +46,14 @@
     int pos = 0;
     if (n >= ANALYSIS_SIGN_PRODUCTS) return 0;
     while (n - pos > ANALYSIS_SIGN_FIRST[sign_plan_pass(n)] && ANALYSIS_SIGN_SET[n - pos - 1] == ANALYSIS_SIGN_SET[n]) pos++;
+    return pos;
+}
+
+constexpr int mdct_plan_pos(int n)
+{
+    int pos = 0;
+    if (n >= MDCT_SIGN_PRODUCTS) return 0;
+    while (n - pos > 0 && MDCT_SIGN_SET[n - pos - 1] == MDCT_SIGN_SET[n]) pos++;
     return pos;
 }
 
@@ -354,10 +363,12 @@
 
 constexpr int MD_ROW = 33, MD_BLK = 18 * MD_ROW;
 
-__device__ __forceinline__ void enc_mdct_pair(const int32_t (&in)[54], int32_t *xs, int lane, int32_t *__restrict__ mdct, long ga, long g_lo, long g_hi)
+__device__ __forceinline__ void enc_mdct_pair(const int32_t (&in)[54], int32_t *xs, int lane, int32_t *__restrict__ mdct, long ga, long g_lo, long g_hi,
+                                              bool shared)
 {
     const int ch = lane >> 5, band = lane & 31;
     int32_t *x0 = xs + ch * MD_BLK + band, *x1 = x0 + 2 * MD_BLK;
+    auto sums_plain = [&]() {
     struct Coef { i32x4 q[9]; };
     auto load_coef = [&](int k) {
         Coef c;
@@ -387,6 +398,97 @@
         __builtin_amdgcn_sched_barrier(0);
         cur = nxt;
     }
+    };
+    auto sums_shared = [&]() {
+    static_assert(MDCT_SIGN_BLOCK == 32 && MDCT_SIGN_STREAM % MDCT_SIGN_BLOCK == 0, "four s_load_dwordx8 per block");
+    constexpr int NBLK = MDCT_SIGN_STREAM / MDCT_SIGN_BLOCK;
+    typedef const int32_t __attribute__((address_space(4))) *cs_ptr;
+    cs_ptr sp = (cs_ptr)&c_mdct_sign[0];
+    asm volatile("" : "+s"(sp));
+    auto load_block = [&](auto bc, i32x8 (&c)[4]) {
+        constexpr int Bk = decltype(bc)::value;
+#pragma unroll
+        for (int o = 0; o < 4; o++) c[o] = *(const i32x8 __attribute__((address_space(4))) *)(sp + Bk * MDCT_SIGN_BLOCK + 8 * o);
+    };
+    i32x8 cur[4], nxt[4];
+    uint32_t a[2][18], S[2] = {0, 0}, pend[2] = {0, 0};
+#pragma unroll
+    for (int m = 0; m < 18; m++) a[0][m] = a[1][m] = 0u - (uint32_t)MDCT_SIGN_NEG[m];
+    load_block(std::integral_constant<int, 0>{}, cur);
+    static_for<0, NBLK>([&](auto bc) {
+        constexpr int Bk = decltype(bc)::value;
+        __builtin_amdgcn_sched_barrier(0);
+        __builtin_amdgcn_s_waitcnt(0xc07f);
+        __builtin_amdgcn_sched_barrier(0);
+        if constexpr (Bk + 1 < NBLK) load_block(std::integral_constant<int, Bk + 1>{}, nxt);
+        __builtin_amdgcn_sched_barrier(0);
+        static_for<0, MDCT_SIGN_BLOCK / 8>([&](auto qc) {
+            constexpr int Q = decltype(qc)::value;
+            uint32_t m[2][8];
+            static_for<0, 8>([&](auto ic) {
+                constexpr int I = Q * 8 + decltype(ic)::value, n = Bk * MDCT_SIGN_BLOCK + I;
+                if constexpr (n < MDCT_SIGN_PRODUCTS) {
+                    m[0][I & 7] = (uint32_t)mulhi_vs(in[MDCT_SIGN_COL[n]], cur[I >> 3][I & 7]);
+                    m[1][I & 7] = (uint32_t)mulhi_vs(in[18 + MDCT_SIGN_COL[n]], cur[I >> 3][I & 7]);
+                }
+            });
+            static_for<0, 8>([&](auto ic) {
+                constexpr int I = Q * 8 + decltype(ic)::value, n = Bk * MDCT_SIGN_BLOCK + I;
+                if constexpr (n < MDCT_SIGN_PRODUCTS) {
+                    constexpr int pos = mdct_plan_pos(n);
+                    constexpr uint64_t set = MDCT_SIGN_SET[n];
+                    constexpr bool last = mdct_plan_pos(n + 1) == 0;
+                    constexpr bool multi = ((set & 0x555555555ull) & ((set & 0x555555555ull) - 1ull)) != 0;
+#pragma unroll
+                    for (int g = 0; g < 2; g++) {
+                        if constexpr ((pos & 1) == 0 && !last) pend[g] = m[g][I & 7];
+                        else {
+                            const uint32_t two = (pos & 1) ? pend[g] + m[g][I & 7] : m[g][I & 7];
+                            if constexpr (multi) {
+                                if constexpr (pos < 2) S[g] = two; else S[g] += two;
+                                if constexpr (last) {
+#pragma unroll
+                                    for (int o = 0; o < 18; o++) {
+                                        const unsigned f = (unsigned)(set >> (2 * o)) & 3u;
+                                        if (f == 1u) a[g][o] += S[g];
+                                        if (f == 3u) a[g][o] -= S[g];
+                                    }
+                                }
+                            } else {
+#pragma unroll
+                                for (int o = 0; o < 18; o++)
+                                    if ((set >> (2 * o)) & 1u) {
+                                        a[g][o] += two;
+                                        if constexpr (last) (g ? x1 : x0)[o * MD_ROW] = (int32_t)a[g][o];
+                                    }
+                            }
+                        }
+                    }
+                }
+            });
+            asm("" : "+v"(S[0]), "+v"(S[1]), "+v"(pend[0]), "+v"(pend[1]));
+            __builtin_amdgcn_sched_barrier(0);
+        });
+        if constexpr (Bk + 1 < NBLK) {
+#pragma unroll
+            for (int o = 0; o < 4; o++) cur[o] = nxt[o];
+        }
+    });
+    };
+    bool use_shared = shared;
+    if (shared) {
+        uint32_t rmin = 0xffffffffu;
+        static_for<0, 54>([&](auto jc) {
+            constexpr int j = decltype(jc)::value;
+            constexpr bool counts = (j < 36 && ((MDCT_SIGN_ROWS >> j) & 1u)) || (j >= 18 && ((MDCT_SIGN_ROWS >> (j - 18)) & 1u));
+            if constexpr (counts) {
+                const uint32_t v = (uint32_t)in[j] << MDCT_SIGN_MAX_V2;
+                rmin = rmin < v ? rmin : v;
+            }
+        });
+        use_shared = __ballot(rmin == 0u) == 0;
+    }
+    if (use_shared) sums_shared(); else sums_plain();
     __builtin_amdgcn_s_waitcnt(0xc07f);
     __builtin_amdgcn_wave_barrier();
     if (band >= 1) {
@@ -419,7 +521,7 @@
 
 __global__ __launch_bounds__(256, 4) void k_enc_mdct(
     const int32_t *__restrict__ SB, long Ts, const mp3s_frame_hdr *__restrict__ hdr, int n_frames,
-    int32_t *__restrict__ mdct)
+    int32_t *__restrict__ mdct, int shared)
 {
     __shared__ int32_t xs_all[4][4 * MD_BLK];
     const int wave = __builtin_amdgcn_readfirstlane(threadIdx.x >> 6), lane = threadIdx.x & 63;
@@ -437,7 +539,7 @@
         in[18 + j] = row[j * 32];
         in[36 + j] = row[(18 + j) * 32];
     }
-    enc_mdct_pair(in, xs_all[wave], lane, mdct, 2l * f, 2l * f, 2l * f + 2);
+    enc_mdct_pair(in, xs_all[wave], lane, mdct, 2l * f, 2l * f, 2l * f + 2, shared != 0);
 }
 
 constexpr int EF_GR = 13, EF_SLOTS = 18 * (EF_GR + 1), EF_WAVES = 8;
@@ -447,7 +549,7 @@
 static_assert(((EF_GR + 1) / 2) * 4 * MD_BLK <= EF_TILE_DW, "the MDCT waves' butterfly tiles fit the tile");
 
 __global__ __launch_bounds__(EF_WAVES * 64, 4) void k_enc_fused(
-    const int16_t *__restrict__ pcm, const mp3s_frame_hdr *__restrict__ hdr, int n_frames, int32_t *__restrict__ mdct, int shared)
+    const int16_t *__restrict__ pcm, const mp3s_frame_hdr *__restrict__ hdr, int n_frames, int32_t *__restrict__ mdct, int shared, int mdct_shared)
 {
     __shared__ __attribute__((aligned(16))) uint32_t tile[EF_TILE_DW];
     const int wave = __builtin_amdgcn_readfirstlane(threadIdx.x >> 6), lane = threadIdx.x & 63;
@@ -481,7 +583,7 @@
         }
     }
     __syncthreads();
-    if (unit) enc_mdct_pair(in, reinterpret_cast<int32_t *>(tile) + wave * 4 * MD_BLK, lane, mdct, ga, g0, g_hi);
-}
-
-}
+    if (unit) enc_mdct_pair(in, reinterpret_cast<int32_t *>(tile) + wave * 4 * MD_BLK, lane, mdct, ga, g0, g_hi, mdct_shared != 0);
+}
+
+}
diff --git a/mp3-steganography-lib_amd/csrc/mdct_sign_plan.h b/mp3-steganography-lib_amd/csrc/mdct_sign_plan.h
--- /dev/null
+++ b/mp3-steganography-lib_amd/csrc/mdct_sign_plan.h
@@ -0,0 +1,139 @@
+#pragma once
+#include <cstdint>
+namespace mp3s {
+constexpr int MDCT_SIGN_PRODUCTS = 488;
+constexpr int MDCT_SIGN_BLOCK = 32;
+constexpr int MDCT_SIGN_STREAM = 512;
+constexpr int MDCT_SIGN_MAX_V2 = 6;
+constexpr uint64_t MDCT_SIGN_ROWS = 0x492492492ull;
+constexpr int MDCT_SIGN_NEG[18] = {8, 8, 12, 12, 12, 12, 0, 0, 0, 0, 4, 4, 4, 4, 0, 0, 0, 0};
+constexpr uint8_t MDCT_SIGN_COL[512] = {
+     1,  7, 10, 16, 19, 25, 28, 34,  1,  7, 10, 16, 19, 25, 28, 34,  1,  7, 10, 16, 19, 25, 28, 34,  1,  7, 10, 16, 19, 25, 28, 34,
+     1,  7, 10, 16, 19, 25, 28, 34,  4, 13, 22, 31,  1,  7, 10, 16, 19, 25, 28, 34,  4, 13, 22, 31,  0,  2,  3,  5,  6,  8,  9, 11,
+    12, 14, 15, 17, 18, 20, 21, 23, 24, 26, 27, 29, 30, 32, 33, 35,  0,  2,  3,  5,  6,  8,  9, 11, 12, 14, 15, 17, 18, 20, 21, 23,
+    24, 26, 27, 29, 30, 32, 33, 35,  0,  2,  3,  5,  6,  8,  9, 11, 12, 14, 15, 17, 18, 20, 21, 23, 24, 26, 27, 29, 30, 32, 33, 35,
+     0,  2,  3,  5,  6,  8,  9, 11, 12, 14, 15, 17, 18, 20, 21, 23, 24, 26, 27, 29, 30, 32, 33, 35,  0,  2,  3,  5,  6,  8,  9, 11,
+    12, 14, 15, 17, 18, 20, 21, 23, 24, 26, 27, 29, 30, 32, 33, 35,  0,  2,  3,  5,  6,  8,  9, 11, 12, 14, 15, 17, 18, 20, 21, 23,
+    24, 26, 27, 29, 30, 32, 33, 35,  0,  2,  3,  5,  6,  8,  9, 11, 12, 14, 15, 17, 18, 20, 21, 23, 24, 26, 27, 29, 30, 32, 33, 35,
+     0,  2,  3,  5,  6,  8,  9, 11, 12, 14, 15, 17, 18, 20, 21, 23, 24, 26, 27, 29, 30, 32, 33, 35,  0,  2,  3,  5,  6,  8,  9, 11,
+    12, 14, 15, 17, 18, 20, 21, 23, 24, 26, 27, 29, 30, 32, 33, 35,  0,  2,  3,  5,  6,  8,  9, 11, 12, 14, 15, 17, 18, 20, 21, 23,
+    24, 26, 27, 29, 30, 32, 33, 35,  0,  2,  3,  5,  6,  8,  9, 11, 12, 14, 15, 17, 18, 20, 21, 23, 24, 26, 27, 29, 30, 32, 33, 35,
+     0,  2,  3,  5,  6,  8,  9, 11, 12, 14, 15, 17, 18, 20, 21, 23, 24, 26, 27, 29, 30, 32, 33, 35,  0,  2,  3,  5,  6,  8,  9, 11,
+    12, 14, 15, 17, 18, 20, 21, 23, 24, 26, 27, 29, 30, 32, 33, 35,  0,  2,  3,  5,  6,  8,  9, 11, 12, 14, 15, 17, 18, 20, 21, 23,
+    24, 26, 27, 29, 30, 32, 33, 35,  0,  2,  3,  5,  6,  8,  9, 11, 12, 14, 15, 17, 18, 20, 21, 23, 24, 26, 27, 29, 30, 32, 33, 35,
+     0,  2,  3,  5,  6,  8,  9, 11, 12, 14, 15, 17, 18, 20, 21, 23, 24, 26, 27, 29, 30, 32, 33, 35,  0,  2,  3,  5,  6,  8,  9, 11,
+    12, 14, 15, 17, 18, 20, 21, 23, 24, 26, 27, 29, 30, 32, 33, 35,  0,  2,  3,  5,  6,  8,  9, 11, 12, 14, 15, 17, 18, 20, 21, 23,
+    24, 26, 27, 29, 30, 32, 33, 35,  0,  0,  0,  0,  0,  0,  0,  0,  0,  0,  0,  0,  0,  0,  0,  0,  0,  0,  0,  0,  0,  0,  0,  0,
+};
+constexpr uint64_t MDCT_SIGN_SET[512] = {
+    0x001400003ull, 0x001400003ull, 0x001400003ull, 0x001400003ull, 0x001400003ull, 0x001400003ull, 0x001400003ull, 0x001400003ull,
+    0x00410000cull, 0x00410000cull, 0x00410000cull, 0x00410000cull, 0x00410000cull, 0x00410000cull, 0x00410000cull, 0x00410000cull,
+    0x010040030ull, 0x010040030ull, 0x010040030ull, 0x010040030ull, 0x010040030ull, 0x010040030ull, 0x010040030ull, 0x010040030ull,
+    0x0400100c0ull, 0x0400100c0ull, 0x0400100c0ull, 0x0400100c0ull, 0x0400100c0ull, 0x0400100c0ull, 0x0400100c0ull, 0x0400100c0ull,
+    0x100004300ull, 0x100004300ull, 0x100004300ull, 0x100004300ull, 0x100004300ull, 0x100004300ull, 0x100004300ull, 0x100004300ull,
+    0x143c143c1ull, 0x143c143c1ull, 0x143c143c1ull, 0x143c143c1ull, 0x400001c00ull, 0x400001c00ull, 0x400001c00ull, 0x400001c00ull,
+    0x400001c00ull, 0x400001c00ull, 0x400001c00ull, 0x400001c00ull, 0x41c341c34ull, 0x41c341c34ull, 0x41c341c34ull, 0x41c341c34ull,
+    0x000000001ull, 0x000000001ull, 0x000000001ull, 0x000000001ull, 0x000000001ull, 0x000000001ull, 0x000000001ull, 0x000000001ull,
+    0x000000001ull, 0x000000001ull, 0x000000001ull, 0x000000001ull, 0x000000001ull, 0x000000001ull, 0x000000001ull, 0x000000001ull,
+    0x000000001ull, 0x000000001ull, 0x000000001ull, 0x000000001ull, 0x000000001ull, 0x000000001ull, 0x000000001ull, 0x000000001ull,
+    0x000000004ull, 0x000000004ull, 0x000000004ull, 0x000000004ull, 0x000000004ull, 0x000000004ull, 0x000000004ull, 0x000000004ull,
+    0x000000004ull, 0x000000004ull, 0x000000004ull, 0x000000004ull, 0x000000004ull, 0x000000004ull, 0x000000004ull, 0x000000004ull,
+    0x000000004ull, 0x000000004ull, 0x000000004ull, 0x000000004ull, 0x000000004ull, 0x000000004ull, 0x000000004ull, 0x000000004ull,
+    0x000000010ull, 0x000000010ull, 0x000000010ull, 0x000000010ull, 0x000000010ull, 0x000000010ull, 0x000000010ull, 0x000000010ull,
+    0x000000010ull, 0x000000010ull, 0x000000010ull, 0x000000010ull, 0x000000010ull, 0x000000010ull, 0x000000010ull, 0x000000010ull,
+    0x000000010ull, 0x000000010ull, 0x000000010ull, 0x000000010ull, 0x000000010ull, 0x000000010ull, 0x000000010ull, 0x000000010ull,
+    0x000000040ull, 0x000000040ull, 0x000000040ull, 0x000000040ull, 0x000000040ull, 0x000000040ull, 0x000000040ull, 0x000000040ull,
+    0x000000040ull, 0x000000040ull, 0x000000040ull, 0x000000040ull, 0x000000040ull, 0x000000040ull, 0x000000040ull, 0x000000040ull,
+    0x000000040ull, 0x000000040ull, 0x000000040ull, 0x000000040ull, 0x000000040ull, 0x000000040ull, 0x000000040ull, 0x000000040ull,
+    0x000000100ull, 0x000000100ull, 0x000000100ull, 0x000000100ull, 0x000000100ull, 0x000000100ull, 0x000000100ull, 0x000000100ull,
+    0x000000100ull, 0x000000100ull, 0x000000100ull, 0x000000100ull, 0x000000100ull, 0x000000100ull, 0x000000100ull, 0x000000100ull,
+    0x000000100ull, 0x000000100ull, 0x000000100ull, 0x000000100ull, 0x000000100ull, 0x000000100ull, 0x000000100ull, 0x000000100ull,
+    0x000000400ull, 0x000000400ull, 0x000000400ull, 0x000000400ull, 0x000000400ull, 0x000000400ull, 0x000000400ull, 0x000000400ull,
+    0x000000400ull, 0x000000400ull, 0x000000400ull, 0x000000400ull, 0x000000400ull, 0x000000400ull, 0x000000400ull, 0x000000400ull,
+    0x000000400ull, 0x000000400ull, 0x000000400ull, 0x000000400ull, 0x000000400ull, 0x000000400ull, 0x000000400ull, 0x000000400ull,
+    0x000001000ull, 0x000001000ull, 0x000001000ull, 0x000001000ull, 0x000001000ull, 0x000001000ull, 0x000001000ull, 0x000001000ull,
+    0x000001000ull, 0x000001000ull, 0x000001000ull, 0x000001000ull, 0x000001000ull, 0x000001000ull, 0x000001000ull, 0x000001000ull,
+    0x000001000ull, 0x000001000ull, 0x000001000ull, 0x000001000ull, 0x000001000ull, 0x000001000ull, 0x000001000ull, 0x000001000ull,
+    0x000004000ull, 0x000004000ull, 0x000004000ull, 0x000004000ull, 0x000004000ull, 0x000004000ull, 0x000004000ull, 0x000004000ull,
+    0x000004000ull, 0x000004000ull, 0x000004000ull, 0x000004000ull, 0x000004000ull, 0x000004000ull, 0x000004000ull, 0x000004000ull,
+    0x000004000ull, 0x000004000ull, 0x000004000ull, 0x000004000ull, 0x000004000ull, 0x000004000ull, 0x000004000ull, 0x000004000ull,
+    0x000010000ull, 0x000010000ull, 0x000010000ull, 0x000010000ull, 0x000010000ull, 0x000010000ull, 0x000010000ull, 0x000010000ull,
+    0x000010000ull, 0x000010000ull, 0x000010000ull, 0x000010000ull, 0x000010000ull, 0x000010000ull, 0x000010000ull, 0x000010000ull,
+    0x000010000ull, 0x000010000ull, 0x000010000ull, 0x000010000ull, 0x000010000ull, 0x000010000ull, 0x000010000ull, 0x000010000ull,
+    0x000040000ull, 0x000040000ull, 0x000040000ull, 0x000040000ull, 0x000040000ull, 0x000040000ull, 0x000040000ull, 0x000040000ull,
+    0x000040000ull, 0x000040000ull, 0x000040000ull, 0x000040000ull, 0x000040000ull, 0x000040000ull, 0x000040000ull, 0x000040000ull,
+    0x000040000ull, 0x000040000ull, 0x000040000ull, 0x000040000ull, 0x000040000ull, 0x000040000ull, 0x000040000ull, 0x000040000ull,
+    0x000100000ull, 0x000100000ull, 0x000100000ull, 0x000100000ull, 0x000100000ull, 0x000100000ull, 0x000100000ull, 0x000100000ull,
+    0x000100000ull, 0x000100000ull, 0x000100000ull, 0x000100000ull, 0x000100000ull, 0x000100000ull, 0x000100000ull, 0x000100000ull,
+    0x000100000ull, 0x000100000ull, 0x000100000ull, 0x000100000ull, 0x000100000ull, 0x000100000ull, 0x000100000ull, 0x000100000ull,
+    0x000400000ull, 0x000400000ull, 0x000400000ull, 0x000400000ull, 0x000400000ull, 0x000400000ull, 0x000400000ull, 0x000400000ull,
+    0x000400000ull, 0x000400000ull, 0x000400000ull, 0x000400000ull, 0x000400000ull, 0x000400000ull, 0x000400000ull, 0x000400000ull,
+    0x000400000ull, 0x000400000ull, 0x000400000ull, 0x000400000ull, 0x000400000ull, 0x000400000ull, 0x000400000ull, 0x000400000ull,
+    0x001000000ull, 0x001000000ull, 0x001000000ull, 0x001000000ull, 0x001000000ull, 0x001000000ull, 0x001000000ull, 0x001000000ull,
+    0x001000000ull, 0x001000000ull, 0x001000000ull, 0x001000000ull, 0x001000000ull, 0x001000000ull, 0x001000000ull, 0x001000000ull,
+    0x001000000ull, 0x001000000ull, 0x001000000ull, 0x001000000ull, 0x001000000ull, 0x001000000ull, 0x001000000ull, 0x001000000ull,
+    0x004000000ull, 0x004000000ull, 0x004000000ull, 0x004000000ull, 0x004000000ull, 0x004000000ull, 0x004000000ull, 0x004000000ull,
+    0x004000000ull, 0x004000000ull, 0x004000000ull, 0x004000000ull, 0x004000000ull, 0x004000000ull, 0x004000000ull, 0x004000000ull,
+    0x004000000ull, 0x004000000ull, 0x004000000ull, 0x004000000ull, 0x004000000ull, 0x004000000ull, 0x004000000ull, 0x004000000ull,
+    0x010000000ull, 0x010000000ull, 0x010000000ull, 0x010000000ull, 0x010000000ull, 0x010000000ull, 0x010000000ull, 0x010000000ull,
+    0x010000000ull, 0x010000000ull, 0x010000000ull, 0x010000000ull, 0x010000000ull, 0x010000000ull, 0x010000000ull, 0x010000000ull,
+    0x010000000ull, 0x010000000ull, 0x010000000ull, 0x010000000ull, 0x010000000ull, 0x010000000ull, 0x010000000ull, 0x010000000ull,
+    0x040000000ull, 0x040000000ull, 0x040000000ull, 0x040000000ull, 0x040000000ull, 0x040000000ull, 0x040000000ull, 0x040000000ull,
+    0x040000000ull, 0x040000000ull, 0x040000000ull, 0x040000000ull, 0x040000000ull, 0x040000000ull, 0x040000000ull, 0x040000000ull,
+    0x040000000ull, 0x040000000ull, 0x040000000ull, 0x040000000ull, 0x040000000ull, 0x040000000ull, 0x040000000ull, 0x040000000ull,
+    0x100000000ull, 0x100000000ull, 0x100000000ull, 0x100000000ull, 0x100000000ull, 0x100000000ull, 0x100000000ull, 0x100000000ull,
+    0x100000000ull, 0x100000000ull, 0x100000000ull, 0x100000000ull, 0x100000000ull, 0x100000000ull, 0x100000000ull, 0x100000000ull,
+    0x100000000ull, 0x100000000ull, 0x100000000ull, 0x100000000ull, 0x100000000ull, 0x100000000ull, 0x100000000ull, 0x100000000ull,
+    0x400000000ull, 0x400000000ull, 0x400000000ull, 0x400000000ull, 0x400000000ull, 0x400000000ull, 0x400000000ull, 0x400000000ull,
+    0x400000000ull, 0x400000000ull, 0x400000000ull, 0x400000000ull, 0x400000000ull, 0x400000000ull, 0x400000000ull, 0x400000000ull,
+    0x400000000ull, 0x400000000ull, 0x400000000ull, 0x400000000ull, 0x400000000ull, 0x400000000ull, 0x400000000ull, 0x400000000ull,
+    0x000000000ull, 0x000000000ull, 0x000000000ull, 0x000000000ull, 0x000000000ull, 0x000000000ull, 0x000000000ull, 0x000000000ull,
+    0x000000000ull, 0x000000000ull, 0x000000000ull, 0x000000000ull, 0x000000000ull, 0x000000000ull, 0x000000000ull, 0x000000000ull,
+    0x000000000ull, 0x000000000ull, 0x000000000ull, 0x000000000ull, 0x000000000ull, 0x000000000ull, 0x000000000ull, 0x000000000ull,
+};
+constexpr int32_t MDCT_SIGN_COEF[512] = {
+     -170637571,  -170637571,   222379212,  1296121036,  1689137820,  1689137820,  1296121036,   222379212,   258966078,   500284046,  -651982862, -1967042654,
+     -814775745,  1574025869,  1207792529,  -107267261,    36586865,  -795836990,  1037154958,  -277904833, -2110896781,  1351646656,  1037154958,  -277904833,
+     -277904833,  1037154958, -1351646656,  2110896781,  -277904833,  1037154958,   795836990,   -36586865,   107267261, -1207792529,  1574025869,  -814775745,
+     1967042654,   651982862,   500284046,   258966078,   314491698,  -759250124, -1832991948,  -759250124,   222379212,  1296121036, -1689137820, -1689137820,
+     1296121036,   222379212,   170637571,   170637571,  -759250124,  1832991948,  -759250124,  -314491698,    63283832,   249737143,   298179147,   298179147,
+      249737143,    63283832,   -69062184,  -392008792,  -572796813,  -945703435, -1126491457, -1449438064, -1581784081, -1768237392, -1816679397, -1816679397,
+    -1768237392, -1581784081, -1449438064, -1126491457,  -945703435,  -572796813,  -392008792,   -69062184,   -74314931,  -460824098,  -640236213,  -786687264,
+     -702414579,  -189369869,   206660948,  1102570034,  1511212175,  2030569848,  2078643179,  1702091766,  1306060948,   273658566,  -267329592, -1159593886,
+    -1436897244, -1569745749, -1438406965,  -915404502,  -603646369,   -84288696,    60668643,    57023852,   -50329886,   139768215,   436269664,   990653814,
+     1023470462,   314014687,  -342686898, -1606526823, -1903028272, -1383670599,  -630453677,  1152743920,  1809445506,  1999543607,  1510011487,   -83088008,
+     -836304930, -1545760704, -1416428721,  -532784999,   -43252879,   476104793,   443288145,    79002096,    83088008,   342686898,   139768215,  -836304930,
+    -1152743920,  -436269664,   476104793,  1809445506,  1606526823,  -443288145, -1545760704, -1903028272,  -990653814,  1416428721,  1999543607,  1023470462,
+      -79002096, -1510011487, -1383670599,   -50329886,   532784999,   630453677,   314014687,   -43252879,    35846692,  -429419697,  -596605174,   379467971,
+     1066011120,   555204365,  -605899243, -1673302281,  -728951191,  1892189868,  1936987082,  -821024235, -1982127844,  -802326319,   783770706,  1759843851,
+      693104498, -1462770171, -1340381908,   441556263,   916116723,   247121954,  -177871462,   -86541570,   -89336498,    20274314,   544629123,   214621000,
+     -779524439,  -669913625,   731082434,  1223608269,  -412283106, -1727342898,   -91451522,  2046142226,   645146165, -2094584230, -1100438790,  1859688915,
+     1335334105, -1404396290, -1286892101,   850701647,   968092773,  -346967017,  -464358144,    28167689,   -20274314,   412283106,   -28167689,  -731082434,
+      346967017,   779524439,  -850701647,  -544629123,  1404396290,    89336498, -1859688915,   464358144,  2094584230,  -968092773, -2046142226,  1286892101,
+     1727342898, -1335334105, -1223608269,  1100438790,   669913625,  -645146165,  -214621000,    91451522,    92870544,  -368751054,  -512316477,   983114341,
+      150606618,  -883202600,   963846506,  -236405037, -1888545077,  1624860276,  1663328516, -2127085184,  -280036077,  1276316860, -1246799142,   248631676,
+     1795674533, -1256109222, -1151012038,  1143970843,   129429458,  -393114259,   282952635,   -12226639,     4085911,  -100601247,   615873008,  -879557809,
+     -619958920,   980159057, -1069655911,   973140575,  1689614832, -1953299633,   453782903,   -93582766, -2143397735,  2046882399,   615873008,  -879557809,
+     1527524726, -1167324589, -1069655911,   973140575,  -457868814,   194184013,   453782903,   -93582766,   -93582766,   453782903,  -194184013,   457868814,
+      973140575, -1069655911,  1167324589, -1527524726,  -879557809,   615873008, -2046882399,  2143397735,   -93582766,   453782903,  1953299633, -1689614832,
+      973140575, -1069655911,  -980159057,   619958920,  -879557809,   615873008,   100601247,    -4085911,    12226639,  -282952635,  -393114259,   129429458,
+    -1143970843,  1151012038, -1256109222,  1795674533,  -248631676,  1246799142,  1276316860,  -280036077,  2127085184, -1663328516,  1624860276, -1888545077,
+      236405037,  -963846506,  -883202600,   150606618,  -983114341,   512316477,  -368751054,    92870544,    91451522,  -214621000,   645146165,  -669913625,
+     1100438790, -1223608269,  1335334105, -1727342898,  1286892101, -2046142226,   968092773, -2094584230,   464358144, -1859688915,   -89336498, -1404396290,
+     -544629123,  -850701647,  -779524439,  -346967017,  -731082434,   -28167689,  -412283106,    20274314,   -28167689,   464358144,  -346967017,   968092773,
+     -850701647,  1286892101, -1404396290,  1335334105, -1859688915,  1100438790, -2094584230,   645146165, -2046142226,    91451522, -1727342898,  -412283106,
+    -1223608269,  -731082434,  -669913625,  -779524439,  -214621000,  -544629123,    20274314,   -89336498,   -86541570,  -177871462,  -247121954,  -916116723,
+      441556263, -1340381908,  1462770171,  -693104498,  1759843851,   783770706,   802326319,  1982127844,  -821024235,  1936987082, -1892189868,   728951191,
+    -1673302281,  -605899243,  -555204365, -1066011120,   379467971,  -596605174,   429419697,   -35846692,    43252879,  -314014687,   630453677,   532784999,
+       50329886,  1383670599, -1510011487,   -79002096, -1023470462, -1999543607,  1416428721,  -990653814,  1903028272,  1545760704,  -443288145,  1606526823,
+    -1809445506,  -476104793,  -436269664, -1152743920,   836304930,  -139768215,   342686898,    83088008,    79002096,   443288145,  -476104793,    43252879,
+     -532784999, -1416428721,  1545760704,   836304930,   -83088008,  1510011487, -1999543607, -1809445506,  1152743920,  -630453677,  1383670599,  1903028272,
+    -1606526823,  -342686898,  -314014687, -1023470462,   990653814,   436269664,  -139768215,    50329886,   -57023852,   -60668643,   -84288696,  -603646369,
+      915404502,  1438406965, -1569745749, -1436897244,  1159593886,   267329592,   273658566,  1306060948, -1702091766, -2078643179,  2030569848,  1511212175,
+    -1102570034,  -206660948,  -189369869,  -702414579,   786687264,   640236213,  -460824098,   -74314931,   -69062184,  -392008792,   572796813,   945703435,
+    -1126491457, -1449438064,  1581784081,  1768237392, -1816679397, -1816679397,  1768237392,  1581784081, -1449438064, -1126491457,   945703435,   572796813,
+     -392008792,   -69062184,   -63283832,  -249737143,   298179147,   298179147,  -249737143,   -63283832,           0,           0,           0,           0,
+              0,           0,           0,           0,           0,           0,           0,           0,           0,           0,           0,           0,
+              0,           0,           0,           0,           0,           0,           0,           0,
+};
+}
diff --git a/mp3-steganography-lib_amd/csrc/mp3s_api.cpp b/mp3-steganography-lib_amd/csrc/mp3s_api.cpp
--- a/mp3-steganography-lib_amd/csrc/mp3s_api.cpp
+++ b/mp3-steganography-lib_amd/csrc/mp3s_api.cpp
@@ -151,6 +151,7 @@
     c->chain = new ChainResolver();
     c->device = device;
     for (const OptRow &o : kOptions) c->opt[o.id] = option_from_env(o);
+    if (const char *v = getenv("MP3S_MDCT_SHARED")) c->mdct_shared = !*v || atoll(v) != 0;
     if (hipStreamCreateWithFlags(&c->stream, hipStreamNonBlocking) != hipSuccess ||
         hipEventCreate(&c->ev0) != hipSuccess || hipEventCreate(&c->ev1) != hipSuccess ||
         hipEventCreateWithFlags(&c->ev_order, hipEventDisableTiming) != hipSuccess) {
@@ -540,9 +541,12 @@
     if (!host_tables().analysis_plan_ok)
         return fail(MP3S_E_TABLES, "the analysis filter table built on this host does not repeat itself where the kernel shares products "
                                    "(csrc/analysis_plan.h, csrc/analysis_sign_plan.h: run tools/gen_analysis_plan.py and tools/gen_analysis_sign_plan.py here and rebuild)");
+    if (!host_tables().mdct_plan_ok)
+        return fail(MP3S_E_TABLES, "the MDCT table built on this host does not repeat itself where the kernel shares products "
+                                   "(csrc/mdct_sign_plan.h: run tools/gen_mdct_sign_plan.py here and rebuild)");
     const bool fused = c->opt[MP3S_OPT_FUSED_ENCODE] != 0;
     if (const int rc = fused ? (int)MP3S_OK : c->ensure_scratch_enc(enc_scratch_bytes(n_frames))) return rc;
-    const int e = launch_encode(stream, d_pcm, d_hdr, n_frames, d_mdct, c->scratch_enc, &c->prof, fused, c->opt[MP3S_OPT_ANALYSIS_SHARED] != 0);
+    const int e = launch_encode(stream, d_pcm, d_hdr, n_frames, d_mdct, c->scratch_enc, &c->prof, fused, c->opt[MP3S_OPT_ANALYSIS_SHARED] != 0, c->mdct_shared);
     return e ? fail(MP3S_E_HIP, "encode launch: %s", hipGetErrorString((hipError_t)e)) : (int)MP3S_OK;
 }
 
diff --git a/mp3-steganography-lib_amd/csrc/mp3s_device.h b/mp3-steganography-lib_amd/csrc/mp3s_device.h
--- a/mp3-steganography-lib_amd/csrc/mp3s_device.h
+++ b/mp3-steganography-lib_amd/csrc/mp3s_device.h
@@ -48,7 +48,7 @@
 size_t enc_scratch_bytes(int n_frames);
 int launch_encode(hipStream_t stream, const int16_t *d_pcm, const mp3s_frame_hdr *d_hdr, int n_frames, int32_t *d_mdct,
                   void *d_scratch, Profiler *prof, bool fused = false ,
-                  bool analysis_shared = true );
+                  bool analysis_shared = true , bool mdct_shared = true );
 
 struct RateVariantArgs {
     const int32_t *d_unit, *d_cursor;
diff --git a/mp3-steganography-lib_amd/csrc/mp3s_device.hip b/mp3-steganography-lib_amd/csrc/mp3s_device.hip
--- a/mp3-steganography-lib_amd/csrc/mp3s_device.hip
+++ b/mp3-steganography-lib_amd/csrc/mp3s_device.hip
@@ -9,10 +9,12 @@
 #include "mp3s_host.h"
 #include "mp3s_tables.h"
 #include "analysis_sign_plan.h"
+#include "mdct_sign_plan.h"
 
 namespace mp3s {
 __constant__ DevTables c_tab;
 __constant__ __attribute__((aligned(64))) int32_t c_fl_sign[ANALYSIS_SIGN_STREAM];
+__constant__ __attribute__((aligned(64))) int32_t c_mdct_sign[MDCT_SIGN_STREAM];
 }
 
 #include "k_wave.hpp"
@@ -73,6 +75,9 @@
     if (e != hipSuccess) return (int)e;
     static_assert(sizeof h.fl_sign == sizeof(int32_t) * ANALYSIS_SIGN_STREAM, "the coefficient stream and its symbol");
     e = hipMemcpyToSymbolAsync(HIP_SYMBOL(c_fl_sign), h.fl_sign, sizeof h.fl_sign, 0, hipMemcpyHostToDevice, stream);
+    if (e != hipSuccess) return (int)e;
+    static_assert(sizeof h.mdct_sign == sizeof(int32_t) * MDCT_SIGN_STREAM, "the coefficient stream and its symbol");
+    e = hipMemcpyToSymbolAsync(HIP_SYMBOL(c_mdct_sign), h.mdct_sign, sizeof h.mdct_sign, 0, hipMemcpyHostToDevice, stream);
     if (e != hipSuccess) return (int)e;
     return (int)hipStreamSynchronize(stream);
 }
@@ -167,12 +172,12 @@
 }
 
 int launch_encode(hipStream_t stream, const int16_t *d_pcm, const mp3s_frame_hdr *d_hdr, int n_frames, int32_t *d_mdct,
-                  void *d_scratch, Profiler *prof, bool fused, bool analysis_shared)
+                  void *d_scratch, Profiler *prof, bool fused, bool analysis_shared, bool mdct_shared)
 {
     if (fused) {
         const long n_gran = (long)n_frames * 2;
         const int pf = prof ? prof->begin(stream, K_ENC_ANALYSIS) : -1;
-        hipLaunchKernelGGL(k_enc_fused, dim3((unsigned)((n_gran + EF_GR - 1) / EF_GR)), dim3(EF_WAVES * 64), 0, stream, d_pcm, d_hdr, n_frames, d_mdct, (int)analysis_shared);
+        hipLaunchKernelGGL(k_enc_fused, dim3((unsigned)((n_gran + EF_GR - 1) / EF_GR)), dim3(EF_WAVES * 64), 0, stream, d_pcm, d_hdr, n_frames, d_mdct, (int)analysis_shared, (int)mdct_shared);
         if (prof) prof->end(stream, pf);
         return (int)hipGetLastError();
     }
@@ -185,7 +190,7 @@
     if (prof) prof->end(stream, pp);
     pp = prof ? prof->begin(stream, K_ENC_MDCT) : -1;
     hipLaunchKernelGGL(k_enc_mdct, dim3((n_frames + 3) / 4), dim3(256), 0, stream, (const int32_t *)SB, Ts, d_hdr, n_frames,
-                       d_mdct);
+                       d_mdct, (int)mdct_shared);
     if (prof) prof->end(stream, pp);
     return (int)hipGetLastError();
 }
diff --git a/mp3-steganography-lib_amd/csrc/mp3s_internal.h b/mp3-steganography-lib_amd/csrc/mp3s_internal.h
--- a/mp3-steganography-lib_amd/csrc/mp3s_internal.h
+++ b/mp3-steganography-lib_amd/csrc/mp3s_internal.h
@@ -61,6 +61,7 @@
 struct mp3s_ctx {
     int device = 0;
     int64_t opt[MP3S_OPT_COUNT] = {0};
+    bool mdct_shared = true;
     mp3s_run_stats run_stats = {0, 0, 0, 0, 0};
     mp3s_pipe *own_pipe = nullptr;
     std::vector<mp3s_pipe *> parked_pipes;
diff --git a/mp3-steganography-lib_amd/csrc/mp3s_tables.cpp b/mp3-steganography-lib_amd/csrc/mp3s_tables.cpp
--- a/mp3-steganography-lib_amd/csrc/mp3s_tables.cpp
+++ b/mp3-steganography-lib_amd/csrc/mp3s_tables.cpp
@@ -2,6 +2,7 @@
 #include "iso_tables.h"
 #include "analysis_plan.h"
 #include "analysis_sign_plan.h"
+#include "mdct_sign_plan.h"
 
 #include <algorithm>
 #include <cmath>
@@ -295,6 +296,30 @@
             T.cos_l[m][k] = (int32_t)(std::sin(0.087266462599717 * (k + 0.5)) *
                                       std::cos((3.14159265358979 / 72) * (double)(2 * k + 19) * (double)(2 * m + 1)) *
                                       2147483647.0);
+    {
+        static_assert(sizeof H.mdct_sign == sizeof(int32_t) * MDCT_SIGN_STREAM, "HostTables::mdct_sign holds the plan's stream");
+        H.mdct_plan_ok = true;
+        std::memset(H.mdct_sign, 0, sizeof H.mdct_sign);
+        uint8_t fed[18][36] = {};
+        for (int n = 0; n < MDCT_SIGN_PRODUCTS; n++) {
+            const int k = MDCT_SIGN_COL[n];
+            const int32_t rep = MDCT_SIGN_COEF[n];
+            bool have = false;
+            for (int m = 0; m < 18; m++) {
+                const unsigned f = (unsigned)(MDCT_SIGN_SET[n] >> (2 * m)) & 3u;
+                if (!f) continue;
+                const int32_t c = T.cos_l[m][k];
+                if (c == 0 || c == INT32_MIN || (f != 1u && f != 3u) || (int64_t)c != (f == 1u ? (int64_t)rep : -(int64_t)rep)) H.mdct_plan_ok = false;
+                fed[m][k]++;
+                have = true;
+            }
+            if (!have) H.mdct_plan_ok = false;
+            H.mdct_sign[n] = rep;
+        }
+        for (int m = 0; m < 18; m++)
+            for (int k = 0; k < 36; k++)
+                if (fed[m][k] != 1) H.mdct_plan_ok = false;
+    }
     for (int i = 0; i < 128; i++) {
         T.steptab[i] = std::pow(2.0, (double)(127 - i) / 4);
         T.steptabi[i] = (T.steptab[i] * 2 > 2147483647.0) ? 0x7fffffff : (int32_t)(T.steptab[i] * 2 + 0.5);
diff --git a/mp3-steganography-lib_amd/csrc/mp3s_tables.h b/mp3-steganography-lib_amd/csrc/mp3s_tables.h
--- a/mp3-steganography-lib_amd/csrc/mp3s_tables.h
+++ b/mp3-steganography-lib_amd/csrc/mp3s_tables.h
@@ -80,6 +80,8 @@
     uint8_t in_h0[32];
     bool analysis_plan_ok;
     int32_t fl_sign[1056];
+    bool mdct_plan_ok;
+    int32_t mdct_sign[512];
 };
 
 const HostTables &host_tables();
```

Result: no change. 21.17 million frames/s (median of 6 runs) (+0.9%).
